# young-how/DQN-based-UAV-3D_path_planer

Hardware: AMD Instinct MI355X
Metric: env-steps/sec + learner updates/sec, PathPlan_City DQN (higher is better)
Workload: dtype f64

## Files before the change

### dqn_based_uav_3d_path_planer_amd/_lib.py

```python
from __future__ import annotations

import ctypes as C
import os

from . import _build

OBS_DIM = 100
MAX_BUILDINGS = 64
ABI_VERSION = 5

OK, EINVAL, ENOMEM, EHIP, ENODEV, EP2P = 0, -22, -12, -5, -19, -70
P2P_ERR_TIMEOUT, P2P_ERR_DIVERGED = 1, 2
COLL_ID_BYTES = 128
INFO_NORMAL, INFO_SUCCESS, INFO_LOSE, INFO_SKIPPED = 0, 1, 2, 3
INFO_NAMES = ("normal", "success", "lose", "skipped")
ACT_STEER_F32, ACT_STEER_F64, ACT_INDEX_I32 = 0, 1, 2
OBS_F32, OBS_F16, OBS_PACKED = 0, 1, 2
PACKED_DWORDS = 20
META_BYTES = 16
MFMA_F32, MFMA_F16 = 0, 1
P2P_HANDLE_BYTES = 64
P2P_CHECK_MAX_BLOCKS = 40
STEP_AUTO_RESET, STEP_SKIP_DONE, STEP_NO_OBS, STEP_ONE_WAVE, STEP_APF_LANE = 1, 2, 4, 8, 16

SYMBOLS = (
    "uavenv_abi_version", "uavenv_last_error", "uavenv_create", "uavenv_destroy", "uavenv_num_agents",
    "uavenv_set_buildings", "uavenv_load_scenarios", "uavenv_plan_scenarios", "uavenv_bank_stats", "uavenv_replan_begin", "uavenv_replan_ready", "uavenv_replan_commit", "uavenv_replan_stats", "uavenv_bank_read", "uavenv_set_moved_word", "uavenv_set_step_meta", "uavenv_tick", "uavenv_dqn_reduce_adam_gated", "uavenv_per_set_f32_gated", "uavenv_rrt_plan", "uavenv_reset_all", "uavenv_set_state", "uavenv_get_state",
    "uavenv_step", "uavenv_step_policy", "uavenv_set_debug_buffer", "uavenv_observe", "uavenv_threaten_rate", "uavenv_threaten_rate_allpairs", "uavenv_geometry",
    "uavenv_replay_sample", "uavenv_obs_unpack", "uavenv_replay_draw", "uavenv_replay_draw_valid", "uavenv_select_actions",
    "uavenv_dqn_num_params", "uavenv_dqn_partial_stride", "uavenv_dqn_partial_rows", "uavenv_dqn_set_debug_buffer", "uavenv_dqn_grad", "uavenv_dqn_grad_w", "uavenv_dqn_reduce", "uavenv_dqn_adam", "uavenv_dqn_reduce_adam", "uavenv_dqn_act",
    "uavenv_p2p_create", "uavenv_p2p_handle", "uavenv_p2p_connect", "uavenv_p2p_destroy", "uavenv_p2p_errors",
    "uavenv_p2p_configure", "uavenv_p2p_status", "uavenv_p2p_error_word", "uavenv_p2p_check_blocks", "uavenv_p2p_inject_fault", "uavenv_p2p_can_reach",
    "uavenv_coll_last_error", "uavenv_coll_unique_id", "uavenv_coll_create", "uavenv_coll_destroy", "uavenv_coll_allreduce_sum",
    "uavenv_dqn_reduce_p2p", "uavenv_dqn_adam_p2p",
    "uavenv_loop_create", "uavenv_loop_destroy", "uavenv_loop_set_eps", "uavenv_loop_run", "uavenv_loop_get", "uavenv_loop_get_per", "uavenv_loop_step_times",
    "uavenv_randn", "uavenv_sac_loop_noise_floats", "uavenv_sac_loop_create", "uavenv_sac_loop_destroy", "uavenv_sac_loop_run",
    "uavenv_sac_loop_get", "uavenv_sac_loop_get_per", "uavenv_per_fill_frame_strided", "uavenv_sac_act_multi", "uavenv_sac_critic_grad_multi", "uavenv_sac_actor_grad_multi",
    "uavenv_sac_critic_adam_multi", "uavenv_sac_actor_adam_multi",
    "uavenv_per_num_chunks", "uavenv_per_rotation", "uavenv_per_rebuild", "uavenv_per_sample", "uavenv_per_set", "uavenv_per_fill", "uavenv_per_set_f32", "uavenv_per_weights", "uavenv_per_fill_frame", "uavenv_per_rebuild_frame", "uavenv_p2p_allreduce", "uavenv_sac_partial_rows_n",
    "uavenv_sac_act", "uavenv_sac_reduce", "uavenv_sac_partial_rows", "uavenv_sac_last_error", "uavenv_sac_set_debug_buffer", "uavenv_sac_critic_grad", "uavenv_sac_critic_adam", "uavenv_sac_actor_grad",
    "uavenv_sac_actor_adam", "uavenv_fed_aggregate", "uavenv_eval_episodes", "uavenv_eval_episodes_sac", "uavenv_eval_noise_fill",
)
SAC_CRITIC_IN, SAC_ACTOR_PARAMS, SAC_CRITIC_PARAMS, SAC_ACTOR_STRIDE, SAC_CRITIC_STRIDE = 102, 6724, 10882, 6728, 21768


class UavEnvConfig(C.Structure):
    _fields_ = [
        ("abi_version", C.c_int32), ("device", C.c_int32), ("n_envs", C.c_int32), ("uav_per_env", C.c_int32),
        ("max_subgoals", C.c_int32), ("max_step", C.c_int32), ("apf_enabled", C.c_int32), ("obs_dtype", C.c_int32),
        ("n_actions", C.c_int32), ("reserved0", C.c_int32),
        ("len", C.c_double), ("width", C.c_double), ("h", C.c_double),
        ("max_v", C.c_double), ("steering_angle", C.c_double), ("power", C.c_double * 8), ("cell_size", C.c_double),
    ]


class UavReplayRing(C.Structure):
    _fields_ = [
        ("obs", C.c_void_p), ("action", C.c_void_p), ("reward", C.c_void_p), ("done", C.c_void_p),
        ("valid", C.c_void_p), ("frames", C.c_int32), ("n_agents", C.c_int32), ("obs_dtype", C.c_int32),
        ("action_is_index", C.c_int32), ("meta", C.c_void_p),
    ]


class UavDqnNet(C.Structure):
    _fields_ = [("local", C.c_void_p), ("target", C.c_void_p), ("m", C.c_void_p), ("v", C.c_void_p),
                ("w", C.c_int32), ("hid", C.c_int32), ("n_actions", C.c_int32), ("dueling", C.c_int32),
                ("mfma_dtype", C.c_int32), ("reserved0", C.c_int32)]


EVAL_SUCCESS, EVAL_LOSE, EVAL_TRUNCATED, EVAL_INVALID = 1, 2, 4, 5
EVAL_RECORD_BYTES = 64


class UavEvalRecord(C.Structure):
    _fields_ = [("ret", C.c_double), ("total_score", C.c_double), ("path_len", C.c_double), ("energy", C.c_double),
                ("v0x", C.c_double), ("v0y", C.c_double), ("steps", C.c_int32), ("subgoals", C.c_int32),
                ("collisions", C.c_int32), ("outcome", C.c_uint8), ("reach_goal", C.c_uint8), ("slot", C.c_uint8),
                ("reserved", C.c_uint8)]


class UavEvalArgs(C.Structure):
    _fields_ = [("n", C.c_int32), ("first", C.c_int32), ("start_goal", C.c_void_p), ("sub", C.c_void_p),
                ("nsub", C.c_void_p), ("m", C.c_int32), ("max_steps", C.c_int32), ("v0", C.c_void_p),
                ("seed", C.c_uint64), ("eps", C.c_float), ("traj_steps", C.c_int32), ("records", C.c_void_p),
                ("traj_pos", C.c_void_p), ("traj_act", C.c_void_p), ("max_workgroups", C.c_int32),
                ("reserved0", C.c_int32)]


EVAL_SAC_MEAN, EVAL_SAC_SAMPLE = 0, 1


class UavSacEvalArgs(C.Structure):
    _fields_ = [("n", C.c_int32), ("first", C.c_int32), ("start_goal", C.c_void_p), ("sub", C.c_void_p),
                ("nsub", C.c_void_p), ("m", C.c_int32), ("max_steps", C.c_int32), ("v0", C.c_void_p),
                ("seed", C.c_uint64), ("actors", C.POINTER(C.c_void_p)), ("n_actors", C.c_int32),
                ("action_bound", C.c_float), ("mode", C.c_int32), ("traj_steps", C.c_int32), ("records", C.c_void_p),
                ("traj_pos", C.c_void_p), ("traj_act", C.c_void_p), ("max_workgroups", C.c_int32),
                ("reserved0", C.c_int32)]


class UavPer(C.Structure):
    _fields_ = [("prio", C.c_void_p), ("chunk_sum", C.c_void_p), ("chunk_prefix", C.c_void_p),
                ("capacity", C.c_int64), ("rot", C.c_int64), ("group_sum", C.c_void_p)]


class UavLoopConfig(C.Structure):
    _fields_ = [("env", C.c_void_p), ("ring", UavReplayRing), ("net", UavDqnNet),
                ("head", C.c_int32), ("filled", C.c_int32), ("batch", C.c_int32), ("kind", C.c_int32),
                ("huber", C.c_int32), ("update_loop", C.c_int32), ("epoch", C.c_int32), ("learn_start", C.c_int32),
                ("seed", C.c_uint64), ("counter", C.c_uint64),
                ("eps", C.c_float), ("gamma", C.c_float), ("lr", C.c_float), ("beta1", C.c_float), ("beta2", C.c_float),
                ("adam_eps", C.c_float), ("step_flags", C.c_uint32), ("partials_dev", C.c_void_p),
                ("loss_dev", C.c_void_p), ("info_dev", C.c_void_p), ("p2p", C.c_void_p), ("time_every", C.c_int32),
                ("sample_lag", C.c_int32), ("coll", C.c_void_p), ("raw_dev", C.c_void_p),
                ("per", UavPer), ("per_alpha", C.c_double), ("per_beta", C.c_double), ("per_beta_inc", C.c_double),
                ("per_eps", C.c_double), ("per_clip", C.c_double),
                ("per_slots_dev", C.c_void_p), ("per_prio_dev", C.c_void_p), ("per_w_dev", C.c_void_p),
                ("per_abs_dev", C.c_void_p), ("per_idx_dev", C.c_void_p),
                ("replan_every", C.c_int32), ("replan_count", C.c_int32), ("replan_max_iter", C.c_int32), ("reserved1", C.c_int32),
                ("moved_dev", C.c_void_p)]


class UavLoopCursor(C.Structure):
    _fields_ = [("head", C.c_int32), ("filled", C.c_int32), ("epoch", C.c_int32), ("reserved0", C.c_int32),
                ("counter", C.c_uint64)]


class UavSacNets(C.Structure):
    _fields_ = [("actor", C.c_void_p), ("critic1", C.c_void_p), ("critic2", C.c_void_p), ("target1", C.c_void_p),
                ("target2", C.c_void_p), ("log_alpha", C.c_void_p)]


class UavSacBatch(C.Structure):
    _fields_ = [("obs_packed", C.c_void_p), ("idx_s", C.c_void_p), ("idx_n", C.c_void_p), ("draws", C.c_void_p),
                ("n_agents", C.c_int32), ("uav_per_env", C.c_int32), ("slot", C.c_int32), ("frames", C.c_int32),
                ("act0", C.c_void_p), ("act1", C.c_void_p), ("reward", C.c_void_p), ("done", C.c_void_p), ("valid", C.c_void_p),
                ("eps", C.c_void_p), ("batch", C.c_int32), ("tiles_per_wg", C.c_int32),
                ("is_weights", C.c_void_p), ("abs_td_out", C.c_void_p), ("meta", C.c_void_p), ("td_scratch", C.c_void_p)]


class UavSacAdam(C.Structure):
    _fields_ = [("lr", C.c_float), ("beta1", C.c_float), ("beta2", C.c_float), ("eps", C.c_float),
                ("bias_correction1", C.c_float), ("bias_correction2_sqrt", C.c_float), ("tau", C.c_float), ("grad_scale", C.c_float),
                ("skip_word", C.c_void_p), ("go_word", C.c_void_p), ("go_value", C.c_uint32), ("reserved0", C.c_uint32)]


SAC_LOOP_MAX_SLOTS = 8
FED_MAX_BLOCKS = 8
DRAW_MAX_TRIES = 8
DQN_IMAGE_FLOATS = 6912


class UavSacLoopSlot(C.Structure):
    _fields_ = [("nets", UavSacNets), ("m_actor", C.c_void_p), ("v_actor", C.c_void_p), ("alpha_mv", C.c_void_p),
                ("m1", C.c_void_p), ("v1", C.c_void_p), ("m2", C.c_void_p), ("v2", C.c_void_p), ("scalars", C.c_void_p),
                ("partials_critic", C.c_void_p), ("partials_actor", C.c_void_p),
                ("epoch", C.c_int32), ("adam_steps", C.c_int32),
                ("per", UavPer), ("per_slots_dev", C.c_void_p), ("per_prio_dev", C.c_void_p), ("per_w_dev", C.c_void_p),
                ("per_abs_dev", C.c_void_p), ("per_beta", C.c_double), ("td_dev", C.c_void_p)]


class UavSacLoopConfig(C.Structure):
    _fields_ = [("env", C.c_void_p), ("ring", UavReplayRing), ("act1_plane", C.c_void_p), ("info_dev", C.c_void_p),
                ("n_slots", C.c_int32), ("batch", C.c_int32), ("head", C.c_int32), ("filled", C.c_int32),
                ("is_train", C.c_int32), ("valid_draws", C.c_int32), ("seed", C.c_uint64), ("counter", C.c_uint64),
                ("beta1", C.c_double), ("beta2", C.c_double), ("adam_eps", C.c_double),
                ("gamma", C.c_float), ("tau", C.c_float), ("action_bound", C.c_float), ("actor_lr", C.c_float),
                ("critic_lr", C.c_float), ("alpha_lr", C.c_float), ("target_entropy", C.c_float), ("reserved1", C.c_float),
                ("step_flags", C.c_uint32), ("reserved2", C.c_uint32),
                ("draws_dev", C.c_void_p), ("noise_dev", C.c_void_p), ("slot", UavSacLoopSlot * SAC_LOOP_MAX_SLOTS),
                ("p2p", C.c_void_p), ("coll", C.c_void_p), ("xbuf_dev", C.c_void_p),
                ("per_alpha", C.c_double), ("per_beta_inc", C.c_double), ("per_eps", C.c_double), ("per_clip", C.c_double),
                ("moved_dev", C.c_void_p), ("check_every", C.c_int32), ("reserved3", C.c_int32)]


class UavSacLoopCursor(C.Structure):
    _fields_ = [("head", C.c_int32), ("filled", C.c_int32), ("counter", C.c_uint64),
                ("epoch", C.c_int32 * SAC_LOOP_MAX_SLOTS), ("adam_steps", C.c_int32 * SAC_LOOP_MAX_SLOTS)]


class UavEnvError(RuntimeError):
    pass


_LIB = None


def load() -> C.CDLL:
    global _LIB
    if _LIB is not None:
        return _LIB
    import torch
    path = _build.LIB_PATH
    if _build.needs_build():
        _build.build()
    if not os.path.exists(path):
        raise UavEnvError(f"{path} is missing and could not be built; the env hot path has no CPU fallback")
    lib = C.CDLL(path)
    vp, i32, u32, u64, i64, f32 = C.c_void_p, C.c_int32, C.c_uint32, C.c_uint64, C.c_int64, C.c_float
    lib.uavenv_abi_version.restype = C.c_int
    lib.uavenv_last_error.restype = C.c_char_p
    lib.uavenv_create.restype = C.c_int
    lib.uavenv_create.argtypes = [C.POINTER(UavEnvConfig), C.POINTER(vp)]
    lib.uavenv_destroy.restype = C.c_int
    lib.uavenv_destroy.argtypes = [vp]
    lib.uavenv_num_agents.restype = C.c_int
    lib.uavenv_num_agents.argtypes = [vp]
    lib.uavenv_set_buildings.restype = C.c_int
    lib.uavenv_set_buildings.argtypes = [vp, vp, vp, i32]
    lib.uavenv_load_scenarios.restype = C.c_int
    lib.uavenv_load_scenarios.argtypes = [vp, vp, vp, vp, i32]
    lib.uavenv_plan_scenarios.restype = C.c_int
    lib.uavenv_plan_scenarios.argtypes = [vp, i32, u64, i32, vp]
    lib.uavenv_bank_stats.restype = C.c_int
    lib.uavenv_bank_stats.argtypes = [vp, vp, vp]
    lib.uavenv_replan_begin.restype = C.c_int
    lib.uavenv_replan_begin.argtypes = [vp, i32, i32, u64, i32, vp]
    lib.uavenv_replan_ready.restype = C.c_int
    lib.uavenv_replan_ready.argtypes = [vp]
    lib.uavenv_replan_commit.restype = C.c_int
    lib.uavenv_replan_commit.argtypes = [vp, i32, vp]
    lib.uavenv_replan_stats.restype = C.c_int
    lib.uavenv_replan_stats.argtypes = [vp, vp]
    lib.uavenv_set_moved_word.restype = C.c_int
    lib.uavenv_set_moved_word.argtypes = [vp, vp]
    lib.uavenv_set_step_meta.restype = C.c_int
    lib.uavenv_set_step_meta.argtypes = [vp, vp, vp]
    lib.uavenv_tick.restype = C.c_uint64
    lib.uavenv_tick.argtypes = [vp]
    lib.uavenv_bank_read.restype = C.c_int
    lib.uavenv_bank_read.argtypes = [vp, i32, i32, vp, vp, vp]
    lib.uavenv_rrt_plan.restype = C.c_int
    lib.uavenv_rrt_plan.argtypes = [vp, i32, vp, vp, i32, u64, i32, C.c_double, C.c_double, vp, vp, vp, vp, vp]
    lib.uavenv_reset_all.restype = C.c_int
    lib.uavenv_reset_all.argtypes = [vp, u64, vp]
    lib.uavenv_set_state.restype = C.c_int
    lib.uavenv_set_state.argtypes = [vp, i32, i32, vp, vp, vp, vp, vp]
    lib.uavenv_get_state.restype = C.c_int
    lib.uavenv_get_state.argtypes = [vp, i32, i32, vp, vp, vp]
    lib.uavenv_step.restype = C.c_int
    lib.uavenv_step.argtypes = [vp, vp, i32, vp, vp, vp, vp, vp, vp, vp, vp, vp, u32, vp]
    lib.uavenv_step_policy.restype = C.c_int
    lib.uavenv_step_policy.argtypes = [vp, C.POINTER(UavDqnNet), vp, f32, u64, u64, vp, vp, vp, vp, vp, vp, vp, vp, vp, vp, u32, vp]
    lib.uavenv_set_debug_buffer.restype = C.c_int
    lib.uavenv_set_debug_buffer.argtypes = [vp, vp]
    lib.uavenv_observe.restype = C.c_int
    lib.uavenv_observe.argtypes = [vp, vp, vp]
    lib.uavenv_threaten_rate.restype = C.c_int
    lib.uavenv_threaten_rate.argtypes = [vp, vp, vp, i64, vp]
    lib.uavenv_geometry.restype = C.c_int
    lib.uavenv_geometry.argtypes = [vp, vp, vp, i64, vp]
    lib.uavenv_threaten_rate_allpairs.restype = C.c_int
    lib.uavenv_threaten_rate_allpairs.argtypes = [vp, vp, vp, i64, vp]
    lib.uavenv_replay_sample.restype = C.c_int
    lib.uavenv_replay_sample.argtypes = [C.POINTER(UavReplayRing), i32, i32, i32, u64, u64, vp, vp, vp, vp, vp, vp, vp]
    lib.uavenv_obs_unpack.restype = C.c_int
    lib.uavenv_obs_unpack.argtypes = [vp, i64, vp, i32, vp]
    lib.uavenv_replay_draw.restype = C.c_int
    lib.uavenv_replay_draw.argtypes = [i32, i32, i32, i32, i32, u64, u64, vp, vp]
    lib.uavenv_replay_draw_valid.restype = C.c_int
    lib.uavenv_replay_draw_valid.argtypes = [i32, i32, i32, i32, i32, i32, i32, i32, vp, i32, u64, u64, vp, vp]
    lib.uavenv_p2p_create.restype = C.c_int
    lib.uavenv_p2p_create.argtypes = [i32, i32, i32, C.POINTER(vp)]
    lib.uavenv_p2p_handle.restype = C.c_int
    lib.uavenv_p2p_handle.argtypes = [vp, vp]
    lib.uavenv_p2p_connect.restype = C.c_int
    lib.uavenv_p2p_connect.argtypes = [vp, vp]
    lib.uavenv_p2p_destroy.restype = C.c_int
    lib.uavenv_p2p_destroy.argtypes = [vp]
    lib.uavenv_p2p_errors.restype = C.c_int
    lib.uavenv_p2p_errors.argtypes = [vp, C.POINTER(i32)]
    lib.uavenv_p2p_configure.restype = C.c_int
    lib.uavenv_p2p_configure.argtypes = [vp, i32, i32]
    lib.uavenv_p2p_status.restype = C.c_int
    lib.uavenv_p2p_status.argtypes = [vp, i32, C.POINTER(i32)]
    lib.uavenv_p2p_can_reach.restype = C.c_int
    lib.uavenv_p2p_can_reach.argtypes = [i32, i32]
    lib.uavenv_p2p_inject_fault.restype = C.c_int
    lib.uavenv_p2p_inject_fault.argtypes = [vp, i32]
    lib.uavenv_coll_last_error.restype = C.c_char_p
    lib.uavenv_coll_unique_id.restype = C.c_int
    lib.uavenv_coll_unique_id.argtypes = [C.c_char_p, vp]
    lib.uavenv_coll_create.restype = C.c_int
    lib.uavenv_coll_create.argtypes = [C.c_char_p, i32, i32, vp, C.POINTER(vp)]
    lib.uavenv_coll_destroy.restype = C.c_int
    lib.uavenv_coll_destroy.argtypes = [vp]
    lib.uavenv_coll_allreduce_sum.restype = C.c_int
    lib.uavenv_coll_allreduce_sum.argtypes = [vp, vp, i64, vp]
    lib.uavenv_dqn_reduce_p2p.restype = C.c_int
    lib.uavenv_dqn_reduce_p2p.argtypes = [C.POINTER(UavDqnNet), vp, i32, vp, vp]
    lib.uavenv_dqn_adam_p2p.restype = C.c_int
    lib.uavenv_dqn_adam_p2p.argtypes = [C.POINTER(UavDqnNet), vp, f32, f32, f32, f32, i32, i32, vp, vp, vp]
    lib.uavenv_loop_create.restype = C.c_int
    lib.uavenv_loop_create.argtypes = [C.POINTER(UavLoopConfig), C.POINTER(vp)]
    lib.uavenv_loop_destroy.restype = C.c_int
    lib.uavenv_loop_destroy.argtypes = [vp]
    lib.uavenv_loop_set_eps.restype = C.c_int
    lib.uavenv_loop_set_eps.argtypes = [vp, f32]
    lib.uavenv_loop_run.restype = C.c_int
    lib.uavenv_loop_run.argtypes = [vp, i32, vp]
    lib.uavenv_loop_get.restype = C.c_int
    lib.uavenv_loop_get.argtypes = [vp, C.POINTER(UavLoopCursor)]
    lib.uavenv_loop_step_times.restype = C.c_int
    lib.uavenv_loop_step_times.argtypes = [vp, vp, i32, C.POINTER(i32)]
    for _n in ("uavenv_sac_act_multi", "uavenv_sac_critic_grad_multi", "uavenv_sac_actor_grad_multi",
               "uavenv_sac_critic_adam_multi", "uavenv_sac_actor_adam_multi"):
        getattr(lib, _n).restype = C.c_int
    lib.uavenv_sac_critic_grad_multi.argtypes = [vp, vp, i32, f32, f32, vp, vp]
    lib.uavenv_sac_actor_grad_multi.argtypes = [vp, vp, i32, f32, vp, vp]
    lib.uavenv_sac_critic_adam_multi.argtypes = [vp, vp, i32, vp, vp, vp, vp, vp, vp, i32, vp]
# ... 123 lines not shown
```

### dqn_based_uav_3d_path_planer_amd/csrc/dqn_internal.hpp

```cpp
#pragma once
#include <stdint.h>

#include "../../include/uavenv.h"

extern "C" {

#define UAVENV_DQN_IMAGE_FLOATS 6912

int uavenv_dqn_split_image(const UavDqnNet *net, float *image_dev, void *stream);

int uavenv_dqn_grad_img(const UavReplayRing *ring, int32_t head, int32_t filled, int32_t batch, uint64_t seed, uint64_t counter,
                        const int32_t *explicit_idx, const UavDqnNet *net, int32_t kind, float gamma, int32_t huber,
                        const float *is_weights, float *abs_td_out, float *partials, const float *image_dev, void *stream);

int uavenv_dqn_reduce_adam_img(const UavDqnNet *net, const float *partials, int32_t n_partials, float lr, float beta1, float beta2,
                               float eps, int32_t step_t, int32_t hard_update, float *loss_out, float *raw_out,
                               const uint32_t *go_word, uint32_t go_value, float *image_dev, void *stream);

int uavenv_dqn_adam_p2p_img(const UavDqnNet *net, struct UavP2P *c, float lr, float beta1, float beta2, float eps, int32_t step_t,
                            int32_t hard_update, float *loss_out, float *raw_out, float *image_dev, void *stream);
int uavenv_dqn_adam_img(const UavDqnNet *net, const float *raw, float lr, float beta1, float beta2, float eps, int32_t step_t,
                        int32_t hard_update, float *loss_out, float *image_dev, void *stream);

int uavenv_step_policy_img(UavEnv *e, const UavDqnNet *net, const void *obs_cur, float eps, uint64_t seed, uint64_t counter,
                           int32_t *action_out, void *obs, double *reward64, float *reward32, uint8_t *ret_done, uint8_t *agent_done,
                           uint8_t *info, uint8_t *valid, double *energy64, const uint8_t *active, uint32_t flags,
                           const float *image_dev, void *stream);

}
```

### dqn_based_uav_3d_path_planer_amd/csrc/learner.hip

```cpp
#include <hip/hip_runtime.h>
#include <hip/hip_fp16.h>
#include <stdint.h>
#include <stdlib.h>

#include "../../include/uavenv.h"
#include "uavenv_device.hpp"
#include "qnet_device.hpp"
#include "dqn_internal.hpp"

using namespace uav;
using namespace uavq;

namespace {

struct GradArgs {
    UavReplayRing ring;
    int head, filled, batch;
    uint64_t seed, counter;
    ReplayPerm perm;
    const int32_t *explicit_idx;
    const float *local, *target;
    int n_actions, dueling, kind;
    float gamma;
    int huber;
    float *partials;
    int P;
    unsigned long long *dbg;
    const float *is_w;
    float *abs_td;
    const float *img;
};

#ifdef UAVENV_PHASE_PROFILE
#define L_STAMP(slot) do { if (g.dbg && threadIdx.x == 0) g.dbg[(size_t)blockIdx.x * 8 + (slot)] = __builtin_amdgcn_s_memtime(); } while (0)
#define L_STAMP2(slot) do { if (g.dbg && threadIdx.x == 0) g.dbg[((size_t)gridDim.x + blockIdx.x) * 8 + (slot)] = __builtin_amdgcn_s_memtime(); } while (0)
#else
#define L_STAMP(slot) do { } while (0)
#define L_STAMP2(slot) do { } while (0)
#endif


__device__ __forceinline__ void load_transition(const UavReplayRing &R, uint32_t row, int &act, float &rew, uint32_t &done, uint32_t &valid)
{
    if (R.meta) {
        const uint4 m = reinterpret_cast<const uint4 *>(R.meta)[row];
        act = (int)m.y;
        rew = __uint_as_float(m.z);
        done = m.w & 0xffu;
        valid = (m.w >> 8) & 0xffu;
    } else {
        act = reinterpret_cast<const int32_t *>(R.action)[row];
        rew = R.reward[row];
        done = R.done[row];
        valid = R.valid ? (uint32_t)R.valid[row] : 1u;
    }
}

template <typename T>
__device__ __forceinline__ floatx4 x_load(const T *obs, uint32_t ring_row, int q)
{
    if (sizeof(T) == 4) {
        return *reinterpret_cast<const floatx4 *>(reinterpret_cast<const float *>(obs) + (size_t)ring_row * kW + 4 * q);
    } else {
        const uint2 raw = *reinterpret_cast<const uint2 *>(reinterpret_cast<const __half *>(obs) + (size_t)ring_row * kW + 4 * q);
        return floatx4{__uint_as_float(raw.x), __uint_as_float(raw.y), 0.0f, 0.0f};
    }
}

template <typename T>
__device__ __forceinline__ void x_issue(floatx4 (&v)[kXIters], const T *obs, uint32_t my_row)
{
    const int lane = (int)threadIdx.x & 63;
#pragma unroll
    for (int it = 0; it < kXIters; ++it) {
        int c = it * 64 + lane;
        c = c < 400 ? c : 399;
        const int row = c / 25, q = c - row * 25;
        const uint32_t ring_row = (uint32_t)__shfl((int)my_row, row, 64);
        v[it] = x_load<T>(obs, ring_row, q);
    }
}

template <typename T>
__device__ __forceinline__ void x_commit(float *strip, floatx4 (&v)[kXIters])
{
    const int lane = (int)threadIdx.x & 63;
#pragma unroll
    for (int it = 0; it < kXIters; ++it) {
        const int c = it * 64 + lane;
        if (c < 400) {
            const int row = c / 25, q = c - row * 25;
            floatx4 w = v[it];
            if (sizeof(T) != 4) {
                const uint32_t rx = __float_as_uint(v[it][0]), ry = __float_as_uint(v[it][1]);
                const __half2 lo = *reinterpret_cast<const __half2 *>(&rx);
                const __half2 hi = *reinterpret_cast<const __half2 *>(&ry);
                w = floatx4{__low2float(lo), __high2float(lo), __low2float(hi), __high2float(hi)};
            }
            *reinterpret_cast<floatx4 *>(strip + row * kLd + 4 * q) = w;
        }
    }
    if (lane < 16) *reinterpret_cast<floatx4 *>(strip + lane * kLd + kW) = floatx4{1.0f, 0.0f, 0.0f, 0.0f};
}

__device__ __forceinline__ void fwd_strip(const float *W, const float *strip, floatx4 (&acc)[4])
{
    const int lane = (int)threadIdx.x & 63, r = lane & 15, g = lane >> 4;
    const float *xp = strip + r * kLd + 26 * g;
    const float *wp = W + r * kLd + 26 * g;
#pragma unroll
    for (int t = 0; t < 4; ++t) acc[t] = floatx4{0.0f, 0.0f, 0.0f, 0.0f};
    float2 b = *reinterpret_cast<const float2 *>(xp);
    float2 a[4];
// ... 577 lines not shown
struct FlagOps {
    half8 one[2][6];
};
__device__ __forceinline__ half8 tiny_of(const half8 &one)
{
    uintx4 d = *reinterpret_cast<const uintx4 *>(&one);
#pragma unroll
    for (int k = 0; k < 4; ++k) d[k] = (d[k] << 2) & 0x10001000u;
    return *reinterpret_cast<const half8 *>(&d);
}
__device__ __forceinline__ void flag_ops_build(const GradLdsP &L, int r, int gq, FlagOps &F)
{
    const uint32_t *pr = L.Ps + 4 * gq * kPackedDwords;
#pragma unroll
    for (int q = 0; q < 2; ++q) {
        uintx4 mk[8];
#pragma unroll
        for (int i = 0; i < 8; ++i) mk[i] = *reinterpret_cast<const uintx4 *>(pr + (32 * q + 16 * (i >> 2) + (i & 3)) * kPackedDwords);
#pragma unroll
        for (int u = 0; u < 6; ++u) {
            half8 tiny;
            flags_to_half8(mk, u >> 1, (uint32_t)(16 * (u & 1) + r), F.one[q][u], tiny);
        }
    }
}
__device__ __forceinline__ void grad_products_split8b(const GradLdsP &L, const float *amax4, int grp, int strip, int r, int gq,
                                                      const FlagOps &F, GradAcc8 &A)
{
    const float *db = L.dHs + 4 * gq * kLh + 16 * strip + r;
    float dh[2][8];
    if (grp == 1) {
        float up, down;
        split_scale(fmaxf(fmaxf(amax4[0], amax4[1]), fmaxf(amax4[2], amax4[3])), up, down);
#pragma unroll
        for (int q = 0; q < 2; ++q)
#pragma unroll
            for (int i = 0; i < 8; ++i) dh[q][i] = db[(32 * q + 16 * (i >> 2) + (i & 3)) * kLh];
        floatx4 ch[6];
#pragma unroll
        for (int u = 0; u < 6; ++u) ch[u] = floatx4{0.0f, 0.0f, 0.0f, 0.0f};
#pragma unroll
        for (int q = 0; q < 2; ++q) {
            half8 bh, bm;
            split_half8(dh[q], up, bh, bm);
#pragma unroll
            for (int u = 0; u < 6; ++u) ch[u] = mfma16h(F.one[q][u], bh, ch[u]);
#pragma unroll
            for (int u = 0; u < 6; ++u) ch[u] = mfma16h(tiny_of(F.one[q][u]), bm, ch[u]);
        }
#pragma unroll
        for (int u = 0; u < 6; ++u)
#pragma unroll
            for (int k = 0; k < 4; ++k) A.acc[u][k] += ch[u][k] * down;
        return;
    }
    const uint32_t *pr = L.Ps + 4 * gq * kPackedDwords;
    const int dsc = r < 15 ? 4 + r : 19;
    const float *ha = L.Hs + 4 * gq * kLh + 16 * strip + r;
    const float *ob = L.douts + 4 * gq * kMaxOut + r;
    float xs[2][8], hh[2][8], bo[2][8];
#pragma unroll
    for (int q = 0; q < 2; ++q)
#pragma unroll
        for (int i = 0; i < 8; ++i) {
            const int s1 = 32 * q + 16 * (i >> 2) + (i & 3);
            dh[q][i] = db[s1 * kLh];
            xs[q][i] = __uint_as_float(pr[s1 * kPackedDwords + dsc]);
            hh[q][i] = ha[s1 * kLh];
            bo[q][i] = ob[s1 * kMaxOut];
        }
    floatx4 csc = floatx4{0.0f, 0.0f, 0.0f, 0.0f}, cw2 = floatx4{0.0f, 0.0f, 0.0f, 0.0f};
    const bool ones = r == 15;
#pragma unroll
    for (int q = 0; q < 2; ++q)
#pragma unroll
        for (int i = 0; i < 8; ++i) {
            csc = mfma16(ones ? 1.0f : xs[q][i], dh[q][i], csc);
            cw2 = mfma16(hh[q][i], bo[q][i], cw2);
        }
#pragma unroll
    for (int k = 0; k < 4; ++k) { A.acc[0][k] += csc[k]; A.acc[1][k] += cw2[k]; }
}

template <bool FIRST, int SPLIT, bool GLDS>
__device__ __forceinline__ void grad_tile_packed8(const GradArgs &g, const GradLdsP &L, float *qn_lds, int tile, bool more,
                                                  GradAcc8 &A)
{
    constexpr int NMAX = 4;
    const int tid = (int)threadIdx.x, lane = tid & 63, wv = __builtin_amdgcn_readfirstlane(tid >> 6), grp = wv >> 2, strip = wv & 3;
    const int r = lane & 15, gq = lane >> 4, t256 = tid & 255;
    const int n2 = g.n_actions + (g.dueling ? 1 : 0);
    const uint32_t *obs = reinterpret_cast<const uint32_t *>(g.ring.obs);
    const float *net = grp == 0 ? g.local : g.target;
    floatx4 vW[kStageIters];
    SplitScRegs vS;
    float pw[4] = {0, 0, 0, 0}, pb2 = 0.0f;
    if (FIRST) {
        if (GLDS) img_glds(grp == 0 ? L.W1l : L.W1t, g.img + (grp == 0 ? 0 : kSplitF), strip);
        else if (g.img) img_issue(vW, g.img + (grp == 0 ? 0 : kSplitF));
        else w_issue_half(vW, net, t256);
        const NetDev nv = net_view(net, n2);
        if (!GLDS && !g.img) w_issue_sc(vS, net, nv.b1);
#pragma unroll
        for (int k = 0; k < 4; ++k) pw[k] = nv.W2[t256 + 256 * k < n2 * kHid ? t256 + 256 * k : 0];
        pb2 = nv.b2[t256 < n2 ? t256 : 0];
    }
    L_STAMP2(0);
    const int smp = tile * kTile + strip * 16 + r;
    int f, agent;
    if (g.explicit_idx) {
        f = g.explicit_idx[2 * smp];
        agent = g.explicit_idx[2 * smp + 1];
    } else {
        replay_slot_to_frame(g.perm, replay_perm_apply(g.perm, (uint32_t)smp), g.head, g.ring.frames, f, agent);
    }
    int fn = f + 1;
    if (fn >= g.ring.frames) fn = 0;
    const uint32_t row_s = (uint32_t)f * (uint32_t)g.ring.n_agents + (uint32_t)agent;
    const uint32_t row_n = (uint32_t)fn * (uint32_t)g.ring.n_agents + (uint32_t)agent;
    L_STAMP2(1);
    PRow R;
    prow_load(R, obs + (size_t)(grp == 0 ? row_s : row_n) * kPackedDwords);
    int p_act = 0;
    float p_rew = 0.0f, p_w = 1.0f;
    uint32_t raw_done = 0u, raw_valid = 1u;
    if (grp == 0) {
        load_transition(g.ring, row_s, p_act, p_rew, raw_done, raw_valid);
        p_w = g.is_w ? g.is_w[smp] : 1.0f;
    }
    L_STAMP(6);
    if (FIRST) {
        if (!GLDS) {
            if (g.img) img_commit(grp == 0 ? L.W1l : L.W1t, vW); else w_commit_split(w1split_at(grp == 0 ? L.W1l : L.W1t), vW, vS);
        }
        L_STAMP(7);
        float *W2 = grp == 0 ? L.W2l : L.W2t, *b2 = grp == 0 ? L.b2l : L.b2t;
#pragma unroll
        for (int k = 0; k < 4; ++k)
            if (t256 + 256 * k < n2 * kHid) W2[t256 + 256 * k] = pw[k];
        if (t256 < n2) b2[t256] = pb2;
        __syncthreads();
    }
    L_STAMP(1);
    floatx4 hl[4];
    W2Frag<NMAX> Fl;
    float ql[NMAX];
    if (grp == 0) {
        fwd_strip_split<false>(w1split_at(L.W1l), R, hl);
        w2_load<NMAX>(Fl, L.W2l, L.b2l, n2);
        q_strip<NMAX>(hl, Fl, n2, g.n_actions, g.dueling, ql);
        if (gq == 0) prow_store_lds(L.Ps + (strip * 16 + r) * kPackedDwords, R);
    } else {
        int best = 0;
        floatx4 ht[4];
        if (g.kind == 1) {
            fwd_strip_split<false>(w1split_at(L.W1l), R, ht);
            W2Frag<NMAX> F;
            w2_load<NMAX>(F, L.W2l, L.b2l, n2);
            float qn_l[NMAX];
            q_strip<NMAX>(ht, F, n2, g.n_actions, g.dueling, qn_l);
            float bq = qn_l[0];
#pragma unroll
            for (int a = 1; a < NMAX; ++a)
                if (a < g.n_actions && qn_l[a] > bq) { bq = qn_l[a]; best = a; }
        }
        fwd_strip_split<false>(w1split_at(L.W1t), R, ht);
        W2Frag<NMAX> Ft;
        w2_load<NMAX>(Ft, L.W2t, L.b2t, n2);
        float qt[NMAX];
        q_strip<NMAX>(ht, Ft, n2, g.n_actions, g.dueling, qt);
        if (gq == 0) qn_lds[strip * 16 + r] = pick_qn<NMAX>(g, qt, best);
    }
    L_STAMP(2);
    __syncthreads();
    L_STAMP(3);
    FlagOps FO;
    if (SPLIT == 2 && grp == 1) flag_ops_build(L, r, gq, FO);
    if (grp == 0) {
        GradAcc<NMAX> T;
#pragma unroll
        for (int a = 0; a < NMAX + 2; ++a) T.csum[a] = A.csum[a];
        float amax = 0.0f;
        const float p_done = (float)raw_done, p_valid = (float)raw_valid;
        td_backward<NMAX>(g, L.W2l, hl, Fl, ql, qn_lds[strip * 16 + r], p_act, p_rew, p_done, p_valid, p_w, smp, T,
                          L.Hs + (strip * 16 + r) * kLh, L.dHs + (strip * 16 + r) * kLh, L.douts + (strip * 16 + r) * kMaxOut,
                          SPLIT ? &amax : nullptr);
#pragma unroll
        for (int a = 0; a < NMAX + 2; ++a) A.csum[a] = T.csum[a];
        if (SPLIT) {
            amax = wave_max64(amax);
            if (lane == 0) qn_lds[kTile + strip] = amax;
        }
    }
    __syncthreads();
    L_STAMP(4);
    if (SPLIT) {
        if (SPLIT == 2) grad_products_split8b(L, qn_lds + kTile, grp, strip, r, gq, FO, A);
        else grad_products_split8(L, qn_lds + kTile, grp, strip, r, gq, A);
        if (more) __syncthreads();
        return;
    }
    {
        const uint32_t *pr = L.Ps + 4 * gq * kPackedDwords;
        const int ia = 4 + (r < 11 ? r : 10), ib = 15 + (r < 6 ? 0 : (r > 9 ? 3 : r - 6));
        const bool sc0 = r < 11, sc5 = r >= 6 && r <= 9;
        const float ones = r == 4 ? 1.0f : 0.0f;
        const int sh = grp == 0 ? r : 16 + r;
        const float *db = L.dHs + 4 * gq * kLh + 16 * strip + r;
        const float *ha = L.Hs + 4 * gq * kLh + 16 * strip + r;
        const float *ob = L.douts + 4 * gq * kMaxOut + r;
        struct Raw { uintx4 mk; float sx, bdh, ah, bo; };
        auto load = [&](int k) {
            const int s1 = (k & 3) + 16 * (k >> 2);
            Raw w;
            w.mk = *reinterpret_cast<const uintx4 *>(pr + s1 * kPackedDwords);
            w.sx = __uint_as_float(pr[s1 * kPackedDwords + (grp == 0 ? ia : ib)]);
            w.bdh = db[s1 * kLh];
            w.ah = ha[s1 * kLh];
            w.bo = ob[s1 * kMaxOut];
            return w;
        };
        auto decode = [&](const Raw &w, float (&ax)[4]) {
            const float b0 = (float)((w.mk[0] >> sh) & 1u), b1 = (float)((w.mk[1] >> sh) & 1u), b2 = (float)((w.mk[2] >> sh) & 1u);
            if (grp == 0) { ax[0] = sc0 ? w.sx : b0; ax[1] = b1; ax[2] = b2; ax[3] = ones; }
            else { ax[0] = b0; ax[1] = b1; ax[2] = sc5 ? w.sx : b2; ax[3] = w.ah; }
        };
        Raw cur = load(0), nxt = load(1);
        float ax[4];
        decode(cur, ax);
#pragma unroll
        for (int kk = 0; kk < 16; ++kk) {
            Raw nn = nxt;
            if (kk + 2 < 16) nn = load(kk + 2);
            float axn[4];
            decode(nxt, axn);
            __builtin_amdgcn_sched_barrier(0);
#pragma unroll
            for (int u = 0; u < 3; ++u) A.acc[u] = mfma16(ax[u], cur.bdh, A.acc[u]);
            A.acc[3] = mfma16(ax[3], grp == 0 ? cur.bdh : cur.bo, A.acc[3]);
            __builtin_amdgcn_sched_barrier(0);
            cur = nxt;
            nxt = nn;
#pragma unroll
            for (int u = 0; u < 4; ++u) ax[u] = axn[u];
        }
    }
    if (more) __syncthreads();
}

template <int SPLIT, bool GLDS = false>
__global__ void __launch_bounds__(512) k_dqn_grad_packed8(Grad2Args ga)
{
    UAV_HOT_PRIO();
    constexpr int NMAX = 4;
    const GradArgs &g = ga.g;
    extern __shared__ __align__(16) float lds[];
    GradLdsP L;
    L.W1l = lds;
    L.W1t = L.W1l + kTileF;
    L.Hs = L.W1t + kTileF;
    L.dHs = L.Hs + kTile * kLh;
    L.douts = L.dHs + kTile * kLh;
    L.W2l = L.douts + kTile * kMaxOut;
    L.W2t = L.W2l + kMaxOut * kHid;
    L.b2l = L.W2t + kMaxOut * kHid;
    L.b2t = L.b2l + kMaxOut;
    L.red = L.b2t + kMaxOut;
    L.Ps = reinterpret_cast<uint32_t *>(L.red + 4 * (kMaxOut + 2));
    float *qn_lds = reinterpret_cast<float *>(L.Ps + kTile * kPackedDwords + 4);
    const int tid = (int)threadIdx.x, lane = tid & 63, wv = __builtin_amdgcn_readfirstlane(tid >> 6), grp = wv >> 2, strip = wv & 3;
    const int r = lane & 15, gq = lane >> 4;
    const int n2 = g.n_actions + (g.dueling ? 1 : 0);
    GradAcc8 A;
#pragma unroll
    for (int u = 0; u < 6; ++u) A.acc[u] = floatx4{0.0f, 0.0f, 0.0f, 0.0f};
#pragma unroll
    for (int a = 0; a < 6; ++a) A.csum[a] = 0.0f;
    L_STAMP(0);
    const int step = (int)gridDim.x;
    int tile = (int)blockIdx.x;
    grad_tile_packed8<true, SPLIT, GLDS>(g, L, qn_lds, tile, tile + step < ga.n_tiles, A);
    for (tile += step; tile < ga.n_tiles; tile += step)
        grad_tile_packed8<false, SPLIT, GLDS>(g, L, qn_lds, tile, tile + step < ga.n_tiles, A);
    L_STAMP(5);
    float *out = g.partials + (size_t)blockIdx.x * ga.stride;
    const int oW2 = kHid * kW + kHid, ob2 = oW2 + n2 * kHid;
    const int j = 16 * strip + r;
#define UAV_ROW_ST4(ptr, val) (*reinterpret_cast<floatx4 *>(ptr) = (val))
    if (SPLIT == 2) {
        if (grp == 1) {
            float *t0 = out + j * kW + 4 * gq;
            if (gq == 3) UAV_ROW_ST4(t0, A.acc[0]);
            else if (gq == 2) t0[3] = A.acc[0][3];
#pragma unroll
            for (int u = 1; u < 5; ++u) UAV_ROW_ST4(out + j * kW + 16 * u + 4 * gq, A.acc[u]);
            float *t5 = out + j * kW + 80 + 4 * gq;
            if (gq == 0 || gq == 3) UAV_ROW_ST4(t5, A.acc[5]);
            else if (gq == 1) { t5[0] = A.acc[5][0]; t5[1] = A.acc[5][1]; }
            else { t5[2] = A.acc[5][2]; t5[3] = A.acc[5][3]; }
        } else {
            const floatx4 sc = A.acc[0];
            if (gq < 2) UAV_ROW_ST4(out + j * kW + 4 * gq, sc);
            else if (gq == 2) { out[j * kW + 8] = sc[0]; out[j * kW + 9] = sc[1]; out[j * kW + 10] = sc[2]; out[j * kW + 86] = sc[3]; }
            else { out[j * kW + 87] = sc[0]; out[j * kW + 88] = sc[1]; out[j * kW + 89] = sc[2]; out[kHid * kW + j] = sc[3]; }
            if (gq == 0) UAV_ROW_ST4(out + j * kW + 96, (floatx4{0.0f, 0.0f, 0.0f, 0.0f}));
            if (r < n2) UAV_ROW_ST4(out + oW2 + r * kHid + 16 * strip + 4 * gq, A.acc[1]);
        }
    } else if (SPLIT) {
        if (grp == 0) {
            floatx4 t0 = A.acc[0];
#pragma unroll
            for (int k = 0; k < 4; ++k) t0[k] += (4 * gq + k <= 10) ? A.acc[3][k] : 0.0f;
            UAV_ROW_ST4(out + j * kW + 4 * gq, t0);
            UAV_ROW_ST4(out + j * kW + 32 + 4 * gq, A.acc[1]);
            UAV_ROW_ST4(out + j * kW + 64 + 4 * gq, A.acc[2]);
            if (gq == 2) out[j * kW + 86] = A.acc[3][3];
            if (gq == 3) { out[j * kW + 87] = A.acc[3][0]; out[j * kW + 88] = A.acc[3][1]; out[j * kW + 89] = A.acc[3][2];
                           out[kHid * kW + j] = A.acc[3][3]; }
            if (gq == 0) *reinterpret_cast<floatx4 *>(out + j * kW + 96) = floatx4{0.0f, 0.0f, 0.0f, 0.0f};
        } else {
            UAV_ROW_ST4(out + j * kW + 16 + 4 * gq, A.acc[0]);
            UAV_ROW_ST4(out + j * kW + 48 + 4 * gq, A.acc[1]);
            float *t5 = out + j * kW + 80 + 4 * gq;
            if (gq == 0 || gq == 3) *reinterpret_cast<floatx4 *>(t5) = A.acc[2];
            else if (gq == 1) { t5[0] = A.acc[2][0]; t5[1] = A.acc[2][1]; }
            else { t5[2] = A.acc[2][2]; t5[3] = A.acc[2][3]; }
            if (r < n2) *reinterpret_cast<floatx4 *>(out + oW2 + r * kHid + 16 * strip + 4 * gq) = A.acc[3];
        }
    } else if (grp == 0) {
#pragma unroll
        for (int u = 0; u < 3; ++u) *reinterpret_cast<floatx4 *>(out + j * kW + 32 * u + 4 * gq) = A.acc[u];
        if (gq == 0) *reinterpret_cast<floatx4 *>(out + j * kW + 96) = A.acc[3];
        else if (gq == 1) out[kHid * kW + j] = A.acc[3][0];
    } else {
#pragma unroll
        for (int u = 0; u < 3; ++u) *reinterpret_cast<floatx4 *>(out + j * kW + 16 + 32 * u + 4 * gq) = A.acc[u];
        if (r < n2) *reinterpret_cast<floatx4 *>(out + oW2 + r * kHid + 16 * strip + 4 * gq) = A.acc[3];
    }
    if (grp == 0 && lane == 0) {
#pragma unroll
        for (int a = 0; a < NMAX + 2; ++a) L.red[strip * (kMaxOut + 2) + a] = A.csum[a];
    }
    __syncthreads();
    if (tid < NMAX + 2) {
        const float s = (L.red[tid] + L.red[(kMaxOut + 2) + tid]) + (L.red[2 * (kMaxOut + 2) + tid] + L.red[3 * (kMaxOut + 2) + tid]);
        if (tid < n2) out[ob2 + tid] = s;
        else if (tid == NMAX) out[g.P] = s;
        else if (tid == NMAX + 1) out[g.P + 1] = s;
    }
}

constexpr size_t kGradP8Lds = (size_t)(2 * kTileF + 2 * kTile * kLh + kTile * kMaxOut + 2 * kMaxOut * kHid + 2 * kMaxOut +
                                       4 * (kMaxOut + 2) + kTile * kPackedDwords + 4 + kTile + 4) * 4;

constexpr size_t kGradPLds = (size_t)(2 * kTileF + 2 * kTile * kLh + kTile * kMaxOut + 2 * kMaxOut * kHid + 2 * kMaxOut +
                                      4 * (kMaxOut + 2) + kTile * kPackedDwords + 4) * 4;
static_assert((2 * kTileF + 2 * kTile * kLh + kTile * kMaxOut + 2 * kMaxOut * kHid + 2 * kMaxOut + 4 * (kMaxOut + 2)) % 4 == 0,
              "packed-row staging must start 16-byte aligned");

constexpr int kLdH = 136;
constexpr int kStageW = 16 * kPackedDwords + 4;

__device__ __forceinline__ floatx4 packed_expand4(const uint32_t *pr, int q)
{
    const int c = 4 * q, w = c >> 5;
    const uint32_t mw = pr[w < 3 ? w : 2];
// ... 973 lines not shown
    hipLaunchKernelGGL((k_dqn_act<ObsT, NMAX>), dim3(grid), dim3(256), kAct2Lds, s, g);
    return UAVENV_OK;
}

template <int NMAX>
static int launch_grad_packed(const Grad2Args &ga, int grid, hipStream_t s)
{
    static bool attr = false;
    if (!attr) {
        if (hipFuncSetAttribute(reinterpret_cast<const void *>(&k_dqn_grad_packed<NMAX>),
                                hipFuncAttributeMaxDynamicSharedMemorySize, (int)kGradPLds) != hipSuccess)
            return UAVENV_EHIP;
        attr = true;
    }
    hipLaunchKernelGGL((k_dqn_grad_packed<NMAX>), dim3(grid), dim3(256), kGradPLds, s, ga);
    return UAVENV_OK;
}

template <typename ObsT, int NMAX>
static int launch_grad(const Grad2Args &ga, int grid, hipStream_t s)
{
    static bool attr = false;
    if (!attr) {
        if (hipFuncSetAttribute(reinterpret_cast<const void *>(&k_dqn_grad<ObsT, NMAX>),
                                hipFuncAttributeMaxDynamicSharedMemorySize, (int)kGrad2Lds) != hipSuccess)
            return UAVENV_EHIP;
        attr = true;
    }
    hipLaunchKernelGGL((k_dqn_grad<ObsT, NMAX>), dim3(grid), dim3(256), kGrad2Lds, s, ga);
    return UAVENV_OK;
}


}

extern "C" {

int uavenv_dqn_set_debug_buffer(unsigned long long *dev_buf)
{
    g_learner_dbg = dev_buf;
    return UAVENV_OK;
}

int uavenv_dqn_num_params(const UavDqnNet *net)
{
    if (!net) return UAVENV_EINVAL;
    const int n2 = net->n_actions + (net->dueling ? 1 : 0);
    return net->hid * net->w + net->hid + n2 * net->hid + n2;
}

int uavenv_dqn_partial_stride(const UavDqnNet *net)
{
    if (!net_ok(net)) return UAVENV_EINVAL;
    return (uavenv_dqn_num_params(net) + 2 + 31) & ~31;
}

int uavenv_dqn_partial_rows(int32_t batch)
{
    if (batch <= 0 || batch % kTile != 0) return UAVENV_EINVAL;
    const int tiles = batch / kTile;
    return tiles < kMaxGradGrid ? tiles : kMaxGradGrid;
}

int uavenv_dqn_grad(const UavReplayRing *ring, int32_t head, int32_t filled, int32_t batch, uint64_t seed,
                    uint64_t counter, const int32_t *explicit_idx, const UavDqnNet *net, int32_t kind, float gamma,
                    int32_t huber, float *partials, void *stream)
{
    return uavenv_dqn_grad_w(ring, head, filled, batch, seed, counter, explicit_idx, net, kind, gamma, huber, nullptr, nullptr,
                             partials, stream);
}

int uavenv_dqn_grad_w(const UavReplayRing *ring, int32_t head, int32_t filled, int32_t batch, uint64_t seed,
                      uint64_t counter, const int32_t *explicit_idx, const UavDqnNet *net, int32_t kind, float gamma,
                      int32_t huber, const float *is_weights, float *abs_td_out, float *partials, void *stream)
{
    return uavenv_dqn_grad_img(ring, head, filled, batch, seed, counter, explicit_idx, net, kind, gamma, huber, is_weights, abs_td_out,
                               partials, nullptr, stream);
}

int uavenv_dqn_grad_img(const UavReplayRing *ring, int32_t head, int32_t filled, int32_t batch, uint64_t seed,
                        uint64_t counter, const int32_t *explicit_idx, const UavDqnNet *net, int32_t kind, float gamma,
                        int32_t huber, const float *is_weights, float *abs_td_out, float *partials, const float *image_dev, void *stream)
{
    if (!ring || !ring->obs || !ring->action || !ring->reward || !ring->done || !partials || !net_ok(net) || !net->target)
        return UAVENV_EINVAL;
    if (batch <= 0 || batch % kTile != 0 || ring->frames < 2 || head < 0 || head >= ring->frames) return UAVENV_EINVAL;
    if (!explicit_idx && (filled <= 0 || filled > ring->frames - 1)) return UAVENV_EINVAL;
    if ((uint64_t)ring->frames * (uint64_t)ring->n_agents >= (1ull << 32)) return UAVENV_EINVAL;
    if (!ring->action_is_index) return UAVENV_EINVAL;
    if ((((uintptr_t)partials | (uintptr_t)net->local | (uintptr_t)net->target | (uintptr_t)ring->meta) & 15u) != 0) return UAVENV_EINVAL;
    Grad2Args ga;
    GradArgs &g = ga.g;
    g.ring = *ring;
    g.head = head; g.filled = filled; g.batch = batch;
    g.seed = seed; g.counter = counter;
    g.explicit_idx = explicit_idx;
    g.perm = replay_perm(seed, counter, explicit_idx ? 1u : (uint32_t)filled * (uint32_t)ring->n_agents, (uint32_t)ring->n_agents);
    g.local = net->local; g.target = net->target;
    g.n_actions = net->n_actions; g.dueling = net->dueling; g.kind = kind;
    g.gamma = gamma; g.huber = huber;
    g.partials = partials;
    g.P = uavenv_dqn_num_params(net);
    g.dbg = g_learner_dbg;
    g.is_w = is_weights;
    g.abs_td = abs_td_out;
    g.img = (image_dev && (((uintptr_t)image_dev) & 15u) == 0) ? image_dev : nullptr;
    ga.n_tiles = batch / kTile;
    ga.stride = uavenv_dqn_partial_stride(net);
    const int grid = uavenv_dqn_partial_rows(batch);
    hipStream_t s = (hipStream_t)stream;
    const bool small = net->n_actions + (net->dueling ? 1 : 0) <= 4;
    int rc;
    if (net->mfma_dtype == UAVENV_MFMA_F16) {
        if (!small || ring->obs_dtype == UAVENV_OBS_F32) return UAVENV_EINVAL;
        static const bool four_waves_h = getenv("UAVENV_GRAD_4WAVES") != nullptr;
        if (four_waves_h)
            rc = ring->obs_dtype == UAVENV_OBS_PACKED ? launch_grad_h<OBS_KIND_PACKED>(ga, grid, s) : launch_grad_h<OBS_KIND_F16>(ga, grid, s);
        else
            rc = ring->obs_dtype == UAVENV_OBS_PACKED ? launch_grad_h8<OBS_KIND_PACKED>(ga, grid, s) : launch_grad_h8<OBS_KIND_F16>(ga, grid, s);
    } else if (ring->obs_dtype == UAVENV_OBS_F32)
        rc = small ? launch_grad<float, 4>(ga, grid, s) : launch_grad<float, kMaxOut - 2>(ga, grid, s);
    else if (ring->obs_dtype == UAVENV_OBS_PACKED) {
        static const bool four_waves = getenv("UAVENV_GRAD_4WAVES") != nullptr;
        if (small && !four_waves) {
            static const bool dw1_f32 = getenv("UAVENV_DW1_F32") != nullptr;
            static bool attr8 = false;
            static const bool dw1_b = getenv("UAVENV_DW1_SPLITA") == nullptr;
            static const bool stage_vgpr = getenv("UAVENV_STAGE_VGPR") && atoi(getenv("UAVENV_STAGE_VGPR")) != 0;
            if (!attr8) {
                if (hipFuncSetAttribute(reinterpret_cast<const void *>(&k_dqn_grad_packed8<1>),
                                        hipFuncAttributeMaxDynamicSharedMemorySize, (int)kGradP8Lds) != hipSuccess ||
                    hipFuncSetAttribute(reinterpret_cast<const void *>(&k_dqn_grad_packed8<2>),
                                        hipFuncAttributeMaxDynamicSharedMemorySize, (int)kGradP8Lds) != hipSuccess ||
                    hipFuncSetAttribute(reinterpret_cast<const void *>(&k_dqn_grad_packed8<2, true>),
                                        hipFuncAttributeMaxDynamicSharedMemorySize, (int)kGradP8Lds) != hipSuccess ||
                    hipFuncSetAttribute(reinterpret_cast<const void *>(&k_dqn_grad_packed8<0>),
                                        hipFuncAttributeMaxDynamicSharedMemorySize, (int)kGradP8Lds) != hipSuccess)
                    return UAVENV_EHIP;
                attr8 = true;
            }
            if (dw1_f32) hipLaunchKernelGGL(k_dqn_grad_packed8<0>, dim3(grid), dim3(512), kGradP8Lds, s, ga);
            else if (dw1_b && g.img && !stage_vgpr) hipLaunchKernelGGL((k_dqn_grad_packed8<2, true>), dim3(grid), dim3(512), kGradP8Lds, s, ga);
            else if (dw1_b) hipLaunchKernelGGL(k_dqn_grad_packed8<2>, dim3(grid), dim3(512), kGradP8Lds, s, ga);
            else hipLaunchKernelGGL(k_dqn_grad_packed8<1>, dim3(grid), dim3(512), kGradP8Lds, s, ga);
            rc = UAVENV_OK;
        } else {
            rc = small ? launch_grad_packed<4>(ga, grid, s) : launch_grad_packed<kMaxOut - 2>(ga, grid, s);
        }
    }
    else
        rc = small ? launch_grad<__half, 4>(ga, grid, s) : launch_grad<__half, kMaxOut - 2>(ga, grid, s);
    if (rc != UAVENV_OK) return rc;
    return hipGetLastError() == hipSuccess ? UAVENV_OK : UAVENV_EHIP;
}

int uavenv_dqn_reduce(const UavDqnNet *net, const float *partials, int32_t n_partials, float *raw_out, void *stream)
{
    if (!net_ok(net) || !partials || !raw_out || n_partials <= 0) return UAVENV_EINVAL;
    const int P = uavenv_dqn_num_params(net);
    hipLaunchKernelGGL(k_dqn_reduce, dim3((P + 2 + 31) / 32), dim3(256), 0, (hipStream_t)stream, partials, n_partials, P,
                       uavenv_dqn_partial_stride(net), raw_out);
    return hipGetLastError() == hipSuccess ? UAVENV_OK : UAVENV_EHIP;
}

int uavenv_dqn_adam(const UavDqnNet *net, const float *raw, float lr, float beta1, float beta2, float eps, int32_t step_t,
                    int32_t hard_update, float *loss_out, void *stream)
{
    return uavenv_dqn_adam_img(net, raw, lr, beta1, beta2, eps, step_t, hard_update, loss_out, nullptr, stream);
}

int uavenv_dqn_adam_img(const UavDqnNet *net, const float *raw, float lr, float beta1, float beta2, float eps, int32_t step_t,
                        int32_t hard_update, float *loss_out, float *image_dev, void *stream)
{
    if (!net_ok(net) || !net->target || !net->m || !net->v || !raw || step_t <= 0) return UAVENV_EINVAL;
    if (image_dev && (net->w != kW || net->hid != kHid || (((uintptr_t)image_dev) & 15u) != 0)) return UAVENV_EINVAL;
    const int P = uavenv_dqn_num_params(net);
    const float bc1 = 1.0f - powf(beta1, (float)step_t);
    const float bc2 = 1.0f - powf(beta2, (float)step_t);
    hipLaunchKernelGGL(k_dqn_adam, dim3((P + 255) / 256), dim3(256), 0, (hipStream_t)stream, net->local, net->target,
                       net->m, net->v, raw, P, lr, beta1, beta2, eps, bc1, sqrtf(bc2), hard_update, loss_out, image_dev);
    return hipGetLastError() == hipSuccess ? UAVENV_OK : UAVENV_EHIP;
}

int uavenv_dqn_reduce_adam(const UavDqnNet *net, const float *partials, int32_t n_partials, float lr, float beta1,
                           float beta2, float eps, int32_t step_t, int32_t hard_update, float *loss_out, float *raw_out,
                           void *stream)
{
    return uavenv_dqn_reduce_adam_gated(net, partials, n_partials, lr, beta1, beta2, eps, step_t, hard_update, loss_out, raw_out,
                                        nullptr, 0u, stream);
}

int uavenv_dqn_reduce_adam_gated(const UavDqnNet *net, const float *partials, int32_t n_partials, float lr, float beta1,
                                 float beta2, float eps, int32_t step_t, int32_t hard_update, float *loss_out, float *raw_out,
                                 const uint32_t *go_word_dev, uint32_t go_value, void *stream)
{
    return uavenv_dqn_reduce_adam_img(net, partials, n_partials, lr, beta1, beta2, eps, step_t, hard_update, loss_out, raw_out, go_word_dev,
                                      go_value, nullptr, stream);
}

int uavenv_dqn_reduce_adam_img(const UavDqnNet *net, const float *partials, int32_t n_partials, float lr, float beta1, float beta2,
                               float eps, int32_t step_t, int32_t hard_update, float *loss_out, float *raw_out,
                               const uint32_t *go_word_dev, uint32_t go_value, float *image_dev, void *stream)
{
    if (image_dev && (net->w != kW || net->hid != kHid || (((uintptr_t)image_dev) & 15u) != 0)) return UAVENV_EINVAL;
    if (!net_ok(net) || !net->target || !net->m || !net->v || !partials || n_partials <= 0 || step_t <= 0)
        return UAVENV_EINVAL;
    const int P = uavenv_dqn_num_params(net);
    const float bc1 = 1.0f - powf(beta1, (float)step_t);
    const float bc2 = 1.0f - powf(beta2, (float)step_t);
    hipLaunchKernelGGL(k_dqn_reduce_adam, dim3((P + 2 + 31) / 32), dim3(256), 0, (hipStream_t)stream, partials, n_partials,
                       P, uavenv_dqn_partial_stride(net), net->local, net->target, net->m, net->v, lr, beta1, beta2, eps, bc1, sqrtf(bc2), hard_update,
                       loss_out, raw_out, go_word_dev, go_value, image_dev);
    return hipGetLastError() == hipSuccess ? UAVENV_OK : UAVENV_EHIP;
}

__global__ void __launch_bounds__(256) k_dqn_split_image(const float *__restrict__ local, const float *__restrict__ target,
                                                         float *__restrict__ img)
{
    const float *net = blockIdx.x == 0 ? local : target;
    floatx4 v[kStageIters];
    SplitScRegs sc;
    w_issue(v, net);
    w_issue_sc(sc, net, net + kHid * kW);
    w_commit_split(w1split_at(img + (size_t)blockIdx.x * kSplitF), v, sc);
// ... 38 lines not shown
```

### dqn_based_uav_3d_path_planer_amd/csrc/loop.hip

```cpp
#include <hip/hip_runtime.h>
#include <stdint.h>
#include <stdlib.h>
#include <math.h>
#include <new>
#include <vector>

#include "../../include/uavenv.h"
#include "dqn_internal.hpp"

#include <chrono>
#include <stdio.h>

struct UavLoop {
    double t_host[4] = {0, 0, 0, 0};
    bool prof = false;
    UavLoopConfig c;
    int32_t head, filled, epoch;
    uint64_t counter;
    size_t obs_row_bytes;
    bool fuse_act = true;
    bool per = false;
    double per_beta = 0.4;
    hipStream_t aux = nullptr;
    hipEvent_t ev_grad = nullptr, ev_join = nullptr;
    std::vector<hipEvent_t> ev;
    std::vector<hipEvent_t> pool;
    hipStream_t plan = nullptr;
    int32_t replan_next = 0, bank_m = 0;
    uint64_t replan_gen = 0;
    float *img = nullptr;
};

static int replan_tick(UavLoop *l, hipStream_t s)
{
    const UavLoopConfig &c = l->c;
    const int ready = uavenv_replan_ready(c.env);
    if (ready == 0) return UAVENV_OK;
    if (ready < -1) return ready;
    if (ready == 1) {
        const int rc = uavenv_replan_commit(c.env, 0, s);
        if (rc != UAVENV_OK) return rc;
    }
    int32_t count = c.replan_count < l->bank_m ? c.replan_count : l->bank_m;
    if (l->replan_next + count > l->bank_m) l->replan_next = 0;
    l->replan_gen += 1;
    const int rc = uavenv_replan_begin(c.env, l->replan_next, count, c.seed * 0x9E3779B97F4A7C15ull + l->replan_gen,
                                       c.replan_max_iter > 0 ? c.replan_max_iter : 10000, l->plan);
    if (rc != UAVENV_OK) return rc;
    l->replan_next += count;
    return UAVENV_OK;
}

extern "C" {

int uavenv_loop_create(const UavLoopConfig *cfg, UavLoop **out)
{
    if (!cfg || !out || !cfg->env || !cfg->ring.obs || !cfg->ring.action || !cfg->ring.reward || !cfg->ring.done ||
        !cfg->net.local)
        return UAVENV_EINVAL;
    if (!cfg->ring.action_is_index || cfg->ring.frames < 3 || cfg->ring.n_agents != uavenv_num_agents(cfg->env))
        return UAVENV_EINVAL;
    if (cfg->head < 0 || cfg->head >= cfg->ring.frames || cfg->filled < 0 || cfg->filled > cfg->ring.frames - 1)
        return UAVENV_EINVAL;
    if (cfg->batch < 0 || cfg->batch % 64 != 0 || (cfg->batch > 0 && (!cfg->partials_dev || !cfg->net.target ||
                                                                        !cfg->net.m || !cfg->net.v)))
        return UAVENV_EINVAL;
    if (cfg->update_loop <= 0 || cfg->epoch < 0) return UAVENV_EINVAL;
    if (!cfg->p2p && cfg->coll && !cfg->raw_dev) return UAVENV_EINVAL;
    if (cfg->per.prio) {
        if (cfg->per.capacity != (int64_t)cfg->ring.frames * cfg->ring.n_agents || cfg->batch <= 0 || !cfg->per_slots_dev ||
            !cfg->per_prio_dev || !cfg->per_w_dev || !cfg->per_abs_dev || !cfg->per_idx_dev || !cfg->ring.valid)
            return UAVENV_EINVAL;
    }
    UavLoop *l = new (std::nothrow) UavLoop();
    if (!l) return UAVENV_ENOMEM;
    l->c = *cfg;
    l->head = cfg->head;
    l->filled = cfg->filled;
    l->epoch = cfg->epoch;
    l->counter = cfg->counter;
    l->per = cfg->per.prio != nullptr;
    l->per_beta = cfg->per_beta;
    {
        static const bool off = getenv("UAVENV_LOOP_IMAGE") && atoi(getenv("UAVENV_LOOP_IMAGE")) == 0;
        if (!off && cfg->sample_lag == 0 && cfg->ring.obs_dtype == UAVENV_OBS_PACKED &&
            cfg->net.mfma_dtype == UAVENV_MFMA_F32 && cfg->net.w == 100 && cfg->net.hid == 64 && cfg->net.local && cfg->net.target) {
            if (hipMalloc((void **)&l->img, 2 * (size_t)UAVENV_DQN_IMAGE_FLOATS * sizeof(float)) != hipSuccess) { delete l; return UAVENV_ENOMEM; }
        }
    }
    if (cfg->sample_lag != 0) {
        if (cfg->sample_lag != 1 || l->per) { delete l; return UAVENV_EINVAL; }
        if (hipStreamCreateWithFlags(&l->aux, hipStreamNonBlocking) != hipSuccess ||
            hipEventCreateWithFlags(&l->ev_grad, hipEventDisableTiming) != hipSuccess ||
            hipEventCreateWithFlags(&l->ev_join, hipEventDisableTiming) != hipSuccess) {
            uavenv_loop_destroy(l);
            return UAVENV_EHIP;
        }
    }
    if (cfg->moved_dev) {
        if (cfg->p2p || cfg->coll || cfg->sample_lag != 0) { uavenv_loop_destroy(l); return UAVENV_EINVAL; }
        if (uavenv_set_moved_word(cfg->env, cfg->moved_dev) != UAVENV_OK) { uavenv_loop_destroy(l); return UAVENV_EINVAL; }
    }
    if (cfg->replan_every > 0) {
        int32_t m = 0;
        int lo = 0, hi = 0;
        if (cfg->replan_count <= 0 || uavenv_bank_stats(cfg->env, &m, nullptr) != UAVENV_OK || m <= 0) { uavenv_loop_destroy(l); return UAVENV_EINVAL; }
        l->bank_m = m;
        (void)hipDeviceGetStreamPriorityRange(&lo, &hi);
        if (hipStreamCreateWithPriority(&l->plan, hipStreamNonBlocking, lo) != hipSuccess) { uavenv_loop_destroy(l); return UAVENV_EHIP; }
    }
    l->fuse_act = getenv("UAVENV_NO_FUSED_ACT") == nullptr;
    l->prof = getenv("UAVENV_LOOP_PROFILE") != nullptr;
    l->obs_row_bytes = (size_t)cfg->ring.n_agents * (cfg->ring.obs_dtype == UAVENV_OBS_PACKED ? UAVENV_OBS_PACKED_DWORDS * 4
                                                     : UAVENV_OBS_DIM * (cfg->ring.obs_dtype == UAVENV_OBS_F16 ? 2 : 4));
    *out = l;
    return UAVENV_OK;
}

int uavenv_loop_destroy(UavLoop *l)
{
    if (!l) return UAVENV_OK;
    if (l->prof && l->t_host[3] > 0)
        fprintf(stderr, "uavenv_loop host us per pass: act+step %.2f grad %.2f adam %.2f (%.0f passes)\n", 1e6 * l->t_host[0] / l->t_host[3],
                1e6 * l->t_host[1] / l->t_host[3], 1e6 * l->t_host[2] / l->t_host[3], l->t_host[3]);
    if (l->c.moved_dev) (void)uavenv_set_moved_word(l->c.env, nullptr);
    for (hipEvent_t e : l->ev) (void)hipEventDestroy(e);
    for (hipEvent_t e : l->pool) (void)hipEventDestroy(e);
    if (l->aux) { (void)hipStreamSynchronize(l->aux); (void)hipStreamDestroy(l->aux); }
    if (l->plan) {
        (void)hipStreamSynchronize(l->plan);
        (void)hipStreamDestroy(l->plan);
    }
    for (hipEvent_t e : {l->ev_grad, l->ev_join}) if (e) (void)hipEventDestroy(e);
    if (l->img) (void)hipFree(l->img);
    delete l;
    return UAVENV_OK;
}

int uavenv_loop_set_eps(UavLoop *l, float eps)
{
    if (!l) return UAVENV_EINVAL;
    l->c.eps = eps;
    return UAVENV_OK;
}

int uavenv_loop_get_per(const UavLoop *l, double *beta_out)
{
    if (!l || !beta_out) return UAVENV_EINVAL;
    *beta_out = l->per_beta;
    return UAVENV_OK;
}

int uavenv_loop_get(const UavLoop *l, UavLoopCursor *out)
{
    if (!l || !out) return UAVENV_EINVAL;
    out->head = l->head;
    out->filled = l->filled;
    out->epoch = l->epoch;
    out->reserved0 = 0;
    out->counter = l->counter;
    return UAVENV_OK;
}

static hipEvent_t take_event(UavLoop *l)
{
    hipEvent_t e = nullptr;
    if (!l->pool.empty()) {
        e = l->pool.back();
        l->pool.pop_back();
    } else if (hipEventCreate(&e) != hipSuccess) {
        e = nullptr;
    }
    return e;
}

int uavenv_loop_run(UavLoop *l, int32_t n_steps, void *stream)
{
    if (!l || n_steps < 0) return UAVENV_EINVAL;
    const UavLoopConfig &c = l->c;
    const UavReplayRing &R = c.ring;
    const size_t n = (size_t)R.n_agents;
    hipStream_t s = (hipStream_t)stream;
    if (c.p2p) {
        int32_t st[4];
        if (uavenv_p2p_status(c.p2p, 0, st) == UAVENV_OK && st[0] != 0) return UAVENV_EP2P;
    }
    const bool lag = l->aux != nullptr;
    if (l->img && n_steps > 0) {
        const int ri = uavenv_dqn_split_image(&c.net, l->img, s);
        if (ri != UAVENV_OK) return ri;
    }
    for (int k = 0; k < n_steps; ++k) {
        const int t = l->head, nxt = t + 1 == R.frames ? 0 : t + 1;
        if (l->plan && l->counter % (uint64_t)c.replan_every == 0) {
            const int rr = replan_tick(l, s);
            if (rr != UAVENV_OK) return rr;
        }
        bool lag_update = false;
        if (lag && c.batch > 0 && l->filled > 0 &&
            (int64_t)l->filled * (int64_t)n >= (int64_t)(c.learn_start > c.batch ? c.learn_start : c.batch)) {
            if (hipEventRecord(l->ev_join, s) != hipSuccess || hipStreamWaitEvent(l->aux, l->ev_join, 0) != hipSuccess) return UAVENV_EHIP;
            const int filled_lag = l->filled < R.frames - 2 ? l->filled : R.frames - 2;
            int rcg = uavenv_dqn_grad(&R, l->head, filled_lag, c.batch, c.seed, l->counter, nullptr, &c.net, c.kind, c.gamma,
                                      c.huber, c.partials_dev, l->aux);
            if (rcg != UAVENV_OK) return rcg;
            if (hipEventRecord(l->ev_grad, l->aux) != hipSuccess) return UAVENV_EHIP;
            lag_update = true;
        }
        unsigned char *obs_t = (unsigned char *)R.obs + (size_t)t * l->obs_row_bytes;
        unsigned char *obs_n = (unsigned char *)R.obs + (size_t)nxt * l->obs_row_bytes;
        int32_t *act_t = (int32_t *)R.action + (size_t)t * n;
        const bool timed = c.time_every > 0 && (l->counter % (uint64_t)c.time_every) == 0;
        hipEvent_t e0 = nullptr, e1 = nullptr;
        int rc = UAVENV_EINVAL;
        std::chrono::steady_clock::time_point tp0, tp1, tp2, tp3;
        if (l->prof) tp0 = std::chrono::steady_clock::now();
        uint8_t *info_t = c.info_dev ? c.info_dev + (size_t)t * n : nullptr;
        uint8_t *valid_t = R.valid ? R.valid + (size_t)t * n : nullptr;
        void *meta_t = R.meta ? (unsigned char *)R.meta + (size_t)t * n * UAVENV_META_BYTES : nullptr;
        if (l->fuse_act) {
            if (timed) {
                e0 = take_event(l);
                e1 = take_event(l);
                if (e0 && e1) (void)hipEventRecord(e0, s);
            }
            rc = uavenv_set_step_meta(c.env, meta_t, nullptr);
            if (rc != UAVENV_OK) return rc;
            rc = uavenv_step_policy_img(c.env, &c.net, obs_t, c.eps, c.seed, l->counter, act_t, obs_n, nullptr, R.reward + (size_t)t * n,
                                        R.done + (size_t)t * n, nullptr, info_t, valid_t, nullptr, nullptr, c.step_flags, l->img, s);
            if (rc == UAVENV_EINVAL) l->fuse_act = false;
            else if (rc != UAVENV_OK) return rc;
        }
        if (!l->fuse_act) {
            rc = uavenv_dqn_act(&c.net, obs_t, R.obs_dtype, R.n_agents, c.eps, c.seed, l->counter, act_t, nullptr, nullptr, s);
            if (rc != UAVENV_OK) return rc;
            if (timed && !e0) {
                e0 = take_event(l);
                e1 = take_event(l);
                if (e0 && e1) (void)hipEventRecord(e0, s);
            }
            rc = uavenv_set_step_meta(c.env, meta_t, nullptr);
            if (rc != UAVENV_OK) return rc;
            rc = uavenv_step(c.env, act_t, UAVENV_ACT_INDEX_I32, obs_n, nullptr, R.reward + (size_t)t * n, R.done + (size_t)t * n,
                             nullptr, info_t, valid_t, nullptr, nullptr, c.step_flags, s);
        }
        if (timed && e0 && e1) {
            (void)hipEventRecord(e1, s);
            l->ev.push_back(e0);
            l->ev.push_back(e1);
        }
        if (rc != UAVENV_OK) return rc;
        if (l->prof) tp1 = std::chrono::steady_clock::now();
        l->head = nxt;
        if (l->filled < R.frames - 1) l->filled += 1;
        const bool learn_now = !lag && c.batch > 0 &&
                               (int64_t)l->filled * (int64_t)n >= (int64_t)(c.learn_start > c.batch ? c.learn_start : c.batch);
        const double per_new = l->per ? pow(0.0 + (double)c.per_eps, (double)c.per_alpha) : 0.0;
        if (l->per && !learn_now) {
            rc = uavenv_per_fill_frame(&c.per, (int64_t)t * (int64_t)n, (int64_t)n, per_new, R.valid + (size_t)t * n,
                                       (int64_t)nxt * (int64_t)n, s);
            if (rc != UAVENV_OK) return rc;
        }
        if (lag ? lag_update
                : (c.batch > 0 && (int64_t)l->filled * (int64_t)n >= (int64_t)(c.learn_start > c.batch ? c.learn_start : c.batch))) {
            if (lag) {
                if (hipStreamWaitEvent(s, l->ev_grad, 0) != hipSuccess) return UAVENV_EHIP;
                rc = UAVENV_OK;
            } else if (l->per) {
                l->per_beta = l->per_beta + (double)c.per_beta_inc < 1.0 ? l->per_beta + (double)c.per_beta_inc : 1.0;
                rc = uavenv_per_rebuild_frame(&c.per, (int64_t)t * (int64_t)n, (int64_t)n, per_new, R.valid + (size_t)t * n,
                                              (int64_t)nxt * (int64_t)n, s);
                if (rc != UAVENV_OK) return rc;
                rc = uavenv_per_sample(&c.per, c.batch, nullptr, c.seed, l->counter, c.per_slots_dev, c.per_prio_dev, s);
                if (rc != UAVENV_OK) return rc;
                rc = uavenv_per_weights(&c.per, c.per_slots_dev, c.per_prio_dev, c.batch, (int64_t)l->filled * (int64_t)n,
                                        l->per_beta, R.n_agents, c.per_w_dev, c.per_idx_dev, s);
                if (rc != UAVENV_OK) return rc;
                rc = uavenv_dqn_grad_img(&R, l->head, l->filled, c.batch, c.seed, l->counter, c.per_idx_dev, &c.net, c.kind, c.gamma,
                                         c.huber, c.per_w_dev, c.per_abs_dev, c.partials_dev, l->img, s);
            } else if ((c.step_flags & UAVENV_STEP_SKIP_DONE) != 0 && c.per_idx_dev && R.valid) {
                rc = uavenv_replay_draw_valid(R.frames, n, l->head, l->filled, c.batch, 1, 1, 0, R.valid, UAVENV_DRAW_MAX_TRIES, c.seed,
                                              l->counter, c.per_idx_dev, s);
                if (rc != UAVENV_OK) return rc;
                rc = uavenv_dqn_grad_img(&R, l->head, l->filled, c.batch, c.seed, l->counter, c.per_idx_dev, &c.net, c.kind, c.gamma,
                                         c.huber, nullptr, nullptr, c.partials_dev, l->img, s);
            } else {
                rc = uavenv_dqn_grad_img(&R, l->head, l->filled, c.batch, c.seed, l->counter, nullptr, &c.net, c.kind, c.gamma,
                                         c.huber, nullptr, nullptr, c.partials_dev, l->img, s);
            }
            if (rc != UAVENV_OK) return rc;
            if (l->prof) tp2 = std::chrono::steady_clock::now();
            l->epoch += 1;
            const int hard = l->epoch % c.update_loop == 0 ? 1 : 0;
            if (c.p2p) {
                rc = uavenv_dqn_reduce_p2p(&c.net, c.partials_dev, uavenv_dqn_partial_rows(c.batch), c.p2p, s);
                if (rc != UAVENV_OK) {
                    l->epoch -= 1;
                    l->counter += 1;
                    return rc;
                }
                rc = uavenv_dqn_adam_p2p_img(&c.net, c.p2p, c.lr, c.beta1, c.beta2, c.adam_eps, l->epoch, hard, c.loss_dev, nullptr, l->img, s);
                if (rc == UAVENV_EP2P) l->counter += 1;
            } else if (c.coll) {
                rc = uavenv_dqn_reduce(&c.net, c.partials_dev, uavenv_dqn_partial_rows(c.batch), c.raw_dev, s);
                if (rc != UAVENV_OK) return rc;
                rc = uavenv_coll_allreduce_sum(c.coll, c.raw_dev, (int64_t)uavenv_dqn_num_params(&c.net) + 2, s);
                if (rc != UAVENV_OK) return rc;
                rc = uavenv_dqn_adam_img(&c.net, c.raw_dev, c.lr, c.beta1, c.beta2, c.adam_eps, l->epoch, hard, c.loss_dev, l->img, s);
            } else {
                rc = uavenv_dqn_reduce_adam_img(&c.net, c.partials_dev, uavenv_dqn_partial_rows(c.batch), c.lr, c.beta1, c.beta2,
                                                c.adam_eps, l->epoch, hard, c.loss_dev, nullptr, c.moved_dev,
                                                (uint32_t)uavenv_tick(c.env), l->img, s);
            }
            if (rc != UAVENV_OK) return rc;
            if (l->per) {
                rc = uavenv_per_set_f32_gated(&c.per, c.per_slots_dev, c.per_abs_dev, c.batch, (double)c.per_eps, (double)c.per_alpha,
                                              (double)c.per_clip, c.moved_dev, (uint32_t)uavenv_tick(c.env), s);
                if (rc != UAVENV_OK) return rc;
            }
            if (l->prof) {
                tp3 = std::chrono::steady_clock::now();
                l->t_host[0] += std::chrono::duration<double>(tp1 - tp0).count();
                l->t_host[1] += std::chrono::duration<double>(tp2 - tp1).count();
                l->t_host[2] += std::chrono::duration<double>(tp3 - tp2).count();
                l->t_host[3] += 1.0;
            }
        }
        l->counter += 1;
    }
    return UAVENV_OK;
}

int uavenv_loop_step_times(UavLoop *l, float *ms_out, int32_t max_n, int32_t *n_out)
{
    if (!l || !n_out || (max_n > 0 && !ms_out)) return UAVENV_EINVAL;
    int n = 0;
    for (size_t i = 0; i + 1 < l->ev.size(); i += 2) {
        if (hipEventSynchronize(l->ev[i + 1]) != hipSuccess) return UAVENV_EHIP;
        float ms = 0.0f;
        if (n < max_n && hipEventElapsedTime(&ms, l->ev[i], l->ev[i + 1]) == hipSuccess) ms_out[n++] = ms;
        l->pool.push_back(l->ev[i]);
        l->pool.push_back(l->ev[i + 1]);
    }
    l->ev.clear();
    *n_out = n;
    return UAVENV_OK;
}

}

#include "uavenv_device.hpp"
#include "dqn_internal.hpp"

namespace {

__global__ void __launch_bounds__(256) k_randn(uint64_t seed, uint64_t counter, int64_t n, float *__restrict__ out)
{
    const int64_t q = (int64_t)blockIdx.x * 256 + threadIdx.x;
    if (4 * q >= n) return;
    const uint4 r = uav::philox4x32_10(make_uint4((uint32_t)q, (uint32_t)(q >> 32), (uint32_t)counter, (uint32_t)(counter >> 32) ^ 0x6a55u),
                                       make_uint2((uint32_t)seed, (uint32_t)(seed >> 32)));
    const float u1 = ((float)(r.x >> 8) + 1.0f) * (1.0f / 16777216.0f);
    const float u2 = (float)(r.y >> 8) * (1.0f / 16777216.0f);
    const float u3 = ((float)(r.z >> 8) + 1.0f) * (1.0f / 16777216.0f);
    const float u4 = (float)(r.w >> 8) * (1.0f / 16777216.0f);
    const float ra = sqrtf(-2.0f * logf(u1)), rb = sqrtf(-2.0f * logf(u3));
    float sa, ca, sb, cb;
    sincosf(6.283185307179586f * u2, &sa, &ca);
    sincosf(6.283185307179586f * u4, &sb, &cb);
    const float v[4] = {ra * ca, ra * sa, rb * cb, rb * sb};
#pragma unroll
    for (int e = 0; e < 4; ++e)
        if (4 * q + e < n) out[4 * q + e] = v[e];
// ... 277 lines not shown
```

### dqn_based_uav_3d_path_planer_amd/csrc/uavenv.hip

```cpp
#include <hip/hip_runtime.h>

#include <algorithm>
#include <cmath>
#include <cstdarg>
#include <cstdio>
#include <cstdlib>
#include <cstring>
#include <map>
#include <mutex>
#include <new>
#include <utility>
#include <vector>

#include "../../include/uavenv.h"
#include "uavenv_device.hpp"
#include "qnet_device.hpp"
#include "dqn_internal.hpp"

using namespace uav;

extern "C" int uavenv_rrt_plan_at(UavEnv *env, int32_t first, int32_t m, const double *start_goal_dev, const double *uniforms_dev,
                                  int32_t stream_len, uint64_t seed, int32_t max_iter, double step_size, double obstacle_step,
                                  double *out_start_goal_dev, double *out_sub_dev, int32_t *out_nsub_dev,
                                  int32_t *out_iters_dev, void *node_scratch, int32_t scratch_wgs, void *stream);
extern "C" int64_t uavenv_rrt_scratch_bytes(int32_t wgs);
extern "C" int uavenv_rrt_plan(UavEnv *env, int32_t m, const double *start_goal_dev, const double *uniforms_dev,
                               int32_t stream_len, uint64_t seed, int32_t max_iter, double step_size, double obstacle_step,
                               double *out_start_goal_dev, double *out_sub_dev, int32_t *out_nsub_dev,
                               int32_t *out_iters_dev, void *stream);

static thread_local char g_err[512] = "";

static int fail(int code, const char *fmt, ...)
{
    va_list ap;
    va_start(ap, fmt);
    vsnprintf(g_err, sizeof(g_err), fmt, ap);
    va_end(ap);
    return code;
}

#define HIP_TRY(expr)                                                                               \
    do {                                                                                            \
        hipError_t e_ = (expr);                                                                     \
        if (e_ != hipSuccess) return fail(UAVENV_EHIP, "%s -> %s", #expr, hipGetErrorString(e_));   \
    } while (0)

enum F64Field { F_PX, F_PY, F_PZ, F_VX, F_VY, F_V, F_GX, F_GY, F_GZ, F_S0X, F_S0Y, F_S0Z, F_S1X, F_S1Y, F_S1Z,
                F_SCORE, F_TOTAL, F_PATHLEN, F_HEAD };
enum I32Field { I_STEP, I_SUBIDX, I_NTOTAL, I_EPOCH, I_SCN, I_FLAGS };
constexpr int kFlagDone = 1, kFlagAlias = 2, kFlagReach = 4;
struct DevState {
    double *f64;
    int32_t *i32;
    size_t npad;
    double *sub;
    __host__ __device__ double *F(int k) const { return f64 + (size_t)k * npad; }
    __host__ __device__ int32_t *I(int k) const { return i32 + (size_t)k * npad; }
};
constexpr int kNumF64 = 19, kNumI32 = 6;

struct Bank {
    const double *start_goal;
    const double *sub;
    const int32_t *nsub;
    int32_t m;
};

struct StepArgs {
    DevState st;
    const unsigned char *world_blob;
    int32_t world_bytes, aux_off, grid_off, grid_stride;
    int32_t nb, gn;
    double inv_cell, W, Hbox;
    const BldApf *apf_b;
    const uint64_t *apf_grid;
    int32_t apf_gn, apf_nz;
    double apf_inv_cell, apf_inv_cz;
    uint64_t apf_all;
    double max_v, steer;
    PowerParams pw;
    int32_t max_step, K, U, N, n_actions;
    int32_t tile_off;
    int32_t wave_slot;
    int32_t obsq_off;
    int32_t apf_split;
    int32_t block;
    const void *actions;
    int32_t action_kind;
    void *obs;
    double *reward64;
    float *reward32;
    uint8_t *ret_done, *agent_done, *info, *valid;
    double *energy64;
    const uint2 *emit_lut;
    const uint8_t *active;
    unsigned long long *dbg;
    uint32_t flags;
    Bank bank;
    uint64_t seed, tick;
    const float *pol_local;
    const float *pol_img;
    const uint32_t *pol_obs;
    int32_t *pol_act;
    int32_t pol_dueling, pol_off;
    float pol_eps;
    uint64_t pol_seed, pol_counter;
    uint32_t *moved_word;
    uint32_t moved_value;
    uint4 *meta;
    const float *meta_a1;
};

struct UavEnv {
    UavEnvConfig cfg;
    int N;
    DevState st;
    void *slab = nullptr;
    size_t slab_bytes = 0;
    unsigned char *world_blob = nullptr;
    int world_bytes = 0, aux_off = 0, grid_off = 0, grid_stride = 0, nb = 0, gn = 0, mask_bytes = 8;
    double cell = 10.0;
    BldApf *apf_b = nullptr;
    uint64_t *apf_grid = nullptr;
    uint64_t apf_all = 0;
    int bank_replaced = 0;
    int apf_gn = 1, apf_nz = 1;
    double apf_cell = 10.0, apf_cz = 10.0;
    uint2 *emit_lut = nullptr;
    bool have_world = false;
    double *bank_sg = nullptr, *bank_sub = nullptr;
    int32_t *bank_nsub = nullptr;
    int bank_m = 0;
    uint64_t seed = 0, tick = 0;
    unsigned long long *dbg = nullptr;
    uint32_t *moved_word = nullptr;
    void *step_meta = nullptr;
    const float *step_meta_a1 = nullptr;
    double *rp_sg = nullptr, *rp_sub = nullptr;
    int32_t *rp_nsub = nullptr;
    int32_t *rp_counters = nullptr;
    int rp_cap = 0, rp_first = 0, rp_count = 0;
    void *rp_nodes = nullptr;
    int rp_wgs = 0;
    bool rp_pending = false;
    hipEvent_t rp_done = nullptr;
    hipEvent_t rp_committed = nullptr;
    bool rp_commit_recorded = false;
    int world_gen = 0, rp_world_gen = 0;
    long long rp_calls = 0, rp_rows_planned = 0;
    float *eval_img = nullptr;
    double *eval_sub = nullptr;
    int64_t eval_sub_lanes = 0;
};

__device__ __forceinline__ void stage_copy(unsigned char *smem, const StepArgs &a, int tid, int nthr)
{
    constexpr int kInFlight = 12;
    const uint4 *src = reinterpret_cast<const uint4 *>(a.world_blob);
    uint4 *dst = reinterpret_cast<uint4 *>(smem);
    const int n16 = a.world_bytes / 16;
    for (int base = 0; base < n16; base += nthr * kInFlight) {
        uint4 tmp[kInFlight];
#pragma unroll
        for (int r = 0; r < kInFlight; ++r) {
            const int k = base + r * nthr + tid;
            tmp[r] = src[k < n16 ? k : n16 - 1];
        }
#pragma unroll
        for (int r = 0; r < kInFlight; ++r)
            asm volatile("" : "+v"(tmp[r].x), "+v"(tmp[r].y), "+v"(tmp[r].z), "+v"(tmp[r].w));
#pragma unroll
        for (int r = 0; r < kInFlight; ++r) {
            const int k = base + r * nthr + tid;
            dst[k < n16 ? k : n16 - 1] = tmp[r];
        }
    }
}

__device__ __forceinline__ void stage_copy_glds(unsigned char *smem, const StepArgs &a, int w, int nw)
{
    const int lane = (int)threadIdx.x & 63;
    const uint4 *src = reinterpret_cast<const uint4 *>(a.world_blob);
    uint4 *dst = reinterpret_cast<uint4 *>(smem);
    const int n16 = a.world_bytes / 16;
    for (int base = w * 64; base < n16; base += nw * 64) {
        const int k = base + lane;
        if (k < n16) uavq::glds16(src + k, dst + base);
    }
}

template <typename MaskT>
__device__ __forceinline__ WorldLds<MaskT> world_view(unsigned char *smem, const StepArgs &a)
{
    WorldLds<MaskT> w;
    w.b = reinterpret_cast<const BldLds *>(smem);
    w.aux = reinterpret_cast<const BldAux *>(smem + a.aux_off);
    for (int h = 0; h < 3; ++h) w.g[h] = reinterpret_cast<const MaskT *>(smem + a.grid_off + h * a.grid_stride);
    w.gn = a.gn;
    w.inv_cell = a.inv_cell;
    w.W = a.W;
    w.Hbox = a.Hbox;
    return w;
}

template <typename MaskT>
__device__ __forceinline__ WorldLds<MaskT> stage_world(unsigned char *smem, const StepArgs &a)
{
    stage_copy(smem, a, (int)threadIdx.x, a.block);
    __syncthreads();
    return world_view<MaskT>(smem, a);
}

struct ForceTerms {
    double s, f1x, f1y, f2x, f2y;
};
__device__ __forceinline__ bool cal_force_terms(const BldApf &B, double x, double y, double z, ForceTerms &t)
{
    const double dx = B.cx - x, dy = B.cy - y, dz = B.cz - z;
    const double h2 = dx * dx + dy * dy;
    if (h2 + dz * dz > B.far2) return false;
// ... 682 lines not shown
            if (stepping) {
                PreStep P;
                PostMid M;
                bool head_set = false;
                const bool pre_alias = g.alias != 0;
                step_pre(a, a0, g, P);
                if (P.moved) g.head = angle_of<true>(g.o.vx, g.o.vy);
                step_post_a<MaskT, APF, true>(a, w, ii, a0, g, P, M, ret_done, info, head_set);
                if (M.live) adjust_subgoals_split(a, ii, g, pre_alias);
                step_post_b<MaskT, APF, true>(a, w, ii, g, M, r, ret_done, info, head_set);
            } else {
                ret_done = g.done; info = UAVENV_INFO_SKIPPED; valid = 0;
            }
        } else if (!stepping) {
            ret_done = g.done; info = UAVENV_INFO_SKIPPED; valid = 0;
        } else {
            step_agent<MaskT, APF, true>(a, w, ii, a0, g, r, ret_done, info);
        }
        UAV_STAMP(3);
        g.o.n_rem = g.n_total - g.sub_idx;
        const int agent_done = g.done;
        const double energy = a.energy64 ? fly_power(a.pw, g.o.V, ii % a.U) : 0.0;

        bool did_reset = false;
        if (a.flags & UAVENV_STEP_AUTO_RESET) {
            const unsigned long long dm = __ballot(active && g.done);
            const int lane = threadIdx.x & 63;
            const int g0 = lane & ~(a.U - 1);
            const unsigned long long gm = (a.U >= 64) ? ~0ull : (((1ull << a.U) - 1ull) << g0);
            did_reset = active && ((dm & gm) == gm);
            if (APF && a.apf_split) reset_agents_wave(a, i - lane, ii, g, did_reset);
            else if (did_reset) reset_agent<APF>(a, ii, g);
        }

        UAV_STAMP(4);
        const bool want_obs = a.obs && !(a.flags & UAVENV_STEP_NO_OBS);
        ObsBits bits;
        ObsScalars sc;
        if (want_obs) {
            ObsWaveLds *L = reinterpret_cast<ObsWaveLds *>(smem + a.obsq_off + (threadIdx.x >> 6) * a.wave_slot);
            bits = obs_bits_queued(w, L, g.o.px, g.o.py, g.o.pz, active);
            sc = obs_scalars(g.o, g.head);
        }
        if (active) {
            UAV_STAMP(5);
            if (a.reward64) a.reward64[i] = r;
            if (a.reward32) a.reward32[i] = (float)r;
            if (a.ret_done) a.ret_done[i] = (uint8_t)ret_done;
            if (a.agent_done) a.agent_done[i] = (uint8_t)agent_done;
            if (a.info) a.info[i] = (uint8_t)info;
            if (a.valid) a.valid[i] = (uint8_t)valid;
            if (a.meta)
                a.meta[i] = make_uint4(meta_a1, meta_action_bits(ra, POLH ? UAVENV_ACT_INDEX_I32 : a.action_kind, a0),
                                       __float_as_uint((float)r), (uint32_t)ret_done | ((uint32_t)valid << 8) | ((uint32_t)info << 16));
            if (a.moved_word && valid)
                __hip_atomic_store(a.moved_word, a.moved_value, __ATOMIC_RELAXED, __HIP_MEMORY_SCOPE_AGENT);
            if (a.energy64) a.energy64[i] = energy;
            if (valid || did_reset) store_agent(S, i, g);
            if (want_obs && a.tile_off < 0) store_obs_row<OBS>(a.obs, i, sc, bits);
            UAV_STAMP(6);
            UAV_DRAIN();
            UAV_STAMP(7);
        }
        if (a.tile_off >= 0 && want_obs) {
            const int first = i - ((int)threadIdx.x & 63);
            uint32_t *tile = reinterpret_cast<uint32_t *>(smem + a.tile_off + (threadIdx.x >> 6) * a.wave_slot);
            store_obs_ctile<OBS>(a.obs, first, N - first, tile, sc, bits);
        }
    }
}

template <typename MaskT, bool APF, int OBS>
__global__ void __launch_bounds__(256, UAVENV_KSTEP_WAVES) k_step(StepArgs a)
{
    k_step_body<MaskT, APF, OBS, false>(a);
}

template <typename MaskT>
__global__ void __launch_bounds__(192, 3) k_step_polh(StepArgs a)
{
    k_step_body<MaskT, false, OBS_KIND_F16, true>(a);
}

struct CoopLds {
    double cand[16][64];
    int32_t cand_n[64], cand_scn[64];
    double pos[64][4];
    double head[64];
    int32_t done[64];
    ObsWaveLds q[3];
    uint32_t tile[64 * kCTileLd];
};

template <typename MaskT, bool APF, int OBS, bool POLICY = false, bool PAHEAD = false, bool GLDS = false>
__global__ void __launch_bounds__(256) k_step_coop(StepArgs a)
{
    UAV_HOT_PRIO();
    extern __shared__ __align__(16) unsigned char smem[];
    const DevState &S = a.st;
    const int N = a.N;
    const int lane = (int)threadIdx.x & 63, wv = __builtin_amdgcn_readfirstlane((int)threadIdx.x >> 6);
    const int first = (int)blockIdx.x * 64;
    const int i = first + lane;
    const bool active = i < N;
    const int ii = active ? i : N - 1;
    CoopLds *C = reinterpret_cast<CoopLds *>(smem + a.obsq_off);
    const bool want_obs = a.obs && !(a.flags & UAVENV_STEP_NO_OBS);
    const bool auto_reset = (a.flags & UAVENV_STEP_AUTO_RESET) != 0;
    UAV_CSTAMP(0);

    const uavq::W1Split pW1 = uavq::w1split_at(reinterpret_cast<float *>(smem + a.pol_off));
    float *pW2 = reinterpret_cast<float *>(smem + a.pol_off) + uavq::kSplitF;
    float *pb2 = pW2 + uavq::kMaxOut * uavq::kHid;
    int32_t *pact = reinterpret_cast<int32_t *>(pb2 + uavq::kMaxOut);
    uavq::floatx4 vW[uavq::kStageIters];
    uavq::PRow prow;
    uavq::SplitScRegs pol_sc;
    float pol_w2[4] = {0, 0, 0, 0}, pol_b2v = 0.0f;
    uint4 pol_rn = make_uint4(0u, 0u, 0u, 0u);
    const int pol_i = first + wv * 16 + (lane & 15);
    const int pol_n2 = a.n_actions + (a.pol_dueling ? 1 : 0);
    if (POLICY) {
        const int tid = (int)threadIdx.x;
        const uavq::NetDev nl = uavq::net_view(a.pol_local, pol_n2);
        if (GLDS) {
            uavq::img_glds(reinterpret_cast<float *>(smem + a.pol_off), a.pol_img, wv);
            if (wv >= 2) stage_copy_glds(smem, a, wv - 2, 2);
        } else if (a.pol_img) uavq::img_issue(vW, a.pol_img);
        else { uavq::w_issue(vW, a.pol_local); uavq::w_issue_sc(pol_sc, a.pol_local, nl.b1); }
#pragma unroll
        for (int k = 0; k < 4; ++k) pol_w2[k] = nl.W2[tid + 256 * k < pol_n2 * uavq::kHid ? tid + 256 * k : pol_n2 * uavq::kHid - 1];
        pol_b2v = nl.b2[tid < pol_n2 ? tid : 0];
        uavq::prow_load(prow, a.pol_obs + (size_t)(pol_i < N ? pol_i : N - 1) * kPackedDwords);
        pol_rn = philox4x32_10(make_uint4((uint32_t)pol_i, (uint32_t)a.pol_counter, (uint32_t)(a.pol_counter >> 32), 0xac7u),
                               make_uint2((uint32_t)a.pol_seed, (uint32_t)(a.pol_seed >> 32)));
    }
    Agent g;
    RawAction ra = {0u, 0u};
    double head_old = 0.0;
    uint32_t meta_a1 = 0u;
    if (wv == 0) {
        load_agent(S, ii, g);
        if (!POLICY) ra = load_action_raw(a.actions, a.action_kind, ii);
        if (a.meta_a1) meta_a1 = __float_as_uint(a.meta_a1[ii]);
    } else if (wv == 2) {
        head_old = S.F(F_HEAD)[ii];
        if (!POLICY) ra = load_action_raw(a.actions, a.action_kind, ii);
    }
    ResetCand cand;
    double cand_heading = 0.0;
    bool cand_want = false;
    if (wv == 1 && auto_reset) {
        const int c_flags = S.I(I_FLAGS)[ii], c_sub = S.I(I_SUBIDX)[ii], c_n = S.I(I_NTOTAL)[ii], c_step = S.I(I_STEP)[ii];
        const double dx = S.F(F_GX)[ii] - S.F(F_PX)[ii], dy = S.F(F_GY)[ii] - S.F(F_PY)[ii],
                     dz = S.F(F_GZ)[ii] - S.F(F_PZ)[ii];
        cand_heading = reset_candidate_draw(a, ii, cand);
        const double reach = 7.0 + a.max_v + 1.0;
        cand_want = (c_flags & kFlagDone) || c_sub >= c_n - 1 || c_step + 1 >= a.max_step ||
                    dx * dx + dy * dy + dz * dz < reach * reach;
        if (cand_want) reset_candidate_fetch(a, cand);
    }
    uint2 lut[7];
    {
        const int lo = wv == 0 ? 0 : 7 + (wv - 1) * 6;
#pragma unroll
        for (int j = 0; j < 6; ++j) lut[j] = a.emit_lut[(lo + j) * 64 + lane];
        lut[6] = a.emit_lut[6 * 64 + lane];
    }
    uint32_t *trow = C->tile + lane * kCTileLd;
    if (wv == 3) { trow[0] = 0u; trow[1] = 0u; trow[2] = 0u; }
    double r = 0.0, a0 = 0.0;
    int ret_done = 0, info = UAVENV_INFO_NORMAL, valid = 1, agent_done = 0;
    double energy = 0.0;
    bool did_reset = false, skip = false, head_set = false;
    PreStep pre;
    pre.moved = false;
    if (POLICY) {
        const int tid = (int)threadIdx.x;
        if (!GLDS) {
// ... 610 lines not shown
#pragma unroll
            for (int k = 0; k < 4; ++k) o[k] = grp == st ? os[k] : o[k];
        }
        wave_lds_sync();
        if (have) {
            float2 z = make_float2(0.0f, 0.0f);
            if (v.mode == UAVENV_EVAL_SAC_SAMPLE) z = eval_sac_noise(v.seed, L.e, L.steps);
            const float act0 = uavq::actor_head_one(o[0], o[2], z.x).act * v.bound;
            const int j = L.e % a.U;
            const double a0 = decode_action(RawAction{__float_as_uint(act0), 0u}, UAVENV_ACT_STEER_F32, a.n_actions);
            PreStep P;
            step_pre(a, a0, g, P);
            if (P.moved) g.head = angle_of<true>(g.o.vx, g.o.vy);
            double r = 0.0;
            int ret_done = 0, info = UAVENV_INFO_NORMAL;
            bool head_set = false;
            step_post<MaskT, APF, true>(a, w, APF ? li : L.e, a0, g, P, r, ret_done, info, head_set);
            g.o.n_rem = g.n_total - g.sub_idx;
            L.steps += 1;
            L.ret += r;
            L.energy += fly_power(a.pw, g.o.V, j);
            if (P.moved && g.o.px == P.ox && g.o.py == P.oy && g.o.pz == P.oz) L.collisions += 1;
            if (L.steps <= v.traj_steps) {
                double *p = v.traj_pos + ((size_t)L.e * (v.traj_steps + 1) + L.steps) * 3;
                p[0] = g.o.px; p[1] = g.o.py; p[2] = g.o.pz;
                const float act1 = uavq::actor_head_one(o[1], o[3], z.y).act * v.bound;
                reinterpret_cast<float2 *>(v.traj_act)[(size_t)L.e * v.traj_steps + L.steps - 1] = make_float2(act0, act1);
            }
            const bool trunc = (v.max_steps > 0 && L.steps >= v.max_steps) || L.steps >= L.cap;
            if (g.done || trunc) {
                const int outcome = g.done ? (info == UAVENV_INFO_LOSE ? UAVENV_EVAL_LOSE : UAVENV_EVAL_SUCCESS) : UAVENV_EVAL_TRUNCATED;
                eval_store_record(v, L.e, g, L, outcome, j);
                L.e += v.lanes;
                install = true;
            }
        }
    }
}

static bool is_pow2(int x) { return x > 0 && (x & (x - 1)) == 0; }

static StepArgs base_args(const UavEnv *e)
{
    StepArgs a;
    memset(&a, 0, sizeof(a));
    a.st = e->st;
    a.world_blob = e->world_blob;
    a.world_bytes = e->world_bytes;
    a.aux_off = e->aux_off;
    a.grid_off = e->grid_off;
    a.grid_stride = e->grid_stride;
    a.nb = e->nb;
    a.gn = e->gn;
    a.inv_cell = 1.0 / e->cell;
    a.W = e->cfg.width;
    a.Hbox = e->cfg.h;
    a.apf_b = e->apf_b;
    a.apf_grid = e->apf_grid;
    a.apf_all = e->apf_all;
    a.apf_gn = e->apf_gn;
    a.apf_nz = e->apf_nz;
    a.apf_inv_cell = 1.0 / e->apf_cell;
    a.apf_inv_cz = 1.0 / e->apf_cz;
    a.emit_lut = e->emit_lut;
    a.max_v = e->cfg.max_v;
    a.steer = e->cfg.steering_angle;
    a.pw = PowerParams{e->cfg.power[0], e->cfg.power[1], e->cfg.power[2], e->cfg.power[3],
                       e->cfg.power[4], e->cfg.power[5], e->cfg.power[6], e->cfg.power[7]};
    a.max_step = e->cfg.max_step;
    a.K = e->cfg.max_subgoals;
    a.U = e->cfg.uav_per_env;
    a.N = e->N;
    a.n_actions = e->cfg.n_actions;
    a.bank.start_goal = e->bank_sg;
    a.bank.sub = e->bank_sub;
    a.bank.nsub = e->bank_nsub;
    a.bank.m = e->bank_m;
    a.seed = e->seed;
    a.tick = e->tick;
    a.moved_word = e->moved_word;
    a.moved_value = (uint32_t)(e->tick + 1);
    a.meta = nullptr;
    a.meta_a1 = nullptr;
    a.dbg = e->dbg;
    return a;
}

static int env_int(const char *name, int dflt)
{
    const char *v = getenv(name);
    return v ? atoi(v) : dflt;
}

template <typename K>
static void launch_lds(K kernel, int grid, int block, size_t lds, hipStream_t s, const StepArgs &a)
{
    if (lds > 65536) {
        static std::mutex mu;
        static std::map<std::pair<const void *, int>, size_t> raised;
        int dev = 0;
        (void)hipGetDevice(&dev);
        std::lock_guard<std::mutex> lock(mu);
        size_t &cur = raised[std::make_pair(reinterpret_cast<const void *>(kernel), dev)];
        if (lds > cur) {
            (void)hipFuncSetAttribute(reinterpret_cast<const void *>(kernel), hipFuncAttributeMaxDynamicSharedMemorySize, (int)lds);
            cur = lds;
        }
    }
    hipLaunchKernelGGL(kernel, dim3(grid), dim3(block), lds, s, a);
}

static void launch_geometry(int n, int &block, int &grid)
{
    static const int thr = env_int("UAVENV_BLOCK64_MAX", 131072);
    static const int big = env_int("UAVENV_BLOCK", 256);
    block = n <= thr ? 64 : big;
    grid = (n + block - 1) / block;
    if (grid < 1) grid = 1;
}

struct PendingMeta {
    void *meta;
    const float *a1;
};
static PendingMeta take_step_meta(UavEnv *e)
{
    PendingMeta p{e->step_meta, e->step_meta_a1};
    e->step_meta = nullptr;
    e->step_meta_a1 = nullptr;
    return p;
}

template <typename MaskT>
static void launch_step(const UavEnv *e, const StepArgs &a_in, hipStream_t s)
{
    int block, grid;
    launch_geometry(e->N, block, grid);
    StepArgs a = a_in;
    a.block = block;
    const int obs = e->cfg.obs_dtype;
    const bool apf = e->cfg.apf_enabled == 1;
    static const int tile_env = env_int("UAVENV_TILE_STORE", -1);
    const int tile_from = obs == UAVENV_OBS_PACKED ? 196608 : (obs == UAVENV_OBS_F16 ? 131072 : 32769);
    const bool tile_store = tile_env >= 0 ? tile_env != 0 : e->N >= tile_from;
    const int nw = block / 64;
    a.obsq_off = (e->world_bytes + 15) & ~15;
    int slot = (int)sizeof(ObsWaveLds);
    if (tile_store && kCTileBytes > slot) slot = kCTileBytes;
    slot = (slot + 15) & ~15;
    a.wave_slot = slot;
    a.tile_off = tile_store ? a.obsq_off : -1;
    const size_t lds = (size_t)a.obsq_off + (size_t)nw * slot;
    static const int coop_env = env_int("UAVENV_COOP", -1);
    const bool apf_split_ok = apf && !(a.flags & UAVENV_STEP_APF_LANE) && kApfAgentsPerBlock * a.K <= 65536;
    const bool coop = !(a.flags & UAVENV_STEP_ONE_WAVE) && (coop_env >= 0 ? coop_env != 0 : (e->N <= 49152 && !apf_split_ok));
#define UAV_LAUNCH(KERNEL, GRID, BLOCK, LDS)                                                                        \
    do {                                                                                                            \
        if (apf) {                                                                                                  \
            if (obs == UAVENV_OBS_F16) launch_lds((KERNEL<MaskT, true, OBS_KIND_F16>), GRID, BLOCK, LDS, s, a);     \
            else if (obs == UAVENV_OBS_PACKED) launch_lds((KERNEL<MaskT, true, OBS_KIND_PACKED>), GRID, BLOCK, LDS, s, a); \
            else launch_lds((KERNEL<MaskT, true, OBS_KIND_F32>), GRID, BLOCK, LDS, s, a);                           \
        } else {                                                                                                    \
            if (obs == UAVENV_OBS_F16) launch_lds((KERNEL<MaskT, false, OBS_KIND_F16>), GRID, BLOCK, LDS, s, a);    \
            else if (obs == UAVENV_OBS_PACKED) launch_lds((KERNEL<MaskT, false, OBS_KIND_PACKED>), GRID, BLOCK, LDS, s, a); \
            else launch_lds((KERNEL<MaskT, false, OBS_KIND_F32>), GRID, BLOCK, LDS, s, a);                          \
        }                                                                                                           \
    } while (0)
    if (coop) {
        a.block = 256;
        a.obsq_off = (e->world_bytes + 15) & ~15;
        const size_t clds = (size_t)a.obsq_off + sizeof(CoopLds);
        const int cgrid = (e->N + 63) / 64;
        if (a.pol_local) {
            a.pol_off = (int32_t)((clds + 15) & ~(size_t)15);
            const size_t plds = (size_t)a.pol_off + (size_t)(uavq::kTileF + uavq::kMaxOut * uavq::kHid + uavq::kMaxOut + 64) * 4;
            static const bool stage_vgpr = env_int("UAVENV_STAGE_VGPR", 0) != 0;
            if (a.pol_img && !stage_vgpr) {
                if (cgrid <= 256) launch_lds((k_step_coop<MaskT, false, OBS_KIND_PACKED, true, true, true>), cgrid, 256, plds, s, a);
                else launch_lds((k_step_coop<MaskT, false, OBS_KIND_PACKED, true, false, true>), cgrid, 256, plds, s, a);
            } else if (cgrid <= 256) launch_lds((k_step_coop<MaskT, false, OBS_KIND_PACKED, true, true>), cgrid, 256, plds, s, a);
            else launch_lds((k_step_coop<MaskT, false, OBS_KIND_PACKED, true, false>), cgrid, 256, plds, s, a);
            return;
        }
        UAV_LAUNCH(k_step_coop, cgrid, 256, clds);
        return;
    }
    if (a.pol_local) {
        if (slot < uavq::kPolBytes) slot = uavq::kPolBytes;
        a.wave_slot = slot;
        launch_lds(k_step_polh<MaskT>, grid, 192, (size_t)a.obsq_off + (size_t)slot, s, a);
        return;
    }
    if (apf_split_ok) {
        a.apf_split = 1;
        const int agents_per_block = kApfAgentsPerBlock;
        const size_t albs = ((size_t)((e->nb > 0 ? e->nb : 1) * sizeof(BldApf) + 31) & ~(size_t)31) + 4 * sizeof(ApfSortLds);
        launch_lds(k_apf_adjust, (e->N + agents_per_block - 1) / agents_per_block, 256, albs, s, a);
    }
    UAV_LAUNCH(k_step, grid, block, lds);
#undef UAV_LAUNCH
}

extern "C" {

int uavenv_abi_version(void) { return UAVENV_ABI_VERSION; }
const char *uavenv_last_error(void) { return g_err; }

int uavenv_create(const UavEnvConfig *cfg, UavEnv **out)
{
    if (!cfg || !out) return fail(UAVENV_EINVAL, "null argument");
    if (cfg->abi_version != UAVENV_ABI_VERSION)
        return fail(UAVENV_EINVAL, "abi_version %d != %d", cfg->abi_version, UAVENV_ABI_VERSION);
    if (cfg->n_envs <= 0 || cfg->max_subgoals < 2 || cfg->max_step <= 0)
        return fail(UAVENV_EINVAL, "n_envs/max_subgoals/max_step out of range");
    if (!is_pow2(cfg->uav_per_env) || cfg->uav_per_env > 64)
        return fail(UAVENV_EINVAL, "uav_per_env must be a power of two <= 64 (got %d)", cfg->uav_per_env);
    if (cfg->obs_dtype != UAVENV_OBS_F32 && cfg->obs_dtype != UAVENV_OBS_F16 && cfg->obs_dtype != UAVENV_OBS_PACKED)
        return fail(UAVENV_EINVAL, "obs_dtype");
    int ndev = 0;
    if (hipGetDeviceCount(&ndev) != hipSuccess || ndev <= 0)
        return fail(UAVENV_ENODEV, "no HIP device visible: libuavenv has no CPU fallback");
    if (cfg->device < 0 || cfg->device >= ndev) return fail(UAVENV_EINVAL, "device %d of %d", cfg->device, ndev);
    HIP_TRY(hipSetDevice(cfg->device));
    UavEnv *e = new (std::nothrow) UavEnv();
    if (!e) return fail(UAVENV_ENOMEM, "host alloc");
    e->cfg = *cfg;
    if (e->cfg.n_actions < 2) e->cfg.n_actions = 3;
    e->cell = cfg->cell_size > 0 ? cfg->cell_size : 20.0;
    const long long n64 = (long long)cfg->n_envs * cfg->uav_per_env;
    if (n64 > (1ll << 30)) { delete e; return fail(UAVENV_EINVAL, "too many agents"); }
    e->N = (int)n64;
    const size_t n = (size_t)e->N, npad = (n + 63) & ~(size_t)63;
    const size_t K = (size_t)cfg->max_subgoals;
    size_t bytes = npad * 8 * kNumF64 + npad * 4 * kNumI32 + n * K * 3 * 8 + 256;
    hipError_t er = hipMalloc(&e->slab, bytes);
    if (er != hipSuccess) { delete e; return fail(UAVENV_ENOMEM, "hipMalloc(%zu): %s", bytes, hipGetErrorString(er)); }
    e->slab_bytes = bytes;
    (void)hipMemset(e->slab, 0, bytes);
    unsigned char *p = (unsigned char *)e->slab;
    e->st.npad = npad;
    e->st.f64 = (double *)p; p += npad * 8 * kNumF64;
    e->st.sub = (double *)p; p += n * K * 3 * 8;
    p = (unsigned char *)(((uintptr_t)p + 63) & ~(uintptr_t)63);
    e->st.i32 = (int32_t *)p; p += npad * 4 * kNumI32;
    (void)hipMemset(e->st.I(I_SCN), 0xff, npad * 4);
    {
        std::vector<uint2> lut(25 * 64);
        for (int it = 0; it < 25; ++it)
            for (int l = 0; l < 64; ++l) lut[(size_t)it * 64 + l] = ctile_emit_lut_entry(it, l);
        if (hipMalloc((void **)&e->emit_lut, lut.size() * sizeof(uint2)) != hipSuccess ||
            hipMemcpy(e->emit_lut, lut.data(), lut.size() * sizeof(uint2), hipMemcpyHostToDevice) != hipSuccess) {
            (void)hipFree(e->slab);
            delete e;
            return fail(UAVENV_ENOMEM, "emit table");
        }
    }
    *out = e;
    return UAVENV_OK;
}

int uavenv_destroy(UavEnv *e)
{
// ... 276 lines not shown
int uavenv_replan_begin(UavEnv *e, int32_t first, int32_t count, uint64_t seed, int32_t max_iter, void *plan_stream)
{
    if (!e || first < 0 || count <= 0 || max_iter <= 0) return fail(UAVENV_EINVAL, "uavenv_replan_begin: bad argument");
    if (!e->have_world || e->bank_m <= 0) return fail(UAVENV_EINVAL, "uavenv_replan_begin: no world / no bank to refresh");
    if (first + count > e->bank_m) return fail(UAVENV_EINVAL, "uavenv_replan_begin: rows [%d, %d) outside the bank of %d", first, first + count, e->bank_m);
    if (e->rp_pending) return fail(UAVENV_EINVAL, "uavenv_replan_begin: the previous slice has not been committed");
    HIP_TRY(hipSetDevice(e->cfg.device));
    const int K = e->cfg.max_subgoals;
    if (e->rp_cap < count) {
        HIP_TRY(hipDeviceSynchronize());
        (void)hipFree(e->rp_sg); (void)hipFree(e->rp_sub); (void)hipFree(e->rp_nsub);
        e->rp_sg = e->rp_sub = nullptr; e->rp_nsub = nullptr; e->rp_cap = 0;
        HIP_TRY(hipMalloc((void **)&e->rp_sg, (size_t)count * 6 * 8));
        HIP_TRY(hipMalloc((void **)&e->rp_sub, (size_t)count * K * 3 * 8));
        HIP_TRY(hipMalloc((void **)&e->rp_nsub, (size_t)2 * count * 4));
        e->rp_cap = count;
    }
    if (!e->rp_counters) {
        HIP_TRY(hipMalloc((void **)&e->rp_counters, 16));
        HIP_TRY(hipMemset(e->rp_counters, 0, 16));
    }
    if (!e->rp_done) HIP_TRY(hipEventCreateWithFlags(&e->rp_done, hipEventDisableTiming));
    if (!e->rp_nodes) {
        const char *ev = getenv("UAVENV_REPLAN_WGS");
        const int v = ev ? atoi(ev) : 0;
        e->rp_wgs = v > 0 && v <= 4096 ? v : 128;
        HIP_TRY(hipMalloc(&e->rp_nodes, (size_t)uavenv_rrt_scratch_bytes(e->rp_wgs)));
    }
    if (e->rp_commit_recorded) HIP_TRY(hipStreamWaitEvent((hipStream_t)plan_stream, e->rp_committed, 0));
    int rc = uavenv_rrt_plan_at(e, first, count, nullptr, nullptr, 0, seed, max_iter, 30.0, 5.0, e->rp_sg, e->rp_sub, e->rp_nsub,
                                nullptr, e->rp_nodes, e->rp_wgs, plan_stream);
    if (rc != UAVENV_OK) return fail(rc, "uavenv_replan_begin: planner launch failed");
    HIP_TRY(hipEventRecord(e->rp_done, (hipStream_t)plan_stream));
    e->rp_first = first; e->rp_count = count; e->rp_pending = true; e->rp_world_gen = e->world_gen;
    e->rp_calls += 1; e->rp_rows_planned += count;
    return UAVENV_OK;
}

int uavenv_replan_ready(UavEnv *e)
{
    if (!e) return UAVENV_EINVAL;
    if (!e->rp_pending) return -1;
    const hipError_t q = hipEventQuery(e->rp_done);
    if (q == hipSuccess) return 1;
    if (q == hipErrorNotReady) { (void)hipGetLastError(); return 0; }
    return fail(UAVENV_EHIP, "uavenv_replan_ready: %s", hipGetErrorString(q));
}

int uavenv_replan_commit(UavEnv *e, int32_t force, void *stream)
{
    if (!e) return fail(UAVENV_EINVAL, "null env");
    if (!e->rp_pending) return fail(UAVENV_EINVAL, "uavenv_replan_commit: nothing planned");
    e->rp_pending = false;
    if (e->rp_world_gen != e->world_gen || e->rp_first + e->rp_count > e->bank_m) return UAVENV_OK;
    hipStream_t s = (hipStream_t)stream;
    HIP_TRY(hipStreamWaitEvent(s, e->rp_done, 0));
    const int cap = e->rp_cap, count = e->rp_count;
    int32_t *inuse = e->rp_nsub + cap, *counters = e->rp_counters;
    if (force) {
        inuse = nullptr;
    } else {
        HIP_TRY(hipMemsetAsync(inuse, 0, (size_t)count * 4, s));
        StepArgs a = base_args(e);
        hipLaunchKernelGGL(k_bank_mark, dim3((e->N + 255) / 256 < 1024 ? (e->N + 255) / 256 : 1024), dim3(256), 0, s, a, e->rp_first, count, inuse);
    }
    hipLaunchKernelGGL(k_bank_commit, dim3((count + 3) / 4), dim3(256), 0, s, e->bank_sg, e->bank_sub, e->bank_nsub, e->rp_first, count,
                       e->cfg.max_subgoals, e->rp_sg, e->rp_sub, e->rp_nsub, inuse, counters);
    HIP_TRY(hipGetLastError());
    if (!e->rp_committed) HIP_TRY(hipEventCreateWithFlags(&e->rp_committed, hipEventDisableTiming));
    HIP_TRY(hipEventRecord(e->rp_committed, s));
    e->rp_commit_recorded = true;
    return UAVENV_OK;
}

int uavenv_set_step_meta(UavEnv *e, void *meta_frame_dev, const float *action1_frame_dev)
{
    if (!e) return fail(UAVENV_EINVAL, "null env");
    if ((((uintptr_t)meta_frame_dev) & 15u) != 0) return fail(UAVENV_EINVAL, "uavenv_set_step_meta: records are 16-byte aligned");
    e->step_meta = meta_frame_dev;
    e->step_meta_a1 = meta_frame_dev ? action1_frame_dev : nullptr;
    return UAVENV_OK;
}

int uavenv_set_moved_word(UavEnv *e, uint32_t *dev_word)
{
    if (!e) return fail(UAVENV_EINVAL, "null env");
    e->moved_word = dev_word;
    return UAVENV_OK;
}

uint64_t uavenv_tick(const UavEnv *e) { return e ? e->tick : 0; }

int uavenv_bank_read(UavEnv *e, int32_t first, int32_t count, double *host_sg, double *host_sub, int32_t *host_nsub)
{
    if (!e || first < 0 || count <= 0 || first + count > e->bank_m) return fail(UAVENV_EINVAL, "uavenv_bank_read: rows outside the bank");
    HIP_TRY(hipSetDevice(e->cfg.device));
    HIP_TRY(hipDeviceSynchronize());
    const size_t K3 = (size_t)e->cfg.max_subgoals * 3;
    if (host_sg) HIP_TRY(hipMemcpy(host_sg, e->bank_sg + (size_t)first * 6, (size_t)count * 6 * 8, hipMemcpyDeviceToHost));
    if (host_sub) HIP_TRY(hipMemcpy(host_sub, e->bank_sub + (size_t)first * K3, (size_t)count * K3 * 8, hipMemcpyDeviceToHost));
    if (host_nsub) HIP_TRY(hipMemcpy(host_nsub, e->bank_nsub + first, (size_t)count * 4, hipMemcpyDeviceToHost));
    return UAVENV_OK;
}

int uavenv_replan_stats(UavEnv *e, int64_t *out5)
{
    if (!e || !out5) return fail(UAVENV_EINVAL, "null argument");
    out5[0] = e->rp_calls; out5[1] = e->rp_rows_planned; out5[2] = out5[3] = out5[4] = 0;
    if (e->rp_counters) {
        int32_t c[4] = {0, 0, 0, 0};
        HIP_TRY(hipMemcpy(c, e->rp_counters, 16, hipMemcpyDeviceToHost));
        out5[2] = c[0]; out5[3] = c[1]; out5[4] = c[2];
    }
    return UAVENV_OK;
}

int uavenv_bank_stats(const UavEnv *e, int32_t *m, int32_t *replaced)
{
    if (!e) return fail(UAVENV_EINVAL, "null env");
    if (m) *m = e->bank_m;
    if (replaced) *replaced = e->bank_replaced;
    return UAVENV_OK;
}

int uavenv_reset_all(UavEnv *e, uint64_t seed, void *stream)
{
    if (!e) return fail(UAVENV_EINVAL, "null env");
    if (e->bank_m <= 0) return fail(UAVENV_EINVAL, "uavenv_reset_all: no scenario bank loaded");
    HIP_TRY(hipSetDevice(e->cfg.device));
    e->seed = seed;
    e->tick = 0;
    StepArgs a = base_args(e);
    const int block = 256, grid = (e->N + block - 1) / block;
    if (e->cfg.apf_enabled == 1) hipLaunchKernelGGL(k_reset_all<true>, dim3(grid), dim3(block), 0, (hipStream_t)stream, a);
    else hipLaunchKernelGGL(k_reset_all<false>, dim3(grid), dim3(block), 0, (hipStream_t)stream, a);
    HIP_TRY(hipGetLastError());
    e->tick = 1;
    return UAVENV_OK;
}

int uavenv_set_state(UavEnv *e, int32_t first, int32_t count, const double *kin, const int32_t *step,
                     const int32_t *n_sub, const int32_t *alias, const double *sub)
{
    if (!e || !kin || !step || !n_sub || !sub) return fail(UAVENV_EINVAL, "null argument");
    if (first < 0 || count <= 0 || first + count > e->N) return fail(UAVENV_EINVAL, "range [%d,+%d) of %d", first, count, e->N);
    const int K = e->cfg.max_subgoals;
    for (int c = 0; c < count; ++c)
        if (n_sub[c] < 0 || n_sub[c] > K) return fail(UAVENV_EINVAL, "n_sub[%d]=%d > K=%d", c, n_sub[c], K);
    HIP_TRY(hipSetDevice(e->cfg.device));
    double *d_kin = nullptr, *d_sub = nullptr;
    int32_t *d_i = nullptr;
    const size_t c = (size_t)count;
    HIP_TRY(hipMalloc((void **)&d_kin, c * 8 * 8));
    HIP_TRY(hipMalloc((void **)&d_sub, c * K * 3 * 8));
    HIP_TRY(hipMalloc((void **)&d_i, c * 4 * 3));
    HIP_TRY(hipMemcpy(d_kin, kin, c * 64, hipMemcpyHostToDevice));
    HIP_TRY(hipMemcpy(d_sub, sub, c * K * 24, hipMemcpyHostToDevice));
    HIP_TRY(hipMemcpy(d_i, step, c * 4, hipMemcpyHostToDevice));
    HIP_TRY(hipMemcpy(d_i + c, n_sub, c * 4, hipMemcpyHostToDevice));
    if (alias) HIP_TRY(hipMemcpy(d_i + 2 * c, alias, c * 4, hipMemcpyHostToDevice));
    StepArgs a = base_args(e);
    const int block = 128, grid = (count + block - 1) / block;
    hipLaunchKernelGGL(k_set_state, dim3(grid), dim3(block), 0, 0, a, first, count, d_kin, d_i, d_i + c,
                       alias ? d_i + 2 * c : (const int32_t *)nullptr, d_sub);
    HIP_TRY(hipGetLastError());
    HIP_TRY(hipDeviceSynchronize());
    (void)hipFree(d_kin); (void)hipFree(d_sub); (void)hipFree(d_i);
    return UAVENV_OK;
}

int uavenv_get_state(UavEnv *e, int32_t first, int32_t count, double *out16, double *out_sub, int32_t *out_alias)
{
    if (!e || !out16) return fail(UAVENV_EINVAL, "null argument");
    if (first < 0 || count <= 0 || first + count > e->N) return fail(UAVENV_EINVAL, "range [%d,+%d) of %d", first, count, e->N);
    HIP_TRY(hipSetDevice(e->cfg.device));
    const int K = e->cfg.max_subgoals;
    const size_t c = (size_t)count;
    double *d16 = nullptr, *dsub = nullptr;
    int32_t *dal = nullptr;
    HIP_TRY(hipMalloc((void **)&d16, c * 16 * 8));
    if (out_sub) HIP_TRY(hipMalloc((void **)&dsub, c * K * 24));
    if (out_alias) HIP_TRY(hipMalloc((void **)&dal, c * 4));
    StepArgs a = base_args(e);
    const int block = 128, grid = (count + block - 1) / block;
    HIP_TRY(hipDeviceSynchronize());
    hipLaunchKernelGGL(k_get_state, dim3(grid), dim3(block), 0, 0, a, first, count, d16, dsub, dal);
    HIP_TRY(hipGetLastError());
    HIP_TRY(hipMemcpy(out16, d16, c * 128, hipMemcpyDeviceToHost));
    if (out_sub) HIP_TRY(hipMemcpy(out_sub, dsub, c * K * 24, hipMemcpyDeviceToHost));
    if (out_alias) HIP_TRY(hipMemcpy(out_alias, dal, c * 4, hipMemcpyDeviceToHost));
    (void)hipFree(d16); (void)hipFree(dsub); (void)hipFree(dal);
    return UAVENV_OK;
}

int uavenv_step(UavEnv *e, const void *actions, int32_t action_kind, void *obs, double *reward64, float *reward32,
                uint8_t *ret_done, uint8_t *agent_done, uint8_t *info, uint8_t *valid, double *energy64,
                const uint8_t *active, uint32_t flags, void *stream)
{
    if (!e) return fail(UAVENV_EINVAL, "null env");
    const PendingMeta pm = take_step_meta(e);
    if (!actions) return fail(UAVENV_EINVAL, "null actions");
    if (!e->have_world) return fail(UAVENV_EINVAL, "uavenv_step before uavenv_set_buildings");
    if (action_kind < 0 || action_kind > 2) return fail(UAVENV_EINVAL, "action_kind %d", action_kind);
    if ((flags & UAVENV_STEP_AUTO_RESET) && e->bank_m <= 0)
        return fail(UAVENV_EINVAL, "AUTO_RESET needs a scenario bank (uavenv_load_scenarios)");
    StepArgs a = base_args(e);
    a.actions = actions;
    a.action_kind = action_kind;
    a.obs = obs;
    a.reward64 = reward64;
    a.reward32 = reward32;
    a.ret_done = ret_done;
    a.agent_done = agent_done;
    a.info = info;
    a.valid = valid;
    a.energy64 = energy64;
    a.active = active;
    a.flags = flags;
    a.meta = reinterpret_cast<uint4 *>(pm.meta);
    a.meta_a1 = pm.a1;
    if (e->mask_bytes == 4) launch_step<uint32_t>(e, a, (hipStream_t)stream);
    else launch_step<uint64_t>(e, a, (hipStream_t)stream);
    HIP_TRY(hipGetLastError());
    e->tick += 1;
    return UAVENV_OK;
}

int uavenv_step_policy(UavEnv *e, const UavDqnNet *net, const void *obs_cur, float eps, uint64_t seed, uint64_t counter,
                       int32_t *action_out, void *obs, double *reward64, float *reward32, uint8_t *ret_done, uint8_t *agent_done,
                       uint8_t *info, uint8_t *valid, double *energy64, const uint8_t *active, uint32_t flags, void *stream)
{
    return uavenv_step_policy_img(e, net, obs_cur, eps, seed, counter, action_out, obs, reward64, reward32, ret_done, agent_done, info, valid,
                                  energy64, active, flags, nullptr, stream);
}

int uavenv_step_policy_img(UavEnv *e, const UavDqnNet *net, const void *obs_cur, float eps, uint64_t seed, uint64_t counter,
                           int32_t *action_out, void *obs, double *reward64, float *reward32, uint8_t *ret_done, uint8_t *agent_done,
                           uint8_t *info, uint8_t *valid, double *energy64, const uint8_t *active, uint32_t flags,
                           const float *image_dev, void *stream)
{
    if (!e) return fail(UAVENV_EINVAL, "null env");
    const PendingMeta pm = take_step_meta(e);
    if (!net || !net->local || !obs_cur || !action_out) return fail(UAVENV_EINVAL, "null argument");
    if (!e->have_world) return fail(UAVENV_EINVAL, "uavenv_step_policy before uavenv_set_buildings");
    if ((flags & UAVENV_STEP_AUTO_RESET) && e->bank_m <= 0)
        return fail(UAVENV_EINVAL, "AUTO_RESET needs a scenario bank (uavenv_load_scenarios)");
    static const int coop_env = env_int("UAVENV_COOP", -1);
    const int n2 = net->n_actions + (net->dueling ? 1 : 0);
    const bool one_wave = (flags & UAVENV_STEP_ONE_WAVE) || (coop_env >= 0 ? coop_env == 0 : e->N > 49152);
    const bool shape_ok = e->cfg.apf_enabled != 1 && net->w == uavq::kW && net->hid == uavq::kHid && n2 <= 4 && net->n_actions >= 2 &&
                          net->n_actions == e->cfg.n_actions && (((uintptr_t)net->local) & 15u) == 0;
    const bool coop_packed = !one_wave && e->cfg.obs_dtype == UAVENV_OBS_PACKED && net->mfma_dtype == UAVENV_MFMA_F32 &&
                             (((uintptr_t)obs_cur) & 15u) == 0;
    int blk = 0, grd = 0;
    launch_geometry(e->N, blk, grd);
    const bool wave_f16 = one_wave && blk == 64 && e->N <= 65536 && (e->N & 1) == 0 && e->cfg.obs_dtype == UAVENV_OBS_F16 && net->mfma_dtype == UAVENV_MFMA_F16 &&
                          (((uintptr_t)obs_cur) & 15u) == 0 && env_int("UAVENV_POLH", 1) != 0 &&
                          (size_t)e->world_bytes + 16 + uavq::kPolBytes <= 40960;
    if (!shape_ok || !(coop_packed || wave_f16))
        return fail(UAVENV_EINVAL, "uavenv_step_policy: this env / net takes uavenv_dqn_act + uavenv_step");
    StepArgs a = base_args(e);
    a.actions = action_out;
    a.action_kind = UAVENV_ACT_INDEX_I32;
    a.obs = obs;
    a.reward64 = reward64;
    a.reward32 = reward32;
    a.ret_done = ret_done;
    a.agent_done = agent_done;
    a.info = info;
    a.valid = valid;
    a.energy64 = energy64;
    a.active = active;
    a.flags = flags;
    a.pol_local = net->local;
    a.pol_img = (coop_packed && image_dev && (((uintptr_t)image_dev) & 15u) == 0) ? image_dev : nullptr;
    a.pol_obs = reinterpret_cast<const uint32_t *>(obs_cur);
    a.pol_act = action_out;
    a.pol_dueling = net->dueling;
    a.pol_eps = eps;
    a.pol_seed = seed;
    a.pol_counter = counter;
    a.meta = reinterpret_cast<uint4 *>(pm.meta);
    a.meta_a1 = pm.a1;
    if (e->mask_bytes == 4) launch_step<uint32_t>(e, a, (hipStream_t)stream);
    else launch_step<uint64_t>(e, a, (hipStream_t)stream);
    HIP_TRY(hipGetLastError());
    e->tick += 1;
    return UAVENV_OK;
}

int uavenv_set_debug_buffer(UavEnv *e, unsigned long long *dev_buf)
{
    if (!e) return fail(UAVENV_EINVAL, "null env");
    e->dbg = dev_buf;
    return UAVENV_OK;
}

int uavenv_observe(UavEnv *e, void *obs, void *stream)
{
    if (!e || !obs) return fail(UAVENV_EINVAL, "null argument");
    if (!e->have_world) return fail(UAVENV_EINVAL, "uavenv_observe before uavenv_set_buildings");
    StepArgs a = base_args(e);
    a.obs = obs;
    int block, grid;
    launch_geometry(e->N, block, grid);
    a.block = block;
    const size_t lds = (size_t)e->world_bytes;
    const int obs_kind = e->cfg.obs_dtype;
    hipStream_t s = (hipStream_t)stream;
#define UAV_OBSERVE(MASK)                                                                                        \
    do {                                                                                                         \
        if (obs_kind == UAVENV_OBS_F16) launch_lds((k_observe<MASK, OBS_KIND_F16>), grid, block, lds, s, a);     \
        else if (obs_kind == UAVENV_OBS_PACKED) launch_lds((k_observe<MASK, OBS_KIND_PACKED>), grid, block, lds, s, a); \
        else launch_lds((k_observe<MASK, OBS_KIND_F32>), grid, block, lds, s, a);                                \
    } while (0)
    if (e->mask_bytes == 4) UAV_OBSERVE(uint32_t);
    else UAV_OBSERVE(uint64_t);
#undef UAV_OBSERVE
    HIP_TRY(hipGetLastError());
    return UAVENV_OK;
}

static int threaten_impl(UavEnv *e, const double *xyz, uint8_t *out, int64_t n, void *stream, bool allpairs)
{
    if (!e || !xyz || !out || n < 0) return fail(UAVENV_EINVAL, "null argument");
    if (!e->have_world) return fail(UAVENV_EINVAL, "threaten_rate before uavenv_set_buildings");
    if (n == 0) return UAVENV_OK;
    StepArgs a = base_args(e);
    const int block = 256;
    a.block = block;
    int64_t g = (n + block - 1) / block;
    const int grid = (int)(g > 2048 ? 2048 : g);
    const size_t lds = (size_t)e->world_bytes;
    hipStream_t s = (hipStream_t)stream;
    if (e->mask_bytes == 4) {
        if (allpairs) hipLaunchKernelGGL((k_threaten<uint32_t, true>), dim3(grid), dim3(block), lds, s, a, xyz, out, n);
        else hipLaunchKernelGGL((k_threaten<uint32_t, false>), dim3(grid), dim3(block), lds, s, a, xyz, out, n);
    } else {
        if (allpairs) hipLaunchKernelGGL((k_threaten<uint64_t, true>), dim3(grid), dim3(block), lds, s, a, xyz, out, n);
        else hipLaunchKernelGGL((k_threaten<uint64_t, false>), dim3(grid), dim3(block), lds, s, a, xyz, out, n);
    }
    HIP_TRY(hipGetLastError());
    return UAVENV_OK;
}

int uavenv_geometry(const double *ab, double *angle_out, double *dist_out, int64_t n, void *stream)
{
    if (!ab || n < 0 || (!angle_out && !dist_out)) return UAVENV_EINVAL;
    if (n == 0) return UAVENV_OK;
    hipLaunchKernelGGL(k_geometry, dim3((unsigned)((n + 255) / 256)), dim3(256), 0, (hipStream_t)stream, ab, angle_out, dist_out, n);
    return hipGetLastError() == hipSuccess ? UAVENV_OK : UAVENV_EHIP;
}

int uavenv_threaten_rate(UavEnv *e, const double *xyz, uint8_t *out, int64_t n, void *stream)
{
    return threaten_impl(e, xyz, out, n, stream, false);
}

int uavenv_threaten_rate_allpairs(UavEnv *e, const double *xyz, uint8_t *out, int64_t n, void *stream)
{
    return threaten_impl(e, xyz, out, n, stream, true);
}

int uavenv_eval_episodes(UavEnv *e, const UavDqnNet *net, const UavEvalArgs *args, void *stream)
{
    if (!e || !net || !args) return fail(UAVENV_EINVAL, "null argument");
// ... 212 lines not shown
```

### dqn_based_uav_3d_path_planer_amd/csrc/uavenv_device.hpp

```cpp
#pragma once
#ifndef UAVENV_HOT_PRIO_DEFINED
#define UAVENV_HOT_PRIO_DEFINED
#ifndef UAVENV_HOT_PRIO
#define UAVENV_HOT_PRIO 3
#endif
#define UAV_HOT_PRIO() __builtin_amdgcn_s_setprio(UAVENV_HOT_PRIO)
#endif
#include <hip/hip_runtime.h>
#include <hip/hip_fp16.h>
#include <stdint.h>

namespace uav {

constexpr double kPi = 3.141592653589793;
constexpr double kRad2Deg = 180.0 / 3.141592653589793;
constexpr double kTwoPi = 2.0 * 3.141592653589793;

struct BldLds {
    double cx, cy, thr, H;
};

struct BldAux {
    double rej2[3], acc2[3];
};
// ... 733 lines not shown
#pragma unroll
        for (int it = 0; it < 25; ++it) ctile_emit<F16>(obs_base, first_agent, n_valid, tile, it, true);
    }
    wave_lds_sync();
}

__host__ __device__ __forceinline__ uint4 philox4x32_10(uint4 c, uint2 k)
{
#pragma unroll
    for (int r = 0; r < 10; ++r) {
        const uint64_t p0 = (uint64_t)0xD2511F53u * c.x, p1 = (uint64_t)0xCD9E8D57u * c.z;
        uint32_t hi0 = (uint32_t)(p0 >> 32), lo0 = (uint32_t)p0;
        uint32_t hi1 = (uint32_t)(p1 >> 32), lo1 = (uint32_t)p1;
        c = make_uint4(hi1 ^ c.y ^ k.x, lo1, hi0 ^ c.w ^ k.y, lo0);
        k.x += 0x9E3779B9u;
        k.y += 0xBB67AE85u;
    }
    return c;
}

__device__ __forceinline__ double u53(uint32_t a, uint32_t b)
{
    return ((double)(a >> 5) * 67108864.0 + (double)(b >> 6)) * (1.0 / 9007199254740992.0);
}

struct ReplayPerm {
    uint32_t k[6];
    uint32_t D, la, lb;
    uint32_t n_agents, magic;
};

__host__ __device__ __forceinline__ uint32_t fmix32(uint32_t h)
{
    h ^= h >> 16; h *= 0x85ebca6bu; h ^= h >> 13; h *= 0xc2b2ae35u; h ^= h >> 16;
    return h;
}

__host__ __device__ __forceinline__ ReplayPerm replay_perm(uint64_t seed, uint64_t counter, uint32_t D, uint32_t n_agents)
{
    ReplayPerm p;
    const uint2 key = make_uint2((uint32_t)seed, (uint32_t)(seed >> 32));
    const uint4 a = philox4x32_10(make_uint4(0u, (uint32_t)counter, (uint32_t)(counter >> 32), 0x5a3bu), key);
    const uint4 b = philox4x32_10(make_uint4(1u, (uint32_t)counter, (uint32_t)(counter >> 32), 0x5a3bu), key);
    p.k[0] = a.x; p.k[1] = a.y; p.k[2] = a.z; p.k[3] = a.w; p.k[4] = b.x; p.k[5] = b.y;
    p.D = D;
    uint32_t bits = 2u;
    while (bits < 32u && (1ull << bits) < (uint64_t)D) ++bits;
    p.la = bits >> 1;
    p.lb = bits - p.la;
    p.n_agents = n_agents ? n_agents : 1u;
    const uint64_t mg = (1ull << 32) / p.n_agents;
    p.magic = mg > 0xFFFFFFFFull ? 0xFFFFFFFFu : (uint32_t)mg;
    return p;
}

__device__ __forceinline__ uint32_t replay_perm_apply(const ReplayPerm &p, uint32_t s)
{
    if (p.D <= 1u) return 0u;
    uint32_t x = s < p.D ? s : s % p.D;
    const uint32_t la = p.la, lb = p.lb, ma = (1u << la) - 1u, mb = (1u << lb) - 1u;
    do {
        uint32_t lo = x & ma, hi = x >> la;
#pragma unroll
        for (int r = 0; r < 6; r += 2) {
            lo ^= fmix32(hi ^ p.k[r]) >> (32u - la);
            hi ^= fmix32(lo ^ p.k[r + 1]) >> (32u - lb);
        }
        x = (hi << la) | lo;
    } while (x >= p.D);
    return x;
}

__device__ __forceinline__ void replay_slot_to_frame(const ReplayPerm &p, uint32_t slot, int head, int frames, int &f, int &agent)
{
    uint32_t back = __umulhi(slot, p.magic);
    uint32_t rem = slot - back * p.n_agents;
    if (rem >= p.n_agents) { rem -= p.n_agents; back += 1u; }
    if (rem >= p.n_agents) { rem -= p.n_agents; back += 1u; }
    agent = (int)rem;
    f = head - 1 - (int)back;
    if (f < 0) f += frames;
}

}
```

### dqn_based_uav_3d_path_planer_amd/loop.py

```python
from __future__ import annotations

import ctypes as C

import numpy as np
import torch

from . import _lib
from .learner import FusedDQNLearner
from .replay import DeviceReplayRing


class P2PExchangeError(_lib.UavEnvError):
    """uavenv_loop_run returned UAVENV_EP2P (csrc/p2p.hip: timeout or diverged ranks)."""


class HotLoop:
    def __init__(self, ring: DeviceReplayRing, learner: FusedDQNLearner, batch: int, seed: int, eps: float = 0.1,
                 counter: int = 0, learn_start: int = 0, auto_reset: bool = True, skip_done: bool = None,
                 time_every: int = 0, info: torch.Tensor = None, per=None, sample_lag: int = 0,
                 replan_every: int = 0, replan_count: int = 0, replan_max_iter: int = 10000, gate_updates: bool = False,
                 valid_draws: bool = None):
        if not ring.discrete:
            raise ValueError("HotLoop drives the discrete (DQN-family) path")
        if batch % 64:
            raise ValueError("batch must be a multiple of 64")
        self.lib = _lib.load()
        self.ring, self.learner = ring, learner
        env = ring.env
        if skip_done is None:
            skip_done = env.uav_per_env > 1
        self._partials = learner.new_partials(max(batch, 64))
        cfg = _lib.UavLoopConfig()
        cfg.env = env._h
        cfg.ring = ring._c
        cfg.net = learner.net
        cfg.head, cfg.filled = ring.head, ring.filled
        cfg.batch = int(batch)
        cfg.kind = 0 if learner.kind == "dqn" else 1
        cfg.huber = learner.huber
        cfg.update_loop = learner.update_loop
        cfg.epoch = learner.epoch
        cfg.learn_start = int(learn_start)
        cfg.seed, cfg.counter = int(seed), int(counter)
        cfg.eps, cfg.gamma, cfg.lr = float(eps), learner.gamma, learner.lr
        cfg.beta1, cfg.beta2, cfg.adam_eps = learner.betas[0], learner.betas[1], learner.eps
        cfg.step_flags = (_lib.STEP_AUTO_RESET if auto_reset else 0) | (_lib.STEP_SKIP_DONE if skip_done else 0) | \
            ring.extra_flags
        cfg.partials_dev = self._partials.data_ptr()
        cfg.loss_dev = learner.loss.data_ptr()
        cfg.time_every = int(time_every)
        cfg.sample_lag = int(sample_lag)
        cfg.replan_every, cfg.replan_count, cfg.replan_max_iter = int(replan_every), int(replan_count), int(replan_max_iter)
        self._moved = torch.zeros(1, dtype=torch.int32, device=env.device) if gate_updates else None
        if self._moved is not None:
            cfg.moved_dev = self._moved.data_ptr()
        if info is not None:
            assert info.dtype == torch.uint8 and tuple(info.shape) == (ring.frames, env.N) and info.is_contiguous()
            cfg.info_dev = info.data_ptr()
        self._info = info
        if getattr(learner, "_p2p", None) is not None:
            cfg.p2p = learner._p2p
        elif getattr(learner, "_coll", None) is not None:
            cfg.coll = learner._coll
            cfg.raw_dev = learner.raw.data_ptr()
        self._per = per
        if per is not None:
            if per.capacity != ring.frames * env.N or per._c.rot != 0:
                raise ValueError("the DevicePER must cover the ring's frames * N slots in slot order (tree_order=False)")
            d, b = env.device, max(int(batch), 64)
            self._per_bufs = (torch.zeros(b, dtype=torch.int64, device=d), torch.zeros(b + (b + 255) // 256, dtype=torch.float64, device=d),
                              torch.zeros(b, dtype=torch.float32, device=d), torch.zeros(b, dtype=torch.float32, device=d),
                              torch.zeros((b, 2), dtype=torch.int32, device=d))
            cfg.per = per._c
            cfg.per_alpha, cfg.per_beta, cfg.per_beta_inc = per.alpha, per.beta, per.beta_inc
            cfg.per_eps, cfg.per_clip = per.epsilon, per.clip
            cfg.per_slots_dev, cfg.per_prio_dev, cfg.per_w_dev, cfg.per_abs_dev, cfg.per_idx_dev = \
                (t.data_ptr() for t in self._per_bufs)
        if valid_draws is None:
            valid_draws = bool(skip_done) and not auto_reset
        self._draw_idx = None
        if valid_draws and per is None and batch > 0:
            if not skip_done:
                raise ValueError("valid_draws needs skip_done (with auto-reset every stored row is valid)")
            self._draw_idx = torch.zeros((int(batch), 2), dtype=torch.int32, device=env.device)
            cfg.per_idx_dev = self._draw_idx.data_ptr()
        self._h = C.c_void_p()
        _lib.check(self.lib.uavenv_loop_create(C.byref(cfg), C.byref(self._h)), "uavenv_loop_create")
        self.counter = int(counter)
        self.batch = int(batch)
        self._seen = (ring.head, ring.filled, learner.epoch)

    def in_sync(self, batch: int = None) -> bool:
        return (self._seen == (self.ring.head, self.ring.filled, self.learner.epoch) and
                (batch is None or int(batch) == self.batch))

    def close(self):
        if getattr(self, "_h", None) is not None and self._h.value:
            self.lib.uavenv_loop_destroy(self._h)
            self._h = C.c_void_p()

    def __del__(self):
        try:
            self.close()
        except Exception:
            pass

    def set_eps(self, eps: float):
        _lib.check(self.lib.uavenv_loop_set_eps(self._h, float(eps)), "uavenv_loop_set_eps")

    def run(self, n_steps: int):
        s = torch.cuda.current_stream(self.ring.env.device).cuda_stream
        rc = self.lib.uavenv_loop_run(self._h, int(n_steps), s)
        if rc == _lib.EP2P:
            self._sync_cursor()
            raise P2PExchangeError("the peer-to-peer gradient exchange raised its sticky error "
                                   f"({self.learner.p2p_status()}): this rank's weights are frozen; fall back to the "
                                   "collective (FusedDQNLearner.enable_coll) and re-broadcast the weights")
        _lib.check(rc, "uavenv_loop_run")
        self._sync_cursor()

    def _sync_cursor(self):
        cur = _lib.UavLoopCursor()
        _lib.check(self.lib.uavenv_loop_get(self._h, C.byref(cur)), "uavenv_loop_get")
        self.ring.head, self.ring.filled = cur.head, cur.filled
        self.learner.epoch = cur.epoch
        self.counter = int(cur.counter)
        self._seen = (cur.head, cur.filled, cur.epoch)
        if self._per is not None:
            beta = C.c_double(0.0)
            _lib.check(self.lib.uavenv_loop_get_per(self._h, C.byref(beta)), "uavenv_loop_get_per")
            self._per.beta = float(beta.value)
            self._per.n_entries = self.ring.filled * self.ring.env.N
            self._per._dirty = True

    def step_times_ms(self, max_n: int = 4096) -> np.ndarray:
        buf = np.zeros(max_n, dtype=np.float32)
        n = C.c_int32(0)
        _lib.check(self.lib.uavenv_loop_step_times(self._h, buf.ctypes.data, max_n, C.byref(n)), "uavenv_loop_step_times")
        return buf[:n.value].copy()



class SACHotLoop:

    def __init__(self, ring: DeviceReplayRing, learners, batch: int, seed: int, act1_plane: torch.Tensor, counter: int = 0,
                 info: torch.Tensor = None, is_train: bool = True, auto_reset: bool = True, skip_done: bool = True,
                 exchange: str = None, spin_limit: int = 0, pers=None, check_every: int = 64, gate_updates: bool = False,
                 valid_draws: bool = None):
        if ring.discrete or not ring.env.packed:
            raise ValueError("SACHotLoop drives the continuous-action path on a packed ring")
        env = ring.env
        U = env.uav_per_env
        if len(learners) != U or U > _lib.SAC_LOOP_MAX_SLOTS:
            raise ValueError("one FusedSACLearner per UAV slot (at most %d)" % _lib.SAC_LOOP_MAX_SLOTS)
        if batch % 64:
            raise ValueError("batch must be a multiple of 64")
        self.lib = _lib.load()
        self.ring, self.learners = ring, list(learners)
        L0 = self.learners[0]
        for L in self.learners:
            if (L.gamma, L.tau, L.action_bound, L.actor_lr, L.critic_lr, L.alpha_lr, L.target_entropy) != \
               (L0.gamma, L0.tau, L0.action_bound, L0.actor_lr, L0.critic_lr, L0.alpha_lr, L0.target_entropy):
                raise ValueError("the SAC slots must share their hyper-parameters")
        d = env.device
        n_envs = env.N // U
        self._draws = torch.zeros((U * batch, 2), dtype=torch.int32, device=d)
        self._noise = torch.zeros(int(self.lib.uavenv_sac_loop_noise_floats(U, n_envs, int(batch))), dtype=torch.float32, device=d)
        cfg = _lib.UavSacLoopConfig()
        cfg.env = env._h
        cfg.ring = ring._c
        assert act1_plane.dtype == torch.float32 and tuple(act1_plane.shape) == (ring.frames, env.N) and act1_plane.is_contiguous()
        cfg.act1_plane = act1_plane.data_ptr()
        ring.attach_action1(act1_plane)
        if info is not None:
            assert info.dtype == torch.uint8 and tuple(info.shape) == (ring.frames, env.N) and info.is_contiguous()
            cfg.info_dev = info.data_ptr()
        cfg.n_slots, cfg.batch = U, int(batch)
        cfg.head, cfg.filled = ring.head, ring.filled
        cfg.is_train = 1 if is_train else 0
        cfg.valid_draws = int(bool(skip_done) and not auto_reset) if valid_draws is None else int(bool(valid_draws))
        cfg.seed, cfg.counter = int(seed), int(counter)
        cfg.beta1, cfg.beta2, cfg.adam_eps = L0.beta1, L0.beta2, L0.adam_eps
        cfg.gamma, cfg.tau, cfg.action_bound = L0.gamma, L0.tau, L0.action_bound
        cfg.actor_lr, cfg.critic_lr, cfg.alpha_lr, cfg.target_entropy = L0.actor_lr, L0.critic_lr, L0.alpha_lr, L0.target_entropy
        cfg.step_flags = (_lib.STEP_AUTO_RESET if auto_reset else 0) | (_lib.STEP_SKIP_DONE if skip_done else 0) | ring.extra_flags
        cfg.draws_dev, cfg.noise_dev = self._draws.data_ptr(), self._noise.data_ptr()
        self._td = []
        for j, L in enumerate(self.learners):
            sl = cfg.slot[j]
            _, pc, pa = L._scratch(int(batch))
            sl.partials_critic, sl.partials_actor = pc.data_ptr(), pa.data_ptr()
            sl.nets = L._nets
            sl.m_actor, sl.v_actor, sl.alpha_mv = L._blocks[1].data_ptr(), L._blocks[2].data_ptr(), L._alpha_mv.data_ptr()
            sl.m1, sl.v1, sl.m2, sl.v2 = (L._cblocks[k].data_ptr() for k in (4, 5, 6, 7))
            sl.scalars = L._scalars.data_ptr()
            sl.epoch, sl.adam_steps = L.epoch, L.adam_steps
            self._td.append(torch.empty(2 * int(batch), dtype=torch.float32, device=d))
            sl.td_dev = self._td[-1].data_ptr()
        self._pers = list(pers) if pers is not None and any(p is not None for p in pers) else None
        if self._pers is not None:
            if len(self._pers) != U or any(p is None for p in self._pers):
                raise ValueError("prioritised replay in the SAC loop: one DevicePER per UAV slot, all slots or none")
            p0 = self._pers[0]
            cfg.per_alpha, cfg.per_beta_inc, cfg.per_eps, cfg.per_clip = p0.alpha, p0.beta_inc, p0.epsilon, p0.clip
            self._per_bufs = []
            for j, p in enumerate(self._pers):
                if p.capacity != ring.frames * n_envs or p._c.rot != 0:
                    raise ValueError("each slot's DevicePER must cover ring.frames * n_envs slots in slot order (tree_order=False)")
                if (p.alpha, p.beta_inc, p.epsilon, p.clip) != (p0.alpha, p0.beta_inc, p0.epsilon, p0.clip):
# ... 99 lines not shown
```

### include/uavenv.h

```cpp
#ifndef UAVENV_H
#define UAVENV_H

#include <stdint.h>

#ifdef __cplusplus
extern "C" {
#endif

#define UAVENV_ABI_VERSION 5
#define UAVENV_OBS_DIM 100
#define UAVENV_MAX_BUILDINGS 64

#define UAVENV_OK 0
#define UAVENV_EINVAL (-22)
#define UAVENV_ENOMEM (-12)
#define UAVENV_EHIP (-5)
#define UAVENV_ENODEV (-19)
#define UAVENV_EP2P (-70)

#define UAVENV_INFO_NORMAL 0
#define UAVENV_INFO_SUCCESS 1
#define UAVENV_INFO_LOSE 2
#define UAVENV_INFO_SKIPPED 3

// ... 9 lines not shown
#define UAVENV_STEP_AUTO_RESET 1u
#define UAVENV_STEP_SKIP_DONE 2u
#define UAVENV_STEP_NO_OBS 4u
#define UAVENV_STEP_ONE_WAVE 8u
#define UAVENV_STEP_APF_LANE 16u

typedef struct UavEnv UavEnv;

typedef struct UavEnvConfig {
    int32_t abi_version;
    int32_t device;
    int32_t n_envs;
    int32_t uav_per_env;
    int32_t max_subgoals;
    int32_t max_step;
    int32_t apf_enabled;
    int32_t obs_dtype;
    int32_t n_actions;
    int32_t reserved0;
    double len, width, h;
    double max_v;
    double steering_angle;
    double power[8];
    double cell_size;
} UavEnvConfig;

int uavenv_abi_version(void);
const char *uavenv_last_error(void);
int uavenv_create(const UavEnvConfig *cfg, UavEnv **out);
int uavenv_destroy(UavEnv *env);
int uavenv_num_agents(const UavEnv *env);

int uavenv_set_buildings(UavEnv *env, const double *host_cxcyczRH, const double *host_vxyz, int32_t nb);

int uavenv_load_scenarios(UavEnv *env, const double *host_start_goal, const double *host_subgoals,
                          const int32_t *host_nsub, int32_t m);
int uavenv_plan_scenarios(UavEnv *env, int32_t m, uint64_t seed, int32_t max_iter, void *stream);
int uavenv_bank_stats(const UavEnv *env, int32_t *m, int32_t *replaced);
int uavenv_replan_begin(UavEnv *env, int32_t first, int32_t count, uint64_t seed, int32_t max_iter, void *plan_stream);
int uavenv_replan_ready(UavEnv *env);
int uavenv_replan_commit(UavEnv *env, int32_t force, void *stream);
int uavenv_replan_stats(UavEnv *env, int64_t *out5);
int uavenv_set_moved_word(UavEnv *env, uint32_t *dev_word);
uint64_t uavenv_tick(const UavEnv *env);
int uavenv_bank_read(UavEnv *env, int32_t first, int32_t count, double *host_start_goal, double *host_subgoals, int32_t *host_nsub);
int uavenv_rrt_plan(UavEnv *env, int32_t m, const double *start_goal_dev, const double *uniforms_dev,
                    int32_t stream_len, uint64_t seed, int32_t max_iter, double step_size, double obstacle_step,
                    double *out_start_goal_dev, double *out_sub_dev, int32_t *out_nsub_dev, int32_t *out_iters_dev,
                    void *stream);
int uavenv_reset_all(UavEnv *env, uint64_t seed, void *stream);

int uavenv_set_state(UavEnv *env, int32_t first, int32_t count, const double *kin, const int32_t *step,
                     const int32_t *n_sub, const int32_t *alias, const double *sub);
int uavenv_get_state(UavEnv *env, int32_t first, int32_t count, double *out16, double *out_sub, int32_t *out_alias);

int uavenv_step(UavEnv *env, const void *actions_dev, int32_t action_kind, void *obs_dev, double *reward64_dev,
                float *reward32_dev, uint8_t *ret_done_dev, uint8_t *agent_done_dev, uint8_t *info_dev,
                uint8_t *valid_dev, double *energy64_dev, const uint8_t *active_dev, uint32_t flags, void *stream);
struct UavDqnNet;
int uavenv_step_policy(UavEnv *env, const struct UavDqnNet *net, const void *obs_cur_dev, float eps, uint64_t seed,
                       uint64_t counter, int32_t *action_out_dev, void *obs_dev, double *reward64_dev, float *reward32_dev,
                       uint8_t *ret_done_dev, uint8_t *agent_done_dev, uint8_t *info_dev, uint8_t *valid_dev,
                       double *energy64_dev, const uint8_t *active_dev, uint32_t flags, void *stream);
int uavenv_set_debug_buffer(UavEnv *env, unsigned long long *dev_buf);
int uavenv_observe(UavEnv *env, void *obs_dev, void *stream);
int uavenv_threaten_rate(UavEnv *env, const double *xyz_dev, uint8_t *out_dev, int64_t n, void *stream);
int uavenv_geometry(const double *ab_dev, double *angle_out_dev, double *dist_out_dev, int64_t n, void *stream);
int uavenv_threaten_rate_allpairs(UavEnv *env, const double *xyz_dev, uint8_t *out_dev, int64_t n, void *stream);

typedef struct UavReplayRing {
    void *obs;
    void *action;
    float *reward;
    uint8_t *done;
    uint8_t *valid;
    int32_t frames;
    int32_t n_agents;
    int32_t obs_dtype;
    int32_t action_is_index;
    void *meta;
} UavReplayRing;
#define UAVENV_META_BYTES 16
int uavenv_set_step_meta(UavEnv *env, void *meta_frame_dev, const float *action1_frame_dev);

int uavenv_replay_sample(const UavReplayRing *ring, int32_t head, int32_t filled, int32_t batch, uint64_t seed,
                         uint64_t counter, void *obs_b, void *next_obs_b, void *action_b, float *reward_b,
                         float *done_b, float *valid_b, void *stream);

int uavenv_obs_unpack(const void *packed_dev, int64_t n, void *out_dev, int32_t out_dtype, void *stream);

int uavenv_replay_draw(int32_t frames, int32_t n_agents, int32_t head, int32_t filled, int32_t batch, uint64_t seed,
                       uint64_t counter, int32_t *frame_agent_out_dev, void *stream);
#define UAVENV_DRAW_MAX_TRIES 8
int uavenv_replay_draw_valid(int32_t frames, int32_t n_envs, int32_t head, int32_t filled, int32_t batch, int32_t n_slots,
                             int32_t uav_per_env, int32_t first_slot, const uint8_t *valid_dev, int32_t max_tries, uint64_t seed,
                             uint64_t counter, int32_t *frame_env_out_dev, void *stream);

int uavenv_select_actions(const float *q_dev, int32_t n, int32_t n_actions, float eps, uint64_t seed,
                          uint64_t counter, int32_t *index_out_dev, float *steer_out_dev, void *stream);

typedef struct UavPer {
    double *prio;
    double *chunk_sum;
    double *chunk_prefix;
    int64_t capacity;
    int64_t rot;
    double *group_sum;
} UavPer;

int uavenv_per_num_chunks(int64_t capacity);
int uavenv_per_rotation(int64_t capacity);
int uavenv_per_rebuild(const UavPer *per, void *stream);
int uavenv_per_sample(const UavPer *per, int32_t batch, const double *draws_dev, uint64_t seed, uint64_t counter,
                      int64_t *out_slot_dev, double *out_prio_dev, void *stream);
int uavenv_per_set(const UavPer *per, const int64_t *slots_dev, const double *abs_err_dev, int32_t n, double epsilon,
                   double alpha, double clip, void *stream);
int uavenv_per_fill(const UavPer *per, int64_t first, int64_t count, double priority, const uint8_t *valid_dev,
                    void *stream);
int uavenv_per_fill_frame(const UavPer *per, int64_t first, int64_t count, double priority, const uint8_t *valid_dev,
                          int64_t retire_first, void *stream);
int uavenv_per_fill_frame_strided(const UavPer *per, int64_t first, int64_t count, double priority, const uint8_t *valid_dev,
                                  int64_t valid_stride, int64_t retire_first, void *stream);
int uavenv_per_rebuild_frame(const UavPer *per, int64_t first, int64_t count, double priority, const uint8_t *valid_dev,
                             int64_t retire_first, void *stream);
int uavenv_per_set_f32(const UavPer *per, const int64_t *slots_dev, const float *abs_err_dev, int32_t n, double epsilon,
                       double alpha, double clip, void *stream);
int uavenv_per_set_f32_gated(const UavPer *per, const int64_t *slots_dev, const float *abs_err_dev, int32_t n, double epsilon,
                             double alpha, double clip, const uint32_t *go_word_dev, uint32_t go_value, void *stream);
int uavenv_per_weights(const UavPer *per, const int64_t *slots_dev, double *prio_dev, int32_t batch,
                       int64_t n_entries, double beta, int32_t n_agents, float *is_weights_out_dev,
                       int32_t *frame_agent_out_dev, void *stream);

#define UAVENV_MFMA_F32 0
#define UAVENV_MFMA_F16 1
typedef struct UavDqnNet {
    float *local;
    float *target;
    float *m, *v;
    int32_t w, hid, n_actions, dueling;
    int32_t mfma_dtype;
    int32_t reserved0;
} UavDqnNet;

int uavenv_dqn_num_params(const UavDqnNet *net);
int uavenv_dqn_set_debug_buffer(unsigned long long *dev_buf);
int uavenv_dqn_partial_stride(const UavDqnNet *net);
int uavenv_dqn_partial_rows(int32_t batch);
int uavenv_dqn_grad(const UavReplayRing *ring, int32_t head, int32_t filled, int32_t batch, uint64_t seed,
                    uint64_t counter, const int32_t *explicit_idx_dev, const UavDqnNet *net, int32_t kind, float gamma,
                    int32_t huber, float *partials_dev, void *stream);
int uavenv_dqn_grad_w(const UavReplayRing *ring, int32_t head, int32_t filled, int32_t batch, uint64_t seed,
                      uint64_t counter, const int32_t *explicit_idx_dev, const UavDqnNet *net, int32_t kind, float gamma,
                      int32_t huber, const float *is_weights_dev, float *abs_td_out_dev, float *partials_dev, void *stream);
int uavenv_dqn_reduce(const UavDqnNet *net, const float *partials_dev, int32_t n_partials, float *raw_out_dev,
                      void *stream);
int uavenv_dqn_adam(const UavDqnNet *net, const float *raw_dev, float lr, float beta1, float beta2, float eps,
                    int32_t step_t, int32_t hard_update, float *loss_out_dev, void *stream);
int uavenv_dqn_reduce_adam_gated(const UavDqnNet *net, const float *partials, int32_t n_partials, float lr, float beta1,
                                 float beta2, float eps, int32_t step_t, int32_t hard_update, float *loss_out, float *raw_out,
                                 const uint32_t *go_word_dev, uint32_t go_value, void *stream);
int uavenv_dqn_reduce_adam(const UavDqnNet *net, const float *partials_dev, int32_t n_partials, float lr, float beta1,
                           float beta2, float eps, int32_t step_t, int32_t hard_update, float *loss_out_dev,
                           float *raw_out_dev, void *stream);
int uavenv_dqn_act(const UavDqnNet *net, const void *obs_dev, int32_t obs_dtype, int32_t n, float eps, uint64_t seed,
                   uint64_t counter, int32_t *index_out_dev, float *steer_out_dev, float *q_out_dev, void *stream);

// ... 35 lines not shown
#define UAVENV_EVAL_SAC_SAMPLE 1
typedef struct UavSacEvalArgs {
    int32_t n, first;
    const double *start_goal;
    const double *sub;
    const int32_t *nsub;
    int32_t m;
    int32_t max_steps;
    const double *v0;
    uint64_t seed;
    const float *const *actors;
    int32_t n_actors;
    float action_bound;
    int32_t mode;
    int32_t traj_steps;
    UavEvalRecord *records;
    double *traj_pos;
    float *traj_act;
    int32_t max_workgroups;
    int32_t reserved0;
} UavSacEvalArgs;
int uavenv_eval_episodes_sac(UavEnv *env, const UavSacEvalArgs *args, void *stream);
int uavenv_eval_noise_fill(uint64_t seed, int32_t n, int32_t steps, float *out_dev, void *stream);

#define UAVENV_P2P_HANDLE_BYTES 64
#define UAVENV_P2P_ERR_TIMEOUT 1
#define UAVENV_P2P_ERR_DIVERGED 2
typedef struct UavP2P UavP2P;
int uavenv_p2p_create(int32_t world, int32_t rank, int32_t bucket_floats, UavP2P **out);
int uavenv_p2p_handle(UavP2P *p2p, void *handle_out_host);
int uavenv_p2p_can_reach(int32_t device, int32_t peer_device);
int uavenv_p2p_connect(UavP2P *p2p, const void *all_handles_host);
int uavenv_p2p_destroy(UavP2P *p2p);
int uavenv_p2p_configure(UavP2P *p2p, int32_t check_every, int32_t spin_limit);
int uavenv_p2p_errors(UavP2P *p2p, int32_t *timeouts_out);
const uint32_t *uavenv_p2p_error_word(const UavP2P *p2p);
int uavenv_p2p_status(UavP2P *p2p, int32_t synchronise, int32_t *out4);
int uavenv_p2p_inject_fault(UavP2P *p2p, int32_t code);
int uavenv_p2p_allreduce(UavP2P *p2p, float *buf_dev, int64_t count, void *stream);
#define UAVENV_P2P_CHECK_MAX_BLOCKS 40
int uavenv_p2p_check_blocks(UavP2P *p2p, const float *const *blocks_dev, const int32_t *n_floats, int32_t n_blocks, void *stream);
int uavenv_dqn_reduce_p2p(const UavDqnNet *net, const float *partials_dev, int32_t n_partials, UavP2P *p2p, void *stream);
int uavenv_dqn_adam_p2p(const UavDqnNet *net, UavP2P *p2p, float lr, float beta1, float beta2, float eps, int32_t step_t,
                        int32_t hard_update, float *loss_out_dev, float *raw_out_dev, void *stream);

#define UAVENV_COLL_ID_BYTES 128
typedef struct UavColl UavColl;
const char *uavenv_coll_last_error(void);
int uavenv_coll_unique_id(const char *rccl_path, void *id_out_host);
int uavenv_coll_create(const char *rccl_path, int32_t world, int32_t rank, const void *id_host, UavColl **out);
int uavenv_coll_destroy(UavColl *coll);
int uavenv_coll_allreduce_sum(UavColl *coll, float *buf_dev, int64_t n, void *stream);

typedef struct UavLoop UavLoop;
typedef struct UavLoopConfig {
    UavEnv *env;
    UavReplayRing ring;
    UavDqnNet net;
    int32_t head, filled;
    int32_t batch;
    int32_t kind;
    int32_t huber;
    int32_t update_loop;
    int32_t epoch;
    int32_t learn_start;
    uint64_t seed, counter;
    float eps, gamma, lr, beta1, beta2, adam_eps;
    uint32_t step_flags;
    float *partials_dev;
    float *loss_dev;
    uint8_t *info_dev;
    UavP2P *p2p;
    int32_t time_every;
    int32_t sample_lag;
    UavColl *coll;
    float *raw_dev;
    UavPer per;
    double per_alpha, per_beta, per_beta_inc, per_eps, per_clip;
    int64_t *per_slots_dev;
    double *per_prio_dev;
    float *per_w_dev;
    float *per_abs_dev;
    int32_t *per_idx_dev;
    int32_t replan_every, replan_count, replan_max_iter, reserved1;
    uint32_t *moved_dev;
} UavLoopConfig;
typedef struct UavLoopCursor {
    int32_t head, filled, epoch, reserved0;
    uint64_t counter;
} UavLoopCursor;

int uavenv_loop_create(const UavLoopConfig *cfg, UavLoop **out);
int uavenv_loop_destroy(UavLoop *loop);
int uavenv_loop_set_eps(UavLoop *loop, float eps);
int uavenv_loop_run(UavLoop *loop, int32_t n_steps, void *stream);
int uavenv_loop_get(const UavLoop *loop, UavLoopCursor *out);
int uavenv_loop_get_per(const UavLoop *loop, double *beta_out);
int uavenv_loop_step_times(UavLoop *loop, float *ms_out, int32_t max_n, int32_t *n_out);

#define UAVENV_SAC_CRITIC_IN 102
#define UAVENV_SAC_ACTOR_PARAMS 6724
#define UAVENV_SAC_CRITIC_PARAMS 10882
#define UAVENV_SAC_ACTOR_STRIDE 6728
#define UAVENV_SAC_CRITIC_STRIDE 21768
typedef struct UavSacNets {
    float *actor, *critic1, *critic2, *target1, *target2;
    float *log_alpha;
} UavSacNets;
typedef struct UavSacBatch {
    const void *obs_packed;
    const int32_t *idx_s, *idx_n;
    const int32_t *draws;
    int32_t n_agents, uav_per_env, slot, frames;
    const float *act0, *act1, *reward;
    const uint8_t *done, *valid;
    const float *eps;
    int32_t batch;
    int32_t tiles_per_wg;
    const float *is_weights;
    float *abs_td_out;
    const void *meta;
    float *td_scratch;
} UavSacBatch;
typedef struct UavSacAdam {
    float lr, beta1, beta2, eps, bias_correction1, bias_correction2_sqrt;
    float tau;
    float grad_scale;
    const uint32_t *skip_word;
    const uint32_t *go_word;
    uint32_t go_value, reserved0;
} UavSacAdam;
int uavenv_sac_act(const float *actor, const void *obs_packed, int32_t first_row, int32_t row_stride, int32_t count,
                   const float *eps, float action_bound, float *act0, float *act1, void *stream);
int uavenv_sac_partial_rows(int32_t batch);
int uavenv_sac_partial_rows_n(int32_t batch, int32_t n_slots, int32_t tiles_per_wg);
const char *uavenv_sac_last_error(void);
int uavenv_sac_set_debug_buffer(unsigned long long *dev_buf);
#define UAVENV_SAC_LOOP_MAX_SLOTS 8
int uavenv_sac_act_multi(const float *const *actors, const void *obs_packed, const int32_t *first_rows, int32_t row_stride,
                         int32_t count, const float *const *eps, float action_bound, float *act0, float *act1, int32_t n,
                         void *stream);
int uavenv_sac_critic_grad_multi(const UavSacNets *nets, const UavSacBatch *batches, int32_t n, float gamma, float action_bound,
                                 float *const *partials, void *stream);
int uavenv_sac_actor_grad_multi(const UavSacNets *nets, const UavSacBatch *batches, int32_t n, float action_bound,
                                float *const *partials, void *stream);
int uavenv_sac_critic_adam_multi(const UavSacNets *nets, float *const *partials, int32_t rows, float *const *m1, float *const *v1,
                                 float *const *m2, float *const *v2, const UavSacAdam *h, float *const *losses_out, int32_t n,
                                 void *stream);
int uavenv_sac_actor_adam_multi(const UavSacNets *nets, float *const *partials, int32_t rows, int32_t batch, float *const *m,
                                float *const *v, float *const *alpha_mv, const UavSacAdam *h, float alpha_lr, float target_entropy,
                                float *const *scalars_out, int32_t n, void *stream);
int uavenv_sac_critic_grad(const UavSacNets *nets, const UavSacBatch *batch, float gamma, float action_bound, float *partials,
                           void *stream);
int uavenv_sac_critic_adam(const UavSacNets *nets, const float *partials, int32_t rows, float *m1, float *v1, float *m2, float *v2,
                           const UavSacAdam *h, float *losses_out, void *stream);
int uavenv_sac_reduce(const float *partials, int32_t rows, int32_t stride, float *raw, void *stream);
int uavenv_sac_actor_grad(const UavSacNets *nets, const UavSacBatch *batch, float action_bound, float *partials, void *stream);
int uavenv_sac_actor_adam(const UavSacNets *nets, const float *partials, int32_t rows, int32_t batch, float *m, float *v,
                          float *alpha_mv, const UavSacAdam *h, float alpha_lr, float target_entropy, float *scalars_out,
                          void *stream);

typedef struct UavSacLoopSlot {
    UavSacNets nets;
    float *m_actor, *v_actor, *alpha_mv;
    float *m1, *v1, *m2, *v2;
    float *scalars;
    float *partials_critic, *partials_actor;
    int32_t epoch, adam_steps;
    UavPer per;
    int64_t *per_slots_dev;
    double *per_prio_dev;
// ... 50 lines not shown
```

Before: 628.1 million.

## Stage replay-batch gather inside the fused env-step kernel for the DQN learner

Adds a staged gather in which the fused step_policy kernel, with spare blocks, pre-gathers the sampled replay rows (packed obs, next obs, records) into a per-tile staging buffer. The gradient kernel then reads these contiguous tiles instead of doing scattered ring loads. Rows that the current step is still writing are flagged fresh and re-read from the ring. The aim is to hide the replay gather latency behind env stepping. The cost is extra kernel complexity, a staging buffer, and a default-on eligibility heuristic based on CU count.

```diff
diff --git a/dqn_based_uav_3d_path_planer_amd/_lib.py b/dqn_based_uav_3d_path_planer_amd/_lib.py
--- a/dqn_based_uav_3d_path_planer_amd/_lib.py
+++ b/dqn_based_uav_3d_path_planer_amd/_lib.py
@@ -25,7 +25,7 @@
 
 SYMBOLS = (
     "uavenv_abi_version", "uavenv_last_error", "uavenv_create", "uavenv_destroy", "uavenv_num_agents",
-    "uavenv_set_buildings", "uavenv_load_scenarios", "uavenv_plan_scenarios", "uavenv_bank_stats", "uavenv_replan_begin", "uavenv_replan_ready", "uavenv_replan_commit", "uavenv_replan_stats", "uavenv_bank_read", "uavenv_set_moved_word", "uavenv_set_step_meta", "uavenv_tick", "uavenv_dqn_reduce_adam_gated", "uavenv_per_set_f32_gated", "uavenv_rrt_plan", "uavenv_reset_all", "uavenv_set_state", "uavenv_get_state",
+    "uavenv_set_buildings", "uavenv_load_scenarios", "uavenv_plan_scenarios", "uavenv_bank_stats", "uavenv_replan_begin", "uavenv_replan_ready", "uavenv_replan_commit", "uavenv_replan_stats", "uavenv_bank_read", "uavenv_set_moved_word", "uavenv_set_step_meta", "uavenv_set_step_gather", "uavenv_tick", "uavenv_dqn_reduce_adam_gated", "uavenv_per_set_f32_gated", "uavenv_rrt_plan", "uavenv_reset_all", "uavenv_set_state", "uavenv_get_state",
     "uavenv_step", "uavenv_step_policy", "uavenv_set_debug_buffer", "uavenv_observe", "uavenv_threaten_rate", "uavenv_threaten_rate_allpairs", "uavenv_geometry",
     "uavenv_replay_sample", "uavenv_obs_unpack", "uavenv_replay_draw", "uavenv_replay_draw_valid", "uavenv_select_actions",
     "uavenv_dqn_num_params", "uavenv_dqn_partial_stride", "uavenv_dqn_partial_rows", "uavenv_dqn_set_debug_buffer", "uavenv_dqn_grad", "uavenv_dqn_grad_w", "uavenv_dqn_reduce", "uavenv_dqn_adam", "uavenv_dqn_reduce_adam", "uavenv_dqn_act",
@@ -62,6 +62,14 @@
     ]
 
 
+STAGED_TILE_BYTES, STAGED_FRESH, GATHER_PLAIN_STORES = 11776, 0x80000000, 1
+
+
+class UavStepGather(C.Structure):
+    _fields_ = [("ring", UavReplayRing), ("head", C.c_int32), ("filled", C.c_int32), ("batch", C.c_int32),
+                ("flags", C.c_uint32), ("seed", C.c_uint64), ("counter", C.c_uint64), ("staged_dev", C.c_void_p)]
+
+
 class UavDqnNet(C.Structure):
     _fields_ = [("local", C.c_void_p), ("target", C.c_void_p), ("m", C.c_void_p), ("v", C.c_void_p),
                 ("w", C.c_int32), ("hid", C.c_int32), ("n_actions", C.c_int32), ("dueling", C.c_int32),
@@ -117,12 +125,12 @@
                 ("per_eps", C.c_double), ("per_clip", C.c_double),
                 ("per_slots_dev", C.c_void_p), ("per_prio_dev", C.c_void_p), ("per_w_dev", C.c_void_p),
                 ("per_abs_dev", C.c_void_p), ("per_idx_dev", C.c_void_p),
-                ("replan_every", C.c_int32), ("replan_count", C.c_int32), ("replan_max_iter", C.c_int32), ("reserved1", C.c_int32),
+                ("replan_every", C.c_int32), ("replan_count", C.c_int32), ("replan_max_iter", C.c_int32), ("staged_gather", C.c_int32),
                 ("moved_dev", C.c_void_p)]
 
 
 class UavLoopCursor(C.Structure):
-    _fields_ = [("head", C.c_int32), ("filled", C.c_int32), ("epoch", C.c_int32), ("reserved0", C.c_int32),
+    _fields_ = [("head", C.c_int32), ("filled", C.c_int32), ("epoch", C.c_int32), ("staged_passes", C.c_int32),
                 ("counter", C.c_uint64)]
 
 
@@ -226,6 +234,8 @@
     lib.uavenv_set_moved_word.argtypes = [vp, vp]
     lib.uavenv_set_step_meta.restype = C.c_int
     lib.uavenv_set_step_meta.argtypes = [vp, vp, vp]
+    lib.uavenv_set_step_gather.restype = C.c_int
+    lib.uavenv_set_step_gather.argtypes = [vp, C.POINTER(UavStepGather)]
     lib.uavenv_tick.restype = C.c_uint64
     lib.uavenv_tick.argtypes = [vp]
     lib.uavenv_bank_read.restype = C.c_int
diff --git a/dqn_based_uav_3d_path_planer_amd/csrc/dqn_internal.hpp b/dqn_based_uav_3d_path_planer_amd/csrc/dqn_internal.hpp
--- a/dqn_based_uav_3d_path_planer_amd/csrc/dqn_internal.hpp
+++ b/dqn_based_uav_3d_path_planer_amd/csrc/dqn_internal.hpp
@@ -27,4 +27,9 @@
                            uint8_t *info, uint8_t *valid, double *energy64, const uint8_t *active, uint32_t flags,
                            const float *image_dev, void *stream);
 
+int uav_dqn_grad_staged(const UavReplayRing *ring, int32_t head, int32_t filled, int32_t batch, uint64_t seed, uint64_t counter,
+                        const int32_t *explicit_idx, const UavDqnNet *net, int32_t kind, float gamma, int32_t huber,
+                        const float *is_weights, float *abs_td_out, float *partials, const float *image_dev, const void *staged_dev,
+                        void *stream);
+
 }
diff --git a/dqn_based_uav_3d_path_planer_amd/csrc/learner.hip b/dqn_based_uav_3d_path_planer_amd/csrc/learner.hip
--- a/dqn_based_uav_3d_path_planer_amd/csrc/learner.hip
+++ b/dqn_based_uav_3d_path_planer_amd/csrc/learner.hip
@@ -29,6 +29,7 @@
     const float *is_w;
     float *abs_td;
     const float *img;
+    const uint32_t *staged;
 };
 
 #ifdef UAVENV_PHASE_PROFILE
@@ -772,7 +773,7 @@
     for (int k = 0; k < 4; ++k) { A.acc[0][k] += csc[k]; A.acc[1][k] += cw2[k]; }
 }
 
-template <bool FIRST, int SPLIT, bool GLDS>
+template <bool FIRST, int SPLIT, bool GLDS, bool STAGED>
 __device__ __forceinline__ void grad_tile_packed8(const GradArgs &g, const GradLdsP &L, float *qn_lds, int tile, bool more,
                                                   GradAcc8 &A)
 {
@@ -785,6 +786,8 @@
     floatx4 vW[kStageIters];
     SplitScRegs vS;
     float pw[4] = {0, 0, 0, 0}, pb2 = 0.0f;
+    uint2 pair = make_uint2(0u, 0u);
+    if (STAGED) pair = *reinterpret_cast<const uint2 *>(g.staged + (size_t)tile * kStagedTileDwords + kStagedIdx + 2 * (strip * 16 + r));
     if (FIRST) {
         if (GLDS) img_glds(grp == 0 ? L.W1l : L.W1t, g.img + (grp == 0 ? 0 : kSplitF), strip);
         else if (g.img) img_issue(vW, g.img + (grp == 0 ? 0 : kSplitF));
@@ -797,6 +800,33 @@
     }
     L_STAMP2(0);
     const int smp = tile * kTile + strip * 16 + r;
+    PRow R;
+    int p_act = 0;
+    float p_rew = 0.0f, p_w = 1.0f;
+    uint32_t raw_done = 0u, raw_valid = 1u;
+    if (STAGED) {
+        const uint32_t *blk = g.staged + (size_t)tile * kStagedTileDwords;
+        const int si = strip * 16 + r;
+        prow_load(R, blk + (grp == 0 ? 0 : kStagedRowsN) + si * kPackedDwords);
+        uint4 m = make_uint4(0u, 0u, 0u, 0u);
+        if (grp == 0) m = reinterpret_cast<const uint4 *>(blk + kStagedRec)[si];
+        L_STAMP2(1);
+        if (pair.x & kStagedFresh) {
+            const int f = (int)min(pair.x & ~kStagedFresh, (uint32_t)g.ring.frames - 1u), agent = (int)min(pair.y, (uint32_t)g.ring.n_agents - 1u);
+            int fn = f + 1;
+            if (fn >= g.ring.frames) fn = 0;
+            const uint32_t row_s = (uint32_t)f * (uint32_t)g.ring.n_agents + (uint32_t)agent;
+            const uint32_t row_n = (uint32_t)fn * (uint32_t)g.ring.n_agents + (uint32_t)agent;
+            prow_load(R, obs + (size_t)(grp == 0 ? row_s : row_n) * kPackedDwords);
+            if (grp == 0) m = reinterpret_cast<const uint4 *>(g.ring.meta)[row_s];
+        }
+        if (grp == 0) {
+            p_act = (int)m.y;
+            p_rew = __uint_as_float(m.z);
+            raw_done = m.w & 0xffu;
+            raw_valid = (m.w >> 8) & 0xffu;
+        }
+    } else {
     int f, agent;
     if (g.explicit_idx) {
         f = g.explicit_idx[2 * smp];
@@ -809,14 +839,11 @@
     const uint32_t row_s = (uint32_t)f * (uint32_t)g.ring.n_agents + (uint32_t)agent;
     const uint32_t row_n = (uint32_t)fn * (uint32_t)g.ring.n_agents + (uint32_t)agent;
     L_STAMP2(1);
-    PRow R;
     prow_load(R, obs + (size_t)(grp == 0 ? row_s : row_n) * kPackedDwords);
-    int p_act = 0;
-    float p_rew = 0.0f, p_w = 1.0f;
-    uint32_t raw_done = 0u, raw_valid = 1u;
     if (grp == 0) {
         load_transition(g.ring, row_s, p_act, p_rew, raw_done, raw_valid);
         p_w = g.is_w ? g.is_w[smp] : 1.0f;
+    }
     }
     L_STAMP(6);
     if (FIRST) {
@@ -938,7 +965,7 @@
     if (more) __syncthreads();
 }
 
-template <int SPLIT, bool GLDS = false>
+template <int SPLIT, bool GLDS = false, bool STAGED = false>
 __global__ void __launch_bounds__(512) k_dqn_grad_packed8(Grad2Args ga)
 {
     UAV_HOT_PRIO();
@@ -969,9 +996,9 @@
     L_STAMP(0);
     const int step = (int)gridDim.x;
     int tile = (int)blockIdx.x;
-    grad_tile_packed8<true, SPLIT, GLDS>(g, L, qn_lds, tile, tile + step < ga.n_tiles, A);
+    grad_tile_packed8<true, SPLIT, GLDS, STAGED>(g, L, qn_lds, tile, tile + step < ga.n_tiles, A);
     for (tile += step; tile < ga.n_tiles; tile += step)
-        grad_tile_packed8<false, SPLIT, GLDS>(g, L, qn_lds, tile, tile + step < ga.n_tiles, A);
+        grad_tile_packed8<false, SPLIT, GLDS, STAGED>(g, L, qn_lds, tile, tile + step < ga.n_tiles, A);
     L_STAMP(5);
     float *out = g.partials + (size_t)blockIdx.x * ga.stride;
     const int oW2 = kHid * kW + kHid, ob2 = oW2 + n2 * kHid;
@@ -2111,6 +2138,15 @@
                         uint64_t counter, const int32_t *explicit_idx, const UavDqnNet *net, int32_t kind, float gamma,
                         int32_t huber, const float *is_weights, float *abs_td_out, float *partials, const float *image_dev, void *stream)
 {
+    return uav_dqn_grad_staged(ring, head, filled, batch, seed, counter, explicit_idx, net, kind, gamma, huber, is_weights, abs_td_out,
+                               partials, image_dev, nullptr, stream);
+}
+
+int uav_dqn_grad_staged(const UavReplayRing *ring, int32_t head, int32_t filled, int32_t batch, uint64_t seed,
+                        uint64_t counter, const int32_t *explicit_idx, const UavDqnNet *net, int32_t kind, float gamma,
+                        int32_t huber, const float *is_weights, float *abs_td_out, float *partials, const float *image_dev,
+                        const void *staged_dev, void *stream)
+{
     if (!ring || !ring->obs || !ring->action || !ring->reward || !ring->done || !partials || !net_ok(net) || !net->target)
         return UAVENV_EINVAL;
     if (batch <= 0 || batch % kTile != 0 || ring->frames < 2 || head < 0 || head >= ring->frames) return UAVENV_EINVAL;
@@ -2134,12 +2170,16 @@
     g.is_w = is_weights;
     g.abs_td = abs_td_out;
     g.img = (image_dev && (((uintptr_t)image_dev) & 15u) == 0) ? image_dev : nullptr;
+    g.staged = reinterpret_cast<const uint32_t *>(staged_dev);
+    if (staged_dev && (explicit_idx || is_weights || !ring->meta || !g.img || (((uintptr_t)staged_dev) & 127u) != 0)) return UAVENV_EINVAL;
     ga.n_tiles = batch / kTile;
     ga.stride = uavenv_dqn_partial_stride(net);
     const int grid = uavenv_dqn_partial_rows(batch);
     hipStream_t s = (hipStream_t)stream;
     const bool small = net->n_actions + (net->dueling ? 1 : 0) <= 4;
     int rc;
+    if (g.staged && !(net->mfma_dtype == UAVENV_MFMA_F32 && ring->obs_dtype == UAVENV_OBS_PACKED && small && getenv("UAVENV_GRAD_4WAVES") == nullptr))
+        return UAVENV_EINVAL;
     if (net->mfma_dtype == UAVENV_MFMA_F16) {
         if (!small || ring->obs_dtype == UAVENV_OBS_F32) return UAVENV_EINVAL;
         static const bool four_waves_h = getenv("UAVENV_GRAD_4WAVES") != nullptr;
@@ -2163,12 +2203,18 @@
                                         hipFuncAttributeMaxDynamicSharedMemorySize, (int)kGradP8Lds) != hipSuccess ||
                     hipFuncSetAttribute(reinterpret_cast<const void *>(&k_dqn_grad_packed8<2, true>),
                                         hipFuncAttributeMaxDynamicSharedMemorySize, (int)kGradP8Lds) != hipSuccess ||
+                    hipFuncSetAttribute(reinterpret_cast<const void *>(&k_dqn_grad_packed8<2, true, true>),
+                                        hipFuncAttributeMaxDynamicSharedMemorySize, (int)kGradP8Lds) != hipSuccess ||
                     hipFuncSetAttribute(reinterpret_cast<const void *>(&k_dqn_grad_packed8<0>),
                                         hipFuncAttributeMaxDynamicSharedMemorySize, (int)kGradP8Lds) != hipSuccess)
                     return UAVENV_EHIP;
                 attr8 = true;
             }
-            if (dw1_f32) hipLaunchKernelGGL(k_dqn_grad_packed8<0>, dim3(grid), dim3(512), kGradP8Lds, s, ga);
+            if (g.staged && (dw1_f32 || !dw1_b || stage_vgpr)) return UAVENV_EINVAL;
+            if (g.staged) {
+                hipLaunchKernelGGL((k_dqn_grad_packed8<2, true, true>), dim3(grid), dim3(512), kGradP8Lds, s, ga);
+            }
+            else if (dw1_f32) hipLaunchKernelGGL(k_dqn_grad_packed8<0>, dim3(grid), dim3(512), kGradP8Lds, s, ga);
             else if (dw1_b && g.img && !stage_vgpr) hipLaunchKernelGGL((k_dqn_grad_packed8<2, true>), dim3(grid), dim3(512), kGradP8Lds, s, ga);
             else if (dw1_b) hipLaunchKernelGGL(k_dqn_grad_packed8<2>, dim3(grid), dim3(512), kGradP8Lds, s, ga);
             else hipLaunchKernelGGL(k_dqn_grad_packed8<1>, dim3(grid), dim3(512), kGradP8Lds, s, ga);
diff --git a/dqn_based_uav_3d_path_planer_amd/csrc/loop.hip b/dqn_based_uav_3d_path_planer_amd/csrc/loop.hip
--- a/dqn_based_uav_3d_path_planer_amd/csrc/loop.hip
+++ b/dqn_based_uav_3d_path_planer_amd/csrc/loop.hip
@@ -29,6 +29,9 @@
     int32_t replan_next = 0, bank_m = 0;
     uint64_t replan_gen = 0;
     float *img = nullptr;
+    void *staged = nullptr;
+    uint32_t gather_flags = 0;
+    int32_t staged_passes = 0;
 };
 
 static int replan_tick(UavLoop *l, hipStream_t s)
@@ -88,8 +91,29 @@
             if (hipMalloc((void **)&l->img, 2 * (size_t)UAVENV_DQN_IMAGE_FLOATS * sizeof(float)) != hipSuccess) { delete l; return UAVENV_ENOMEM; }
         }
     }
+    {
+        const bool valid_draws = (cfg->step_flags & UAVENV_STEP_SKIP_DONE) != 0 && cfg->per_idx_dev && cfg->ring.valid;
+        const bool can = cfg->sample_lag == 0 && !l->per && !valid_draws && cfg->batch > 0 && cfg->ring.meta &&
+                         cfg->ring.obs_dtype == UAVENV_OBS_PACKED && cfg->net.mfma_dtype == UAVENV_MFMA_F32 && cfg->net.w == 100 &&
+                         cfg->net.hid == 64 && cfg->net.n_actions + (cfg->net.dueling ? 1 : 0) <= 4 && cfg->net.target;
+        if (cfg->staged_gather && !can) { uavenv_loop_destroy(l); return UAVENV_EINVAL; }
+        int dev = 0, cus = 0;
+        (void)hipGetDevice(&dev);
+        (void)hipDeviceGetAttribute(&cus, hipDeviceAttributeMultiprocessorCount, dev);
+        const bool beside = (cfg->ring.n_agents + 63) / 64 + cfg->batch / 64 <= 2 * cus && !cfg->p2p && !cfg->coll && cfg->replan_every <= 0;
+        const char *knob = getenv("UAVENV_STAGED_GATHER");
+        const bool want = knob ? atoi(knob) != 0 : (cfg->staged_gather == 1 || (cfg->staged_gather == 2 && beside));
+        const bool forms = l->img && !getenv("UAVENV_NO_FUSED_ACT") && !getenv("UAVENV_GRAD_4WAVES") && !getenv("UAVENV_DW1_F32") &&
+                           !getenv("UAVENV_DW1_SPLITA") && !(getenv("UAVENV_STAGE_VGPR") && atoi(getenv("UAVENV_STAGE_VGPR")) != 0);
+        if (want && can && forms) {
+            if (hipMalloc(&l->staged, (size_t)(cfg->batch / 64) * UAVENV_STAGED_TILE_BYTES) != hipSuccess) { uavenv_loop_destroy(l); return UAVENV_ENOMEM; }
+            l->gather_flags = getenv("UAVENV_GATHER_PLAIN") && atoi(getenv("UAVENV_GATHER_PLAIN")) != 0 ? UAVENV_GATHER_PLAIN_STORES : 0u;
+            const int delay = getenv("UAVENV_GATHER_DELAY") ? atoi(getenv("UAVENV_GATHER_DELAY")) : 18;
+            l->gather_flags |= ((uint32_t)(delay < 0 ? 0 : delay > 255 ? 255 : delay)) << UAVENV_GATHER_DELAY_SHIFT;
+        }
+    }
     if (cfg->sample_lag != 0) {
-        if (cfg->sample_lag != 1 || l->per) { delete l; return UAVENV_EINVAL; }
+        if (cfg->sample_lag != 1 || l->per) { uavenv_loop_destroy(l); return UAVENV_EINVAL; }
         if (hipStreamCreateWithFlags(&l->aux, hipStreamNonBlocking) != hipSuccess ||
             hipEventCreateWithFlags(&l->ev_grad, hipEventDisableTiming) != hipSuccess ||
             hipEventCreateWithFlags(&l->ev_join, hipEventDisableTiming) != hipSuccess) {
@@ -133,6 +157,7 @@
     }
     for (hipEvent_t e : {l->ev_grad, l->ev_join}) if (e) (void)hipEventDestroy(e);
     if (l->img) (void)hipFree(l->img);
+    if (l->staged) (void)hipFree(l->staged);
     delete l;
     return UAVENV_OK;
 }
@@ -157,7 +182,7 @@
     out->head = l->head;
     out->filled = l->filled;
     out->epoch = l->epoch;
-    out->reserved0 = 0;
+    out->staged_passes = l->staged_passes;
     out->counter = l->counter;
     return UAVENV_OK;
 }
@@ -218,6 +243,10 @@
         uint8_t *info_t = c.info_dev ? c.info_dev + (size_t)t * n : nullptr;
         uint8_t *valid_t = R.valid ? R.valid + (size_t)t * n : nullptr;
         void *meta_t = R.meta ? (unsigned char *)R.meta + (size_t)t * n * UAVENV_META_BYTES : nullptr;
+        const int filled_nxt = l->filled < R.frames - 1 ? l->filled + 1 : l->filled;
+        const bool stage_now = l->staged && l->fuse_act && !lag && c.batch > 0 &&
+                               (int64_t)filled_nxt * (int64_t)n >= (int64_t)(c.learn_start > c.batch ? c.learn_start : c.batch);
+        bool staged_done = false;
         if (l->fuse_act) {
             if (timed) {
                 e0 = take_event(l);
@@ -226,10 +255,21 @@
             }
             rc = uavenv_set_step_meta(c.env, meta_t, nullptr);
             if (rc != UAVENV_OK) return rc;
+            if (stage_now) {
+                UavStepGather rq;
+                rq.ring = R;
+                rq.head = nxt; rq.filled = filled_nxt; rq.batch = c.batch;
+                rq.flags = l->gather_flags;
+                rq.seed = c.seed; rq.counter = l->counter;
+                rq.staged_dev = l->staged;
+                rc = uavenv_set_step_gather(c.env, &rq);
+                if (rc != UAVENV_OK) return rc;
+            }
             rc = uavenv_step_policy_img(c.env, &c.net, obs_t, c.eps, c.seed, l->counter, act_t, obs_n, nullptr, R.reward + (size_t)t * n,
                                         R.done + (size_t)t * n, nullptr, info_t, valid_t, nullptr, nullptr, c.step_flags, l->img, s);
             if (rc == UAVENV_EINVAL) l->fuse_act = false;
             else if (rc != UAVENV_OK) return rc;
+            else staged_done = stage_now;
         }
         if (!l->fuse_act) {
             rc = uavenv_dqn_act(&c.net, obs_t, R.obs_dtype, R.n_agents, c.eps, c.seed, l->counter, act_t, nullptr, nullptr, s);
@@ -285,10 +325,11 @@
                 rc = uavenv_dqn_grad_img(&R, l->head, l->filled, c.batch, c.seed, l->counter, c.per_idx_dev, &c.net, c.kind, c.gamma,
                                          c.huber, nullptr, nullptr, c.partials_dev, l->img, s);
             } else {
-                rc = uavenv_dqn_grad_img(&R, l->head, l->filled, c.batch, c.seed, l->counter, nullptr, &c.net, c.kind, c.gamma,
-                                         c.huber, nullptr, nullptr, c.partials_dev, l->img, s);
-            }
-            if (rc != UAVENV_OK) return rc;
+                rc = uav_dqn_grad_staged(&R, l->head, l->filled, c.batch, c.seed, l->counter, nullptr, &c.net, c.kind, c.gamma,
+                                         c.huber, nullptr, nullptr, c.partials_dev, l->img, staged_done ? l->staged : nullptr, s);
+            }
+            if (rc != UAVENV_OK) return rc;
+            if (staged_done) l->staged_passes += 1;
             if (l->prof) tp2 = std::chrono::steady_clock::now();
             l->epoch += 1;
             const int hard = l->epoch % c.update_loop == 0 ? 1 : 0;
diff --git a/dqn_based_uav_3d_path_planer_amd/csrc/uavenv.hip b/dqn_based_uav_3d_path_planer_amd/csrc/uavenv.hip
--- a/dqn_based_uav_3d_path_planer_amd/csrc/uavenv.hip
+++ b/dqn_based_uav_3d_path_planer_amd/csrc/uavenv.hip
@@ -65,6 +65,15 @@
     const double *sub;
     const int32_t *nsub;
     int32_t m;
+};
+
+struct GatherArgs {
+    ReplayPerm perm;
+    const uint32_t *obs;
+    const uint4 *meta;
+    uint32_t *staged;
+    int32_t head, frames, n_agents, n_tiles;
+    uint32_t flags;
 };
 
 struct StepArgs {
@@ -110,6 +119,7 @@
     uint32_t moved_value;
     uint4 *meta;
     const float *meta_a1;
+    GatherArgs gather;
 };
 
 struct UavEnv {
@@ -137,6 +147,7 @@
     uint32_t *moved_word = nullptr;
     void *step_meta = nullptr;
     const float *step_meta_a1 = nullptr;
+    GatherArgs step_gather = GatherArgs();
     double *rp_sg = nullptr, *rp_sub = nullptr;
     int32_t *rp_nsub = nullptr;
     int32_t *rp_counters = nullptr;
@@ -985,6 +996,47 @@
     k_step_body<MaskT, false, OBS_KIND_F16, true>(a);
 }
 
+__device__ __forceinline__ void gather_role(const GatherArgs &G, int tile)
+{
+    const int tid = (int)threadIdx.x;
+    uint32_t *blk = G.staged + (size_t)tile * kStagedTileDwords;
+    const int f_new = G.head == 0 ? G.frames - 1 : G.head - 1;
+    const bool plain = (G.flags & UAVENV_GATHER_PLAIN_STORES) != 0;
+    for (uint32_t d = (G.flags >> UAVENV_GATHER_DELAY_SHIFT) & 0xffu; d; --d) __builtin_amdgcn_s_sleep(8);
+    uavq::uintx4 v[3];
+    bool take[3];
+#pragma unroll
+    for (int k = 0; k < 3; ++k) {
+        const int q = tid + 256 * k;
+        const bool live = q < 704;
+        const int qq = live ? q : 703;
+        const int kind = qq < 320 ? 0 : (qq < 640 ? 1 : 2);
+        const int c = qq - 320 * kind;
+        const int smp = kind == 2 ? c : c / 5, part = kind == 2 ? 0 : c - 5 * smp;
+        int f, agent;
+        replay_slot_to_frame(G.perm, replay_perm_apply(G.perm, (uint32_t)(tile * 64 + smp)), G.head, G.frames, f, agent);
+        const bool fresh = f == f_new;
+        int fr = kind == 1 ? f + 1 : f;
+        if (fr >= G.frames) fr = 0;
+        const uint32_t row = (uint32_t)fr * (uint32_t)G.n_agents + (uint32_t)agent;
+        const uavq::uintx4 *src = kind == 2 ? reinterpret_cast<const uavq::uintx4 *>(G.meta) + row
+                                            : reinterpret_cast<const uavq::uintx4 *>(G.obs + (size_t)row * kPackedDwords) + part;
+        take[k] = live && !fresh;
+        v[k] = uavq::uintx4{0u, 0u, 0u, 0u};
+        if (take[k]) v[k] = *src;
+        if (kind == 2 && live)
+            *reinterpret_cast<uint2 *>(blk + kStagedIdx + 2 * c) = make_uint2((uint32_t)f | (fresh ? kStagedFresh : 0u), (uint32_t)agent);
+    }
+#pragma unroll
+    for (int k = 0; k < 3; ++k) {
+        uavq::uintx4 *dst = reinterpret_cast<uavq::uintx4 *>(blk) + (tid + 256 * k);
+        if (take[k]) {
+            if (plain) *dst = v[k];
+            else __builtin_nontemporal_store(v[k], dst);
+        }
+    }
+}
+
 struct CoopLds {
     double cand[16][64];
     int32_t cand_n[64], cand_scn[64];
@@ -998,6 +1050,13 @@
 template <typename MaskT, bool APF, int OBS, bool POLICY = false, bool PAHEAD = false, bool GLDS = false>
 __global__ void __launch_bounds__(256) k_step_coop(StepArgs a)
 {
+    if (POLICY && GLDS) {
+        const int role_tile = (int)blockIdx.x - ((a.N + 63) >> 6);
+        if (role_tile >= 0) {
+            gather_role(a.gather, role_tile);
+            return;
+        }
+    }
     UAV_HOT_PRIO();
     extern __shared__ __align__(16) unsigned char smem[];
     const DevState &S = a.st;
@@ -1774,6 +1833,7 @@
     a.moved_value = (uint32_t)(e->tick + 1);
     a.meta = nullptr;
     a.meta_a1 = nullptr;
+    a.gather = GatherArgs();
     a.dbg = e->dbg;
     return a;
 }
@@ -1821,6 +1881,12 @@
     e->step_meta = nullptr;
     e->step_meta_a1 = nullptr;
     return p;
+}
+static GatherArgs take_step_gather(UavEnv *e)
+{
+    const GatherArgs g = e->step_gather;
+    e->step_gather = GatherArgs();
+    return g;
 }
 
 template <typename MaskT>
@@ -1868,8 +1934,9 @@
             const size_t plds = (size_t)a.pol_off + (size_t)(uavq::kTileF + uavq::kMaxOut * uavq::kHid + uavq::kMaxOut + 64) * 4;
             static const bool stage_vgpr = env_int("UAVENV_STAGE_VGPR", 0) != 0;
             if (a.pol_img && !stage_vgpr) {
-                if (cgrid <= 256) launch_lds((k_step_coop<MaskT, false, OBS_KIND_PACKED, true, true, true>), cgrid, 256, plds, s, a);
-                else launch_lds((k_step_coop<MaskT, false, OBS_KIND_PACKED, true, false, true>), cgrid, 256, plds, s, a);
+                const int ggrid = cgrid + (a.gather.staged ? a.gather.n_tiles : 0);
+                if (cgrid <= 256) launch_lds((k_step_coop<MaskT, false, OBS_KIND_PACKED, true, true, true>), ggrid, 256, plds, s, a);
+                else launch_lds((k_step_coop<MaskT, false, OBS_KIND_PACKED, true, false, true>), ggrid, 256, plds, s, a);
             } else if (cgrid <= 256) launch_lds((k_step_coop<MaskT, false, OBS_KIND_PACKED, true, true>), cgrid, 256, plds, s, a);
             else launch_lds((k_step_coop<MaskT, false, OBS_KIND_PACKED, true, false>), cgrid, 256, plds, s, a);
             return;
@@ -2312,6 +2379,33 @@
     return UAVENV_OK;
 }
 
+int uavenv_set_step_gather(UavEnv *e, const UavStepGather *r)
+{
+    if (!e) return fail(UAVENV_EINVAL, "null env");
+    e->step_gather = GatherArgs();
+    if (!r) return UAVENV_OK;
+    const UavReplayRing &R = r->ring;
+    if (!R.obs || !R.meta || !r->staged_dev || R.obs_dtype != UAVENV_OBS_PACKED || R.frames < 3 || R.n_agents != e->N)
+        return fail(UAVENV_EINVAL, "uavenv_set_step_gather: a packed ring of this env's agents with records, and a staged buffer");
+    if ((((uintptr_t)R.obs | (uintptr_t)R.meta) & 15u) != 0 || (((uintptr_t)r->staged_dev) & 127u) != 0)
+        return fail(UAVENV_EINVAL, "uavenv_set_step_gather: rows and records are 16-byte aligned, the staged buffer 128-byte");
+    if (r->head < 0 || r->head >= R.frames || r->filled <= 0 || r->filled > R.frames - 1 || r->batch <= 0 || r->batch % 64 != 0 ||
+        r->batch / 64 > 65536 || (uint64_t)R.frames * (uint64_t)R.n_agents >= (1ull << 32))
+        return fail(UAVENV_EINVAL, "uavenv_set_step_gather: cursor / batch out of range");
+    GatherArgs g;
+    g.perm = replay_perm(r->seed, r->counter, (uint32_t)r->filled * (uint32_t)R.n_agents, (uint32_t)R.n_agents);
+    g.obs = reinterpret_cast<const uint32_t *>(R.obs);
+    g.meta = reinterpret_cast<const uint4 *>(R.meta);
+    g.staged = reinterpret_cast<uint32_t *>(r->staged_dev);
+    g.head = r->head;
+    g.frames = R.frames;
+    g.n_agents = R.n_agents;
+    g.n_tiles = r->batch / 64;
+    g.flags = r->flags;
+    e->step_gather = g;
+    return UAVENV_OK;
+}
+
 int uavenv_set_moved_word(UavEnv *e, uint32_t *dev_word)
 {
     if (!e) return fail(UAVENV_EINVAL, "null env");
@@ -2429,6 +2523,7 @@
 {
     if (!e) return fail(UAVENV_EINVAL, "null env");
     const PendingMeta pm = take_step_meta(e);
+    if (take_step_gather(e).staged) return fail(UAVENV_EINVAL, "uavenv_step: a gather is pending (uavenv_set_step_gather) and this launch has no gather role");
     if (!actions) return fail(UAVENV_EINVAL, "null actions");
     if (!e->have_world) return fail(UAVENV_EINVAL, "uavenv_step before uavenv_set_buildings");
     if (action_kind < 0 || action_kind > 2) return fail(UAVENV_EINVAL, "action_kind %d", action_kind);
@@ -2471,6 +2566,7 @@
 {
     if (!e) return fail(UAVENV_EINVAL, "null env");
     const PendingMeta pm = take_step_meta(e);
+    const GatherArgs pg = take_step_gather(e);
     if (!net || !net->local || !obs_cur || !action_out) return fail(UAVENV_EINVAL, "null argument");
     if (!e->have_world) return fail(UAVENV_EINVAL, "uavenv_step_policy before uavenv_set_buildings");
     if ((flags & UAVENV_STEP_AUTO_RESET) && e->bank_m <= 0)
@@ -2489,6 +2585,8 @@
                           (size_t)e->world_bytes + 16 + uavq::kPolBytes <= 40960;
     if (!shape_ok || !(coop_packed || wave_f16))
         return fail(UAVENV_EINVAL, "uavenv_step_policy: this env / net takes uavenv_dqn_act + uavenv_step");
+    if (pg.staged && !(coop_packed && image_dev && (((uintptr_t)image_dev) & 15u) == 0 && env_int("UAVENV_STAGE_VGPR", 0) == 0))
+        return fail(UAVENV_EINVAL, "uavenv_step_policy: a gather is pending (uavenv_set_step_gather) and this launch has no gather role");
     StepArgs a = base_args(e);
     a.actions = action_out;
     a.action_kind = UAVENV_ACT_INDEX_I32;
@@ -2512,6 +2610,7 @@
     a.pol_counter = counter;
     a.meta = reinterpret_cast<uint4 *>(pm.meta);
     a.meta_a1 = pm.a1;
+    a.gather = pg;
     if (e->mask_bytes == 4) launch_step<uint32_t>(e, a, (hipStream_t)stream);
     else launch_step<uint64_t>(e, a, (hipStream_t)stream);
     HIP_TRY(hipGetLastError());
diff --git a/dqn_based_uav_3d_path_planer_amd/csrc/uavenv_device.hpp b/dqn_based_uav_3d_path_planer_amd/csrc/uavenv_device.hpp
--- a/dqn_based_uav_3d_path_planer_amd/csrc/uavenv_device.hpp
+++ b/dqn_based_uav_3d_path_planer_amd/csrc/uavenv_device.hpp
@@ -839,4 +839,8 @@
     if (f < 0) f += frames;
 }
 
-}
+constexpr int kStagedRowsN = 64 * kPackedDwords, kStagedRec = 2 * kStagedRowsN, kStagedIdx = kStagedRec + 64 * 4;
+constexpr int kStagedTileDwords = kStagedIdx + 64 * 2;
+constexpr uint32_t kStagedFresh = 0x80000000u;
+
+}
diff --git a/dqn_based_uav_3d_path_planer_amd/loop.py b/dqn_based_uav_3d_path_planer_amd/loop.py
--- a/dqn_based_uav_3d_path_planer_amd/loop.py
+++ b/dqn_based_uav_3d_path_planer_amd/loop.py
@@ -12,6 +12,16 @@
 
 class P2PExchangeError(_lib.UavEnvError):
     """uavenv_loop_run returned UAVENV_EP2P (csrc/p2p.hip: timeout or diverged ranks)."""
+
+
+STAGED_GATHER_DEFAULT = 2
+
+
+def staged_gather_eligible(ring, learner, batch: int, per=None, sample_lag: int = 0, valid_draws: bool = False) -> bool:
+    net = learner.net
+    return (per is None and not valid_draws and sample_lag == 0 and batch > 0 and ring.meta is not None and
+            ring.env.obs_code == _lib.OBS_PACKED and net.mfma_dtype == _lib.MFMA_F32 and net.w == 100 and net.hid == 64 and
+            net.n_actions + (1 if net.dueling else 0) <= 4 and bool(net.target))
 
 
 class HotLoop:
@@ -19,7 +29,7 @@
                  counter: int = 0, learn_start: int = 0, auto_reset: bool = True, skip_done: bool = None,
                  time_every: int = 0, info: torch.Tensor = None, per=None, sample_lag: int = 0,
                  replan_every: int = 0, replan_count: int = 0, replan_max_iter: int = 10000, gate_updates: bool = False,
-                 valid_draws: bool = None):
+                 valid_draws: bool = None, staged_gather: bool = None):
         if not ring.discrete:
             raise ValueError("HotLoop drives the discrete (DQN-family) path")
         if batch % 64:
@@ -84,9 +94,22 @@
                 raise ValueError("valid_draws needs skip_done (with auto-reset every stored row is valid)")
             self._draw_idx = torch.zeros((int(batch), 2), dtype=torch.int32, device=env.device)
             cfg.per_idx_dev = self._draw_idx.data_ptr()
+        eligible = staged_gather_eligible(ring, learner, int(batch), per=per, sample_lag=int(sample_lag),
+                                          valid_draws=self._draw_idx is not None)
+        if staged_gather and not eligible:
+            raise ValueError("staged_gather needs the plain update (no prioritised replay, no valid-draw list, sample_lag 0) on a "
+                             "packed ring with records and the f32-MFMA 100-64 net with at most 4 layer-2 outputs")
+        if not eligible:
+            self.staged_gather = 0
+        elif staged_gather is None:
+            self.staged_gather = STAGED_GATHER_DEFAULT
+        else:
+            self.staged_gather = 1 if staged_gather else 0
+        cfg.staged_gather = self.staged_gather
         self._h = C.c_void_p()
         _lib.check(self.lib.uavenv_loop_create(C.byref(cfg), C.byref(self._h)), "uavenv_loop_create")
         self.counter = int(counter)
+        self.staged_passes = 0
         self.batch = int(batch)
         self._seen = (ring.head, ring.filled, learner.epoch)
 
@@ -125,6 +148,7 @@
         self.ring.head, self.ring.filled = cur.head, cur.filled
         self.learner.epoch = cur.epoch
         self.counter = int(cur.counter)
+        self.staged_passes = int(cur.staged_passes)
         self._seen = (cur.head, cur.filled, cur.epoch)
         if self._per is not None:
             beta = C.c_double(0.0)
diff --git a/include/uavenv.h b/include/uavenv.h
--- a/include/uavenv.h
+++ b/include/uavenv.h
@@ -115,6 +115,20 @@
 } UavReplayRing;
 #define UAVENV_META_BYTES 16
 int uavenv_set_step_meta(UavEnv *env, void *meta_frame_dev, const float *action1_frame_dev);
+
+#define UAVENV_STAGED_TILE_BYTES 11776
+#define UAVENV_STAGED_FRESH 0x80000000u
+#define UAVENV_GATHER_PLAIN_STORES 1u
+#define UAVENV_GATHER_DELAY_SHIFT 8
+typedef struct UavStepGather {
+    UavReplayRing ring;
+    int32_t head, filled;
+    int32_t batch;
+    uint32_t flags;
+    uint64_t seed, counter;
+    void *staged_dev;
+} UavStepGather;
+int uavenv_set_step_gather(UavEnv *env, const UavStepGather *request);
 
 int uavenv_replay_sample(const UavReplayRing *ring, int32_t head, int32_t filled, int32_t batch, uint64_t seed,
                          uint64_t counter, void *obs_b, void *next_obs_b, void *action_b, float *reward_b,
@@ -316,11 +330,13 @@
     float *per_w_dev;
     float *per_abs_dev;
     int32_t *per_idx_dev;
-    int32_t replan_every, replan_count, replan_max_iter, reserved1;
+    int32_t replan_every, replan_count, replan_max_iter;
+    int32_t staged_gather;
     uint32_t *moved_dev;
 } UavLoopConfig;
 typedef struct UavLoopCursor {
-    int32_t head, filled, epoch, reserved0;
+    int32_t head, filled, epoch;
+    int32_t staged_passes;
     uint64_t counter;
 } UavLoopCursor;
 
```

New measurement: 620.2 million. 0.988x the previous value.
